# al-mcintyre/mCaller

Hardware: AMD Instinct MI355X
Metric: m6A calls/sec (GATC motif, E. coli-like synthetic eventalign) (higher is better)
Workload: dtype f64 (K1 window means, everything written); K2 hidden layer f32 + f64 output + f64 re-evaluation near print boundaries (MCALLER_MLP_FP64=1 = f64 throughout: ms_per_step_fp64_mlp); 1 GPU; synthetic 1e+08 eventalign rows per GPU and step, -m GATC, NN classifier (r95 two-base MLP), skip_thresh 0; two resident tables taken in turn, every step a FULL pass (the table declared new: positions + event indices streamed, every row validated); step=full pass, passes_in_flight=4, events_per_gpu=100000000, flush_records_per_gpu=204194, copy_out_bytes_per_pass=8767737

## Files before the change

include/mcaller_hip.h:

```cpp
#ifndef MCALLER_HIP_H
#define MCALLER_HIP_H

#define MC_E_NO_FREE_SLOT (-16)

#include <stdint.h>

#ifdef __cplusplus
extern "C" {
#endif

#define MC_MAX_K 8

#define MC_F_KMER_EQ    0x01
#define MC_F_MODEL_N    0x02
#define MC_F_SEG_START  0x04
#define MC_F_NAME_START 0x08

typedef struct mc_table_view {
    int64_t n_rows;
    const int32_t *pos;
    const int32_t *event_model_e4;
    const int32_t *event_idx;
    const uint8_t *flags;
    int32_t n_seg;
    const int64_t *seg_row_begin;
    const int32_t *seg_read;
    const int32_t *seg_contig;
    int32_t n_reads;
    const uint8_t *model_n_bits;
    const uint16_t *idx_rel_bits;
} mc_table_view;
void mc_pack_model_n(const uint8_t *flags, int64_t n_rows, uint8_t *out);
void mc_pack_idx_rel(const int32_t *event_idx, int64_t n_rows, uint16_t *out);

typedef struct mc_ref_view {
    int32_t n_contigs;
    const int64_t *contig_len;
    const int64_t *seq_off;
    const uint8_t *seq;
    const int64_t *word_off;
    const uint32_t *mbits_fwd;
    const uint32_t *mbits_rev;
    int64_t n_seq_bytes, n_words;
} mc_ref_view;

#define MC_I_EMPTY_MASK   0x000000FFu
#define MC_I_REV          0x00000100u
#define MC_I_TOO_MANY     0x00000200u
#define MC_I_MULTI        0x00000400u
#define MC_I_EDGE         0x00000800u
#define MC_I_NEXT_SHIFT   16

typedef struct mc_calls_view {
    int64_t capacity;
    double  *feats;
    int32_t *site_pos;
    int32_t *site_seg;
    int64_t *close_row;
    uint32_t *info;
    double  *prob;
    int32_t *call_row;
    int64_t n_call_rows;
    int32_t *close_row32;
    int32_t compacted;
    const int32_t *feats_lo32;
    const uint32_t *feats_hi32;
    const uint8_t *feats_wide;
    int64_t n_wide;
} mc_calls_view;

const char *mc_last_error(void);
const char *mc_version(void);
int mc_host_cores(void);
int mc_mark_motifs(const char *seq, int64_t n, const char *motif_fwd, const char *repl_fwd, int32_t m_fwd,
                   const char *motif_rev, const char *repl_rev, int32_t m_rev, char *upper_out, char *fwd_out, char *rev_out);

#define MC_IUPAC_MAX_MOTIFS 8
#define MC_IUPAC_MAX_LEN 32
typedef struct mc_iupac_motif {
    int32_t m;
    uint32_t called;
    uint8_t set[MC_IUPAC_MAX_LEN];
} mc_iupac_motif;
typedef struct mc_iupac_spec {
    int32_t n_motifs, pad;
    mc_iupac_motif fwd[MC_IUPAC_MAX_MOTIFS];
    mc_iupac_motif rev[MC_IUPAC_MAX_MOTIFS];
} mc_iupac_spec;
int mc_iupac_spec_add(mc_iupac_spec *spec, const char *motif, int32_t m, uint32_t called);
int mc_mark_iupac(const char *seq, int64_t n, const mc_iupac_spec *spec, char *upper_out, char *fwd_out, char *rev_out);

void *mc_host_alloc(int64_t bytes);
void mc_host_free(void *p);
int mc_host_is_pinned(const void *p);
int mc_host_pool_config(int32_t parser_uses_pool, int64_t keep_bytes);

typedef struct mc_parsed mc_parsed;
int mc_parse_eventalign(const char *path, int64_t startline, int64_t endline,
                        const char *const *contig_names, int32_t n_contigs, int32_t n_threads,
                        mc_parsed **out);
int mc_parse_eventalign_range(const char *path, int64_t byte_begin, int64_t byte_end,
                              const char *const *contig_names, int32_t n_contigs, int32_t n_threads, mc_parsed **out);
int mc_eventalign_read_cuts(const char *path, int32_t n_parts, int64_t *cuts);
int mc_eventalign_read_cuts_range(const char *path, int64_t lo, int64_t hi, int32_t n_parts, int64_t *cuts);
int mc_eventalign_read_cuts_at(const char *path, int64_t lo, int64_t hi, const int64_t *want, int32_t n_want, int64_t *cuts);
int mc_eventalign_consumed_range(const char *path, int64_t startline, int64_t endline, int64_t *lo, int64_t *hi);
int mc_parsed_view(const mc_parsed *p, mc_table_view *out);
const char *mc_parsed_read_name(const mc_parsed *p, int32_t read_id);
int64_t mc_parsed_n_unknown(const mc_parsed *p);
const char *mc_parsed_unknown_name(const mc_parsed *p, int64_t i);
int32_t mc_parsed_n_pieces(const mc_parsed *p);
void mc_parsed_free(mc_parsed *p);

typedef struct mc_fastq mc_fastq;
int mc_fastq_read_quality(const char *path, int32_t n_threads, mc_fastq **out);
int64_t mc_fastq_view(const mc_fastq *f, const char **key_pool, const int64_t **key_off, const double **mean);
void mc_fastq_free(mc_fastq *f);

typedef struct mc_ctx mc_ctx;
int mc_ctx_create(int device, mc_ctx **out);
int mc_bind_to_device_numa_node(int device);
// ... 142 lines not shown
} mc_nb_params;
int mc_nb_fit(mc_ctx *ctx, const mc_nb_params *prm, const double *X, const uint8_t *y, int64_t n_samples, int32_t n_in, int32_t n_jobs,
              const int64_t *train_off, const int32_t *train_idx, const int64_t *val_off, const int32_t *val_idx, double *theta,
              double *var, double *epsilon, int64_t *class_count, int64_t *val_correct);

typedef struct mc_devparse_result {
    int32_t status;
    int64_t n_lines, n_rows;
    int32_t n_seg, n_unknown;
    const int64_t *seg_row_begin;
    const int32_t *seg_contig;
    const int64_t *seg_name_off;
    const int32_t *seg_name_len;
    const uint8_t *seg_name_start;
    const int64_t *unknown_off;
    const int32_t *unknown_len;
    const uint8_t *flags;
} mc_devparse_result;
int mc_read_file_range(const char *path, int64_t byte_begin, int64_t byte_end, char *dst, int32_t n_threads);
int mc_map_file_range(const char *path, int64_t lo, int64_t hi, void **handle, const char **ptr);
void mc_unmap_file_range(void *handle);
int mc_ctx_parse_begin(mc_ctx *ctx, const char *text, int64_t n_bytes, const char *const *contig_names, int32_t n_contigs,
                       int64_t max_rows, int32_t *slot);
int mc_ctx_parse_end(mc_ctx *ctx, int32_t slot, mc_devparse_result *out);
int mc_ctx_parse_finish(mc_ctx *ctx, int32_t slot, const int32_t *seg_read, int32_t n_reads, const double *read_qual);
int mc_ctx_parse_abandon(mc_ctx *ctx, int32_t slot);
int mc_ctx_fetch_columns(mc_ctx *ctx, int32_t slot, int64_t n_rows, int32_t *pos, int32_t *event_model_e4, int32_t *event_idx,
                         uint8_t *flags);
int mc_ctx_fetch_model_n_bits(mc_ctx *ctx, int32_t slot, int64_t n_rows, uint8_t *out);
int mc_ctx_fetch_idx_rel_bits(mc_ctx *ctx, int32_t slot, int64_t n_rows, uint16_t *out);
int mc_ctx_fetch_pos_rel_bits(mc_ctx *ctx, int32_t slot, int64_t n_rows, uint16_t *out);
int mc_ctx_fetch_unit_summaries(mc_ctx *ctx, int32_t slot, int64_t n_rows, int32_t *out);

typedef struct mc_format_args {
    const mc_calls_view *rec;
    int64_t n_records;
    int32_t k;
    const mc_table_view *table;
    const mc_ref_view *ref;
    const char *const *contig_names;
    const char *const *read_names;
    const char *const *read_qual_txt;
    const char *tail_chrom;
    const char *label_meth;
    const char *label_unmeth;
    const uint8_t *submodel_of_char;
} mc_format_args;
int mc_format_diffs(const mc_format_args *args, int64_t first, int32_t n_threads, char **text, int64_t *n_bytes,
                    int64_t *n_rows, int64_t *stop_at);
int mc_count_records(const mc_calls_view *rec, int64_t n, const int32_t *seg_read, int64_t n_seg, int64_t *counts3, int32_t *ascending,
                     uint8_t *pos_marks, int64_t n_marks, int64_t *pos_min, int64_t *pos_top);
int mc_calls_expand(const mc_calls_view *rec, int64_t n_records, int32_t k, int32_t *call_row_out, int64_t *close_row_out,
                    double *feats_out);
void mc_free(void *p);
int mc_repr_double(double v, char *out32);
int mc_repr_fixed4(int32_t d, char *out32);
int mc_repr_double_rowtext(double v, char *out32);

typedef struct mc_text_source {
    const char *text;
    const char *path;
    int64_t n_bytes;
} mc_text_source;

typedef struct mc_bed_params {
    int64_t min_depth;
    double mod_threshold;
    int32_t control;
    int32_t with_probs;
    int32_t gff;
    int32_t site_stats;
} mc_bed_params;
typedef struct mc_bed_stats {
    int64_t n_bytes, n_lines, n_counted, n_entries, n_sites, n_out_bytes;
    int64_t decline_line;
    int32_t decline_reason;
    int32_t longest_probe;
    int64_t table_slots;
    int64_t kernel_bytes;
    double ms_read, ms_h2d, ms_kernels, ms_d2h, ms_total;
} mc_bed_stats;
#define MC_BED_DECLINE_HIGH_BYTE   1
#define MC_BED_DECLINE_CONTROL     2
#define MC_BED_DECLINE_FIELDS      3
#define MC_BED_DECLINE_POSITION    4
#define MC_BED_DECLINE_CONTEXT     5
#define MC_BED_DECLINE_LABEL       6
#define MC_BED_DECLINE_NO_PROB     7
#define MC_BED_DECLINE_LONG_LINE   8
#define MC_BED_DECLINE_TABLE       9
#define MC_BED_DECLINE_ROWS        10
#define MC_BED_DECLINE_MEMORY      11
#define MC_BED_DECLINE_OPTIONS     12
#define MC_BED_DECLINE_POS_HIGH_BYTE 13
#define MC_BED_DECLINE_POS_CONTROL   14
#define MC_BED_DECLINE_POS_LONG_LINE 15
#define MC_BED_DECLINE_VALUE         16
#define MC_BED_DECLINE_FEW_VALUES    17
#define MC_BED_DECLINE_MANY_VALUES   18
#define MC_BED_DECLINE_VALUE_COUNT   19
#define MC_BED_DECLINE_ZERO_VARIANCE 20
#define MC_BED_DECLINE_FAR_TAIL      21
#define MC_BED_DECLINE_PRINT_RANGE   22
#define MC_BED_DECLINE_ROUNDING_TIE  23
#define MC_BED_DECLINE_DEPTH         24
#define MC_BED_DECLINE_PROBABILITY   25
// ... 390 lines not shown
```

mcaller_amd/_lib.py:

```python
import ctypes as C
import os

import numpy as np

from . import _abi

_HERE = os.path.dirname(os.path.abspath(__file__))
LIB_PATH = os.environ.get('MCALLER_LIB') or os.path.join(_HERE, 'libmcaller_hip.so')

ABI = _abi.load()
_K, _S = ABI.constants, ABI.structs

MC_MAX_K = _K['MC_MAX_K']
F_KMER_EQ, F_MODEL_N, F_SEG_START, F_NAME_START = (_K['MC_F_' + n] for n in ('KMER_EQ', 'MODEL_N', 'SEG_START', 'NAME_START'))
I_EMPTY_MASK, I_REV, I_TOO_MANY, I_MULTI, I_EDGE, I_NEXT_SHIFT = (
    _K['MC_I_' + n] for n in ('EMPTY_MASK', 'REV', 'TOO_MANY', 'MULTI', 'EDGE', 'NEXT_SHIFT'))
E_NO_FREE_SLOT = _K['MC_E_NO_FREE_SLOT']


class McError(RuntimeError):
    code = None


TableView = _S['mc_table_view']
# ... 597 lines not shown
    if not (L.ndim == 1 and L.shape == bound.shape and len(L) >= 1):
        raise ValueError('curcombine: two arrays of one length, at least 1')
    out, b, st = np.zeros(2), C.c_double(), C.c_int32()
    rc = lib().mc_curcombine(L.ctypes.data, bound.ctypes.data, len(L), float(log10c), out.ctypes.data, C.byref(b), C.byref(st))
    if rc != 0:
        raise ValueError('mc_curcombine: %d' % rc)
    return float(out[0]), float(out[1]), float(b.value), int(st.value)


def hypergeom_round4(v):
    return lib().mc_hypergeom_round4(float(v))


def hypergeom_tie4(v, err):
    return bool(lib().mc_hypergeom_tie4(float(v), float(err)))


def parse_double(token):
    if isinstance(token, str):
        token = token.encode('latin-1', 'replace')
    out = C.c_double()
    return out.value if lib().mc_parse_double(token, len(token), C.byref(out)) else None


def repr_double_rowtext(x):
    buf = C.create_string_buffer(40)
    n = lib().mc_repr_double_rowtext(float(x), buf)
    return buf.value.decode() if n >= 0 else None


def repr_fixed4(d):
    buf = C.create_string_buffer(40)
    lib().mc_repr_fixed4(int(d), buf)
    return buf.value.decode()


class Records(object):

    def __init__(self, capacity, k):
        self.k = k
        self.capacity = int(capacity)
        c = max(1, self.capacity)
        self.feats = np.zeros(c * k, dtype=np.float64)
        self.site_pos = np.zeros(c, dtype=np.int32)
        self.site_seg = np.zeros(c, dtype=np.int32)
        self.close_row = np.zeros(c, dtype=np.int64)
        self.info = np.zeros(c, dtype=np.uint32)
        self.prob = np.full(c, np.nan, dtype=np.float64)
        self.n = 0

    def view(self):
        v = CallsView()
        v.capacity = self.capacity
        v.site_pos, v.site_seg = _ptr(self.site_pos), _ptr(self.site_seg)
        v.info, v.prob = _ptr(self.info), _ptr(self.prob)
        if self._feats is None and self._packed is not None:
            lo, hi, wide = self._packed
            v.feats_lo32, v.feats_hi32, v.feats_wide, v.n_wide = _ptr(lo), _ptr(hi), _ptr(wide), len(hi)
        else:
            v.feats = _ptr(self.feats)
        if self._close_row is not None or self._close_row32 is None:
            v.close_row = _ptr(self.close_row)
        else:
            v.close_row32 = _ptr(self._close_row32)
        if self._compacted:
            v.compacted, v.n_call_rows = 1, int(self._n_calls)
            if self._call_row is not None:
                v.call_row = _ptr(self._call_row)
        return v

    @classmethod
    def from_view(cls, v, n, k, owner):
        r = cls.__new__(cls)
        r.k, r.capacity, r.n, r._owner = k, n, n, owner
        if v.feats:
            r.feats = _from_ptr(v.feats, n * k, np.float64)
        r.site_pos = _from_ptr(v.site_pos, n, np.int32)
        r.site_seg = _from_ptr(v.site_seg, n, np.int32)
        if v.close_row:
            r._close_row = _from_ptr(v.close_row, n, np.int64)
        else:
            r._close_row32 = _from_ptr(v.close_row32, n, np.int32)
        r.info = _from_ptr(v.info, n, np.uint32)
        if v.compacted:
            m = int(v.n_call_rows)
            r._compacted = True
            if v.call_row:
                r._call_row = _from_ptr(v.call_row, n, np.int32)
            r._n_calls = m
            if v.feats:
                r.feats = _from_ptr(v.feats, m * k, np.float64)
            else:
                r._packed = (_from_ptr(v.feats_lo32, m * k, np.int32), _from_ptr(v.feats_hi32, int(v.n_wide), np.uint32),
                             _from_ptr(v.feats_wide, m, np.uint8))
            r.prob = _from_ptr(v.prob, m, np.float64)
        else:
            r.prob = _from_ptr(v.prob, n, np.float64)
        return r

    _close_row = _close_row32 = _call_row = _feats = _packed = None
    _compacted = False

    @property
    def feats(self):
        if self._feats is None and self._packed is not None:
            out = np.empty(max(1, self._n_calls * self.k), dtype=np.float64)
            v = self.view()
            check(lib().mc_calls_expand(C.byref(v), int(self.n), int(self.k), None, None, _ptr(out)))
            self._feats = out[:self._n_calls * self.k]
        return self._feats

    @feats.setter
    def feats(self, a):
        self._feats = a

    @property
    def close_row(self):
        if self._close_row is None and self._close_row32 is not None:
            self._close_row = self._close_row32.astype(np.int64)
        return self._close_row

    @close_row.setter
    def close_row(self, a):
        self._close_row = a

    @property
    def call_row(self):
        if self._call_row is None and self._compacted:
            keep = (self.info[:self.n] & I_TOO_MANY) == 0
            rows = np.cumsum(keep, dtype=np.int64) - 1
            rows[~keep] = -1
            self._call_row = rows.astype(np.int32)
        return self._call_row

    @call_row.setter
    def call_row(self, a):
        self._call_row = a
        self._compacted = a is not None

    def count(self, n, seg_read=None, pos_marks=None):
        v = self.view()
        counts = np.zeros(3, dtype=np.int64)
        asc, lo, top = C.c_int32(0), C.c_int64(0), C.c_int64(0)
        if seg_read is not None:
            seg_read = np.ascontiguousarray(seg_read, dtype=np.int32)
        check(lib().mc_count_records(C.byref(v), int(n), _ptr(seg_read) if seg_read is not None else None,
                                     len(seg_read) if seg_read is not None else 0, _ptr(counts) if seg_read is not None else None,
                                     C.byref(asc), _ptr(pos_marks) if pos_marks is not None else None,
                                     len(pos_marks) if pos_marks is not None else 0, C.byref(lo), C.byref(top)))
        return (tuple(int(c) for c in counts) if seg_read is not None else None), bool(asc.value), int(lo.value), int(top.value)

    @property
    def n_calls(self):
        return self._n_calls if self._compacted else self.n

    def by_record(self):
        if self.call_row is None:
            return self
        n, k = self.n, self.k
        r = Records(n, k)
        r.n = n
        for name in ('site_pos', 'site_seg', 'close_row', 'info'):
            getattr(r, name)[:n] = getattr(self, name)[:n]
        kept = self.call_row[:n] >= 0
        rows = self.call_row[:n][kept]
        r.feats.reshape(-1, k)[:n][kept] = self.feats.reshape(-1, k)[rows]
        r.prob[:n][kept] = self.prob[rows]
        return r


# ... 17 lines not shown
```

mcaller_amd/csrc/mc_classify.hip:

```cpp
#include "mc_dev.h"
#include "mc_rows.h"

namespace {

template <bool PIN>
struct VgprConstT {
    double v;
    __device__ __forceinline__ explicit VgprConstT(double x) : v(x) { if (PIN) asm volatile("" : "+v"(v)); }
    __device__ __forceinline__ operator double() const { return v; }
};
template <bool PIN>
struct ExpConstsT {
    using VgprConst = VgprConstT<PIN>;
    VgprConst two_log2e{2.8853900817779268}, magic{6755399441055744.0}, half_ln2_hi{-0.3465735901845619},
        half_ln2_lo{-9.541074646352939e-11};
    VgprConst t_max4{87.5};
    VgprConst g9{5.1405589494805136e-05}, g8{0.0002828297056809958}, g7{0.0014109321451518497}, g6{0.00634918945176432},
        g5{0.02539682542470863}, g4{0.08888888907016779}, g3{0.26666666666656197}, g2{0.6666666666659861},
        g1{1.3333333333333335}, g0{2.0000000000000004};
};
using ExpConsts = ExpConstsT<true>;

template <class EC>
__device__ __forceinline__ double exp2t_plus1(double t, const EC &C) {
// ... 85 lines not shown
__device__ __forceinline__ float tanh32s(float s) {
    return __builtin_fmaf(__builtin_amdgcn_rcpf(1.0f + __builtin_amdgcn_exp2f(s)), -2.0f, 1.0f);
}
__device__ __forceinline__ f2 tanh32s_2(f2 s) {
    const f2 d = (f2){__builtin_amdgcn_exp2f(s.x), __builtin_amdgcn_exp2f(s.y)} + 1.0f;
    const f2 r = {__builtin_amdgcn_rcpf(d.x), __builtin_amdgcn_rcpf(d.y)};
    return __builtin_elementwise_fma(r, (f2){-2.0f, -2.0f}, (f2){1.0f, 1.0f});
}

__device__ __forceinline__ double threshold_distance(double p) {
    const double t = p * 100.0;
    const double d = fabs((t - floor(t)) - 0.5) * 0.01;
    return fmin(d, fabs(p - 0.5));
}

struct K2Pieces {
    const int32_t *cnt;
    int room;
    int64_t n;
};
#ifndef MC_K2_THREADS
#define MC_K2_THREADS 1024
#endif
constexpr int K2_THREADS = MC_K2_THREADS;
constexpr int K2B = K2_THREADS;
constexpr int K2_WAVES = K2_THREADS / 64;
constexpr int K2_FIX = K2B + 256;
static_assert(K2_WAVES >= 4 && K2_WAVES % 4 == 0, "four unit quarters");
static_assert(K2_MAXM <= 16, "a wave's list claims are one atomic of K2_MAXM lanes; the loops over the sub-models are written out");

#ifdef MC_K2_TRACE
__device__ unsigned long long g_k2_trace[1024 * 16 * 16];
#define K2_STAMP(i) do { if (lane == 0 && blockIdx.x < 1024) g_k2_trace[((size_t)blockIdx.x * K2_WAVES + wave) * 16 + (i)] = wall_clock64(); g_k2_trace[((size_t)blockIdx.x * K2_WAVES + wave) * 16 + 8 + (i)] = clock64(); } while (0)
__device__ unsigned long long g_k2_timeline[256 * 24 * 8];
#define K2_TL(i) do { if (tid == 0 && blockIdx.x < 256 && stretch_no < 24) g_k2_timeline[((size_t)blockIdx.x * 24 + stretch_no) * 8 + (i)] = wall_clock64(); } while (0)
__device__ unsigned long long g_side_trace[1024 * 16 * 16];
#define K2_WALL(i) do { if ((threadIdx.x & 63) == 0 && blockIdx.x < 1024) g_side_trace[((size_t)blockIdx.x * K2_WAVES + (threadIdx.x >> 6)) * 16 + (i)] = wall_clock64(); } while (0)
#else
#define K2_STAMP(i) do { } while (0)
#define K2_TL(i) do { } while (0)
#define K2_WALL(i) do { } while (0)
#endif


#define MC_SCALAR_MEM __attribute__((address_space(4)))

struct SidePack {
    K1Args A;
    const Payload *sorted;
    unsigned char *out;
    size_t out_bytes;
    Counters *host_status;
    int close32, score;
};
struct NoPack {};
#ifndef MC_SIDE_WAVES
#define MC_SIDE_WAVES 4
#endif
template <int NI_T, bool FAST, bool PACK = false, bool ROOMY = false, int TH = K2_THREADS>
__global__ __launch_bounds__(TH) __attribute__((amdgpu_waves_per_eu((FAST && !ROOMY) ? 8 : (ROOMY && FAST ? MC_SIDE_WAVES : 4), (FAST && !ROOMY) ? 8 : (ROOMY && FAST ? MC_SIDE_WAVES : 4)))) void k2_mlp(DevMlp M, const double *__restrict__ feats, int k,
                                                     const int32_t *__restrict__ site_seg, const int32_t *__restrict__ seg_read,
                                                     const double *__restrict__ qual, const uint32_t *__restrict__ info,
                                                     const uint8_t *__restrict__ submodel_in, int64_t n,
                                                     double *__restrict__ prob, const unsigned long long *__restrict__ n_dev,
                                                     const unsigned int *__restrict__ overflow, K2Pieces P,
                                                     std::conditional_t<PACK, SidePack, NoPack> SP) {
    if constexpr (PACK) {
        if (*overflow) {
            constexpr unsigned head_words = offsetof(Counters, end_of_head) / 4;
            if (blockIdx.x == 0 && threadIdx.x < head_words)
                reinterpret_cast<volatile unsigned int *>(SP.host_status)[threadIdx.x] = reinterpret_cast<const unsigned int *>(SP.A.cnt)[threadIdx.x];
            return;
        }
    } else if (overflow && *overflow) return;
    if (n_dev) n = min(n, (int64_t)*n_dev);
    K2_WALL(0);
    constexpr int KB = TH, KW = TH / 64, KFIX = TH + 256;
    static_assert(KW >= 4 && KW % 4 == 0, "four unit quarters");
    constexpr int NX = NI_T ? NI_T : MC_MAX_K + 1;
    const int H = M.n_hidden, NI = NI_T ? NI_T : M.n_in, S = NI + 2, NM = min(M.n_models, K2_MAXM);
    using part_t = std::conditional_t<FAST, float, double>;
    __shared__ uint16_t s_list[K2_MAXM][KB];
    __shared__ int s_tot[2][K2_MAXM];
    __shared__ double s_q[KB];
    __shared__ part_t s_part[4][KB];
    __shared__ float s_marg[FAST ? KB : 1];
    __shared__ unsigned long long s_fixlist[FAST ? KFIX : 1];
    __shared__ int s_nfix;
    __shared__ int32_t s_slot[KB];
    __shared__ uint32_t s_fixrow[(FAST && PACK) ? KFIX : 1];
    __shared__ int2 s_pk[PACK ? 2 : 1][PACK ? KW : 1];
    __shared__ unsigned long long s_base[PACK ? 2 : 1][4];
    __shared__ unsigned long long s_red[PACK ? 6 : 1][PACK ? KW : 1];
    __shared__ unsigned long long s_lay[PACK ? 8 : 1];
    const int tid = threadIdx.x, lane = tid & 63;
    const int wave = __builtin_amdgcn_readfirstlane(tid >> 6);
    const unsigned long long below = (1ull << lane) - 1ull;
    const ExpConstsT<!FAST> C;
    K2_STAMP(0);
    __shared__ uint32_t s_simd_of_wave[KW / 4];
    const int simd = (int)__builtin_amdgcn_s_getreg((2 - 1) << 11 | 4 << 6 | 4) & 3;
    __shared__ uint8_t s_soc[256];
    if (tid < 256) s_soc[tid] = M.sub_of_char ? M.sub_of_char[tid] : (uint8_t)255;
    if (lane == 0) reinterpret_cast<uint8_t *>(s_simd_of_wave)[wave] = (uint8_t)simd;
    if (tid < 2 * K2_MAXM) (&s_tot[0][0])[tid] = 0;
    if (tid == 0) s_nfix = 0;
    __syncthreads();
    int quarter, g_first, g_step;
    {
        uint32_t per_simd = 0;
        int slot = 0;
        for (int w4 = 0; w4 < KW / 4; ++w4) {
            const uint32_t four = __builtin_amdgcn_readfirstlane(s_simd_of_wave[w4]);
#pragma unroll
            for (int b = 0; b < 4; ++b) {
                const int sd = (four >> (8 * b)) & 3;
                per_simd += 1u << (8 * sd);
                slot += (w4 * 4 + b < wave && sd == simd) ? 1 : 0;
            }
        }
        const bool by_simd = (per_simd & 0xFFu) && (per_simd & 0xFF00u) && (per_simd & 0xFF0000u) && (per_simd & 0xFF000000u);
        quarter = by_simd ? simd : wave & 3;
        g_first = by_simd ? slot : wave >> 2;
        g_step = by_simd ? (int)((per_simd >> (8 * simd)) & 0xFFu) : KW / 4;
    }
    const bool pieces = P.cnt != nullptr;
    const int64_t n_units = pieces ? P.n : n;
    const int64_t per = (n_units + gridDim.x - 1) / gridDim.x;
    int64_t lo = min(n_units, blockIdx.x * per), hi = min(n_units, lo + per);
    K2_WALL(1);
    if constexpr (PACK) {
        unsigned long long v[6] = {0, 0, 0, 0, 0, 0};
        if (pieces) {
            for (int64_t j0 = 32 * (int64_t)tid; j0 < P.n; j0 += 32 * TH) {
                int4 k4[8];
#pragma unroll
                for (int e = 0; e < 8; ++e) k4[e] = *reinterpret_cast<const int4 *>(SP.A.piece_kw + min(j0 + 4 * e, (P.n - 1) & ~(int64_t)3));
#pragma unroll
                for (int e = 0; e < 32; ++e) {
                    const int64_t j = j0 + e;
                    if (j >= P.n) continue;
                    const int4 kk = k4[e >> 2];
                    const uint32_t kw = (uint32_t)((e & 3) == 0 ? kk.x : (e & 3) == 1 ? kk.y : (e & 3) == 2 ? kk.z : kk.w);
                    const uint32_t c = kw & 511u, kept = (kw >> 9) & 511u, wide = kw >> 18;
                    v[0] += kept; v[1] += wide; v[2] += c;
                    if (j < lo) { v[3] += kept; v[4] += wide; v[5] += c; }
                }
            }
        } else {
            const int64_t per_c = (n + PACK_WGS - 1) / PACK_WGS;
            const int c0 = (int)((int64_t)blockIdx.x * PACK_WGS / gridDim.x), c1 = (int)((int64_t)(blockIdx.x + 1) * PACK_WGS / gridDim.x);
            lo = min(n, c0 * per_c); hi = min(n, c1 * per_c);
            for (int j = tid; j < PACK_WGS; j += TH) {
                const unsigned long long kk = SP.A.chunk_cnt[PACK_PAD * j], ww = SP.A.chunk_cnt[PACK_PAD * j + 1];
                v[0] += kk; v[1] += ww;
                if (j < c0) { v[3] += kk; v[4] += ww; }
            }
            if (tid == 0) { v[2] = (unsigned long long)n; v[5] = (unsigned long long)lo; }
        }
        K2_WALL(2);
        if (tid < 6) s_red[PACK ? tid : 0][0] = 0ull;
        __syncthreads();
#pragma unroll
        for (int i = 0; i < 6; ++i) {
            unsigned long long x = v[i];
#pragma unroll
            for (int o = 32; o > 0; o >>= 1) x += __shfl_xor(x, o);
            if (lane == 0 && x) atomicAdd(&s_red[PACK ? i : 0][0], x);
        }
        __syncthreads();
#pragma unroll
        for (int i = 0; i < 6; ++i) v[i] = s_red[PACK ? i : 0][0];
        __syncthreads();
        const size_t need_bytes = pack_tail(pack_layout((int64_t)v[2], SP.close32).feats, (size_t)v[0], k, (size_t)v[1]).end;
        const bool too_big = need_bytes > SP.out_bytes;
        if (too_big) lo = hi;
        if (tid == 0) {
            const PackLayout PL = pack_layout((int64_t)v[2], SP.close32);
            const PackTail PTl = pack_tail(PL.feats, (size_t)v[0], k, (size_t)v[1]);
            s_lay[0] = PL.pos; s_lay[1] = PL.seg; s_lay[2] = PL.info; s_lay[3] = PTl.lo32; s_lay[4] = PTl.wmask; s_lay[5] = PTl.hi32;
            s_lay[6] = PTl.prob;
            s_base[0][0] = v[3]; s_base[0][1] = v[4]; s_base[0][2] = v[5];
            s_red[0][1] = v[2]; s_red[1][1] = v[0]; s_red[2][1] = v[1];
            s_red[3][1] = need_bytes;
        }
        __syncthreads();
        K2_WALL(3);
        const int64_t n_rare = too_big ? 0 : (int64_t)SP.A.cnt->n_rare;
        if (n_rare > 0) {
            const int64_t rlo = pieces ? lo * P.room : lo, rhi = pieces ? hi * P.room : hi;
            for (int64_t i = tid; i < n_rare; i += TH) {
                const int64_t q = SP.A.rare_list[i];
#ifndef MC_SIDE_NO_RARE
                if (q >= rlo && q < rhi && finish_rare_record<false>(SP.A, SP.sorted, q, true)) {
                    const unsigned long long was = atomicExch(&SP.A.cnt->irregular_pass, SP.A.pass_no);
                    asm volatile("" :: "v"(was));
                }
#endif
            }
            __syncthreads();
        }
    }
    K2_WALL(4);
    K2_STAMP(1);
    auto again_in_fp64 = [&](int n_fix) {
        for (int f = wave; f < n_fix; f += KW) {
            const unsigned long long ent = s_fixlist[FAST ? f : 0];
            const int64_t r = (int64_t)(ent & ((1ull << 56) - 1ull));
            const int mdl = (int)(ent >> 56);
            double x[NX];
            const double q = qual[seg_read[site_seg[r]]];
#pragma unroll
            for (int i = 0; i < NX; ++i) x[i] = i < k ? feats[r * k + i] : (i == k ? q : 0.0);
            double part = 0.0;
            for (int u = lane; u < H; u += 64) {
                const double *wu = M.wu + ((size_t)mdl * H + u) * S;
                double a0 = x[0] * wu[0];
#pragma unroll
                for (int i = 1; i < NX; ++i)
                    if (i < NI) a0 = fma(x[i], wu[i], a0);
                part = fma(tanh_1exp(a0 + wu[NI], C), wu[NI + 1], part);
            }
#pragma unroll
            for (int o = 32; o > 0; o >>= 1) part += __shfl_xor(part, o);
            if (lane == 0) {
                const double pr = logistic(part + M.b2[mdl], C);
                prob[r] = pr;
                if constexpr (PACK) reinterpret_cast<double *>(SP.out + s_lay[PACK ? 6 : 0])[s_fixrow[(FAST && PACK) ? f : 0]] = pr;
            }
        }
    };
    int buf = 0, stretch_no = 0;
    (void)stretch_no;
    int64_t base = lo;
    while (base < hi) {
        K2_STAMP(7);
        K2_TL(0);
        int n_here, np_here = 1, my_slot = tid;
        int64_t slot0 = base;
        if (pieces) {
            const bool have = lane < 16 && base + lane < hi;
            const int c = have ? min(max(P.cnt[base + lane], 0), P.room) : 0;
            int incl = c;
#pragma unroll
            for (int o = 1; o < 16; o <<= 1) {
                const int v = __shfl_up(incl, o);
                if (lane >= o) incl += v;
            }
            np_here = max(1, __popcll(__ballot(have && incl <= KB)));
            n_here = min(__builtin_amdgcn_readlane(incl, np_here - 1), KB);
            int before = 0, j = 0;
#pragma unroll
            for (int t = 0; t < 15; ++t) {
                const int inc_t = __builtin_amdgcn_readlane(incl, t);
                if (t + 1 < np_here && inc_t <= tid) { j = t + 1; before = inc_t; }
            }
            my_slot = j * P.room + (tid - before);
            slot0 = base * (int64_t)P.room;
            s_slot[tid] = my_slot;
        } else n_here = (int)min((int64_t)KB, hi - base);
        const int64_t r = slot0 + my_slot;
        int mi = 255;
        double qv = 0.0;
        [[maybe_unused]] int p_nw = -1;
        if (tid < n_here) {
            if (submodel_in) mi = submodel_in[r];
            else {
                const uint32_t inf = info[r];
                const int32_t seg = site_seg[r];
                if constexpr (PACK) { if (!(inf & MC_I_TOO_MANY)) p_nw = __popc((uint32_t)SP.A.O.wmask[r] & ((1u << k) - 1u)); }
                bool scored = !(inf & (MC_I_TOO_MANY | MC_I_EDGE));
                if constexpr (PACK) scored = scored && SP.score != 0;
                if (scored) {
                    mi = s_soc[(inf >> MC_I_NEXT_SHIFT) & 0xFFu];
                    qv = qual[seg_read[seg]];
                }
            }
        }
        if constexpr (PACK) {
            const int nk = __popcll(__ballot(p_nw >= 0));
            int nw = max(p_nw, 0);
#pragma unroll
            for (int o = 32; o > 0; o >>= 1) nw += __shfl_xor(nw, o);
            if (lane == 0) s_pk[PACK ? buf : 0][PACK ? wave : 0] = make_int2(nk, nw);
        }
        int rank = 0, cnt_lane = 0;
#pragma unroll
        for (int m = 0; m < K2_MAXM; ++m) {
            const unsigned long long bal = __ballot(mi == m && m < NM);
            if (mi == m) rank = __popcll(bal & below);
            if (lane == m) cnt_lane = __popcll(bal);
        }
        int wbase = 0;
        if (lane < K2_MAXM && cnt_lane) wbase = atomicAdd(&s_tot[buf][lane], cnt_lane);
        int mybase = 0;
#pragma unroll
        for (int m = 0; m < K2_MAXM; ++m) {
            const int b = __builtin_amdgcn_readlane(wbase, m);
            mybase = mi == m ? b : mybase;
        }
        if (mi < NM) s_list[mi][mybase + rank] = (uint16_t)tid;
        s_q[tid] = qv;
        K2_STAMP(2);
        K2_WALL(5);
        K2_TL(1);
        __syncthreads();
        K2_WALL(6);
        K2_TL(2);
        int tot[K2_MAXM], gs[K2_MAXM], n_groups = 0;
#pragma unroll
        for (int m = 0; m < K2_MAXM; ++m) {
            tot[m] = __builtin_amdgcn_readfirstlane(s_tot[buf][m]);
            gs[m] = n_groups;
            n_groups += (tot[m] + 63) >> 6;
        }
        if (tid < K2_MAXM) s_tot[buf ^ 1][tid] = 0;
        K2_STAMP(3);
        K2_WALL(7);
        const int u0 = quarter * H / 4, u1 = (quarter + 1) * H / 4;
        for (int g = g_first; g < n_groups; g += g_step) {
            int mdl = 0, tot_m = tot[0], lg = g;
#pragma unroll
            for (int m = 1; m < K2_MAXM; ++m)
                if (g >= gs[m] && tot[m] > 0) { mdl = m; tot_m = tot[m]; lg = g - gs[m]; }
            const int idx = lg * 64 + lane;
            const bool valid = idx < tot_m;
            const int off = s_list[mdl][valid ? idx : lg * 64];
            const int64_t rr = slot0 + (pieces ? s_slot[off] : off);
            double x[NX];
            if (submodel_in) {
#pragma unroll
                for (int i = 0; i < NX; ++i) x[i] = i < NI ? feats[rr * NI + i] : 0.0;
            } else {
                const double q = s_q[off];
#pragma unroll
                for (int i = 0; i < NX; ++i) x[i] = i < k ? feats[rr * k + i] : (i == k ? q : 0.0);
            }
// ... 35 lines not shown
                        if (i < NI) m = __builtin_fmaf(fabsf(xx[i].x) * 1.0000002f, mg[1 + i], m);
                    s_marg[FAST ? off : 0] = m * 1.000001f;
                }
            } else {
                const MC_SCALAR_MEM double *wu = (const MC_SCALAR_MEM double *)M.wu + ((size_t)mdl * H + u0) * S;
                int u = u0;
                for (; u + 4 <= u1; u += 4, wu += 4 * S) {
                    double a0 = x[0] * wu[0], a1 = x[0] * wu[S], a2 = x[0] * wu[2 * S], a3 = x[0] * wu[3 * S];
    #pragma unroll
                    for (int i = 1; i < NX; ++i)
                        if (i < NI) {
                            a0 = fma(x[i], wu[i], a0);
                            a1 = fma(x[i], wu[S + i], a1);
                            a2 = fma(x[i], wu[2 * S + i], a2);
                            a3 = fma(x[i], wu[3 * S + i], a3);
                        }
                    a0 += wu[NI]; a1 += wu[S + NI]; a2 += wu[2 * S + NI]; a3 += wu[3 * S + NI];
                    tanh_4(a0, a1, a2, a3, C);
                    z = fma(a0, wu[NI + 1], z);
                    z = fma(a1, wu[S + NI + 1], z);
                    z = fma(a2, wu[2 * S + NI + 1], z);
                    z = fma(a3, wu[3 * S + NI + 1], z);
                }
                for (; u < u1; ++u, wu += S) {
                    double a0 = x[0] * wu[0];
    #pragma unroll
                    for (int i = 1; i < NX; ++i)
                        if (i < NI) a0 = fma(x[i], wu[i], a0);
                    z = fma(tanh_1exp(a0 + wu[NI], C), wu[NI + 1], z);
                }
            }
            if (valid) s_part[quarter][off] = (part_t)z;
        }
        K2_STAMP(4);
        K2_WALL(8);
        K2_TL(3);
        __syncthreads();
        K2_WALL(9);
        K2_STAMP(5);
        K2_TL(4);
        [[maybe_unused]] double p_pr = __longlong_as_double(0x7ff8000000000000LL);
        [[maybe_unused]] bool p_fix = false;
        if (mi < NM) {
            const double z = (((double)s_part[0][tid] + (double)s_part[1][tid]) + (double)s_part[2][tid]) + (double)s_part[3][tid];
            const double pr = logistic(z + M.b2[mi], C);
            prob[r] = pr;
            const bool fix = FAST && !(threshold_distance(pr) > (double)s_marg[FAST ? tid : 0]);
            if constexpr (PACK) { p_pr = pr; p_fix = fix; }
            else if (fix) s_fixlist[FAST ? atomicAdd(&s_nfix, 1) : 0] = (unsigned long long)r | (unsigned long long)mi << 56;
        }
        if constexpr (PACK) {
            K2_WALL(11);
            if (tid == 0) {
                unsigned kept_s = 0, wide_s = 0;
                for (int w = 0; w < KW; ++w) { const int2 c = s_pk[PACK ? buf : 0][PACK ? w : 0]; kept_s += (unsigned)c.x; wide_s += (unsigned)c.y; }
                s_base[PACK ? buf ^ 1 : 0][0] = s_base[PACK ? buf : 0][0] + kept_s;
                s_base[PACK ? buf ^ 1 : 0][1] = s_base[PACK ? buf : 0][1] + wide_s;
                s_base[PACK ? buf ^ 1 : 0][2] = s_base[PACK ? buf : 0][2] + (unsigned long long)n_here;
            }
            if (tid < n_here) {
                const uint32_t inf = info[r];
                const int32_t seg = site_seg[r], pos = SP.A.O.site_pos[r];
                const int64_t close = SP.A.O.close_row[r];
                const bool keep = !(inf & MC_I_TOO_MANY);
                const uint32_t wm = keep ? ((uint32_t)SP.A.O.wmask[r] & ((1u << k) - 1u)) : 0u;
                double fx[MC_MAX_K];
#pragma unroll
                for (int f = 0; f < MC_MAX_K; ++f) fx[f] = (keep && f < k) ? feats[r * k + f] : 0.0;
                const unsigned long long kb = __ballot(keep);
                const int nw = __popc(wm);
                int w_incl = nw;
#pragma unroll
                for (int o = 1; o < 64; o <<= 1) {
                    const int y = __shfl_up(w_incl, o);
                    if (lane >= o) w_incl += y;
                }
                unsigned long long row = s_base[PACK ? buf : 0][0] + (unsigned)__popcll(kb & below), wpos = s_base[PACK ? buf : 0][1] + (unsigned)(w_incl - nw);
#pragma unroll
                for (int w = 0; w < KW; ++w) {
                    const int2 c = s_pk[PACK ? buf : 0][PACK ? w : 0];
                    if (w < wave) { row += (unsigned)c.x; wpos += (unsigned)c.y; }
                }
                const unsigned long long real0 = s_base[PACK ? buf : 0][2];
                const int64_t io = pieces ? (int64_t)real0 + tid : r;
                unsigned char *const out = SP.out;
                if (SP.close32) reinterpret_cast<int32_t *>(out)[io] = (int32_t)close;
                else reinterpret_cast<int64_t *>(out)[io] = close;
                reinterpret_cast<int32_t *>(out + s_lay[0])[io] = pos;
                reinterpret_cast<int32_t *>(out + s_lay[PACK ? 1 : 0])[io] = seg;
                reinterpret_cast<uint32_t *>(out + s_lay[PACK ? 2 : 0])[io] = inf;
                if (keep) {
                    int32_t *o_lo = reinterpret_cast<int32_t *>(out + s_lay[PACK ? 3 : 0]) + row * k;
                    uint32_t *o_hi = reinterpret_cast<uint32_t *>(out + s_lay[PACK ? 5 : 0]);
                    (out + s_lay[PACK ? 4 : 0])[row] = (uint8_t)wm;
                    reinterpret_cast<double *>(out + s_lay[PACK ? 6 : 0])[row] = p_pr;
#pragma unroll
                    for (int f = 0; f < MC_MAX_K; ++f)
                        if (f < k) {
                            if (!((wm >> f) & 1u)) o_lo[f] = (int32_t)rint(fx[f] * 1e4);
                            else {
                                const unsigned long long bits = (unsigned long long)__double_as_longlong(fx[f]);
                                o_lo[f] = (int32_t)(uint32_t)bits;
                                o_hi[wpos++] = (uint32_t)(bits >> 32);
                            }
                        }
                    if (p_fix) {
                        const int at = atomicAdd(&s_nfix, 1);
                        s_fixlist[FAST ? at : 0] = (unsigned long long)r | (unsigned long long)mi << 56;
                        s_fixrow[(FAST && PACK) ? at : 0] = (uint32_t)row;
                    }
                }
            }
        }
        base += pieces ? np_here : KB;
        buf ^= 1;
        K2_STAMP(6);
        K2_WALL(10);
        K2_TL(5);
        ++stretch_no;
#ifdef MC_K2_TRACE
        if (lane == 0 && blockIdx.x < 1024)
            g_k2_trace[((size_t)blockIdx.x * K2_WAVES + wave) * 16 + 7] = (unsigned)simd | (unsigned)quarter << 4 | (unsigned)g_first << 8 | (unsigned)g_step << 16 | (unsigned long long)n_groups << 24;
#endif
    }
    if constexpr (FAST) {
        __syncthreads();
        again_in_fp64(s_nfix);
    }
    K2_WALL(13);
    if constexpr (PACK) {
        __shared__ int s_last;
        __syncthreads();
        if (tid == 0) s_last = atomicAdd(&SP.A.cnt->side_done, 1ull) == (unsigned long long)gridDim.x - 1ull;
        __syncthreads();
        if (s_last) {
            constexpr unsigned head_words = offsetof(Counters, end_of_head) / 4;
            constexpr int kept_word = (int)(offsetof(Counters, n_kept) / 4);
            constexpr int overflow_word = (int)(offsetof(Counters, overflow) / 4), need_word = (int)(offsetof(Counters, pack_need) / 4);
            static_assert(offsetof(Counters, n_wide) == offsetof(Counters, n_kept) + 8 && offsetof(Counters, n_records) == 0, "Counters layout");
            static_assert(sizeof(Counters::overflow) == 4 && sizeof(Counters::pack_need) == 8 && offsetof(Counters, pack_need) % 8 == 0, "Counters layout");
            const unsigned long long need_bytes = s_red[PACK ? 3 : 0][PACK ? 1 : 0];
            const bool too_big = need_bytes > SP.out_bytes;
            if (tid < (int)head_words && (tid < kept_word || tid >= kept_word + 4) && tid >= 2) {
                unsigned int w = __hip_atomic_load(reinterpret_cast<unsigned int *>(SP.A.cnt) + tid, __ATOMIC_RELAXED, __HIP_MEMORY_SCOPE_AGENT);
                if (too_big && tid == overflow_word) w |= 1u;
                if (too_big && (tid == need_word || tid == need_word + 1)) w = (unsigned int)(need_bytes >> (tid == need_word ? 0 : 32));
                reinterpret_cast<volatile unsigned int *>(SP.host_status)[tid] = w;
            }
            if (tid == 0) {
                *reinterpret_cast<volatile unsigned long long *>(&SP.host_status->n_records) = s_red[0][PACK ? 1 : 0];
                *reinterpret_cast<volatile unsigned long long *>(&SP.host_status->n_kept) = s_red[PACK ? 1 : 0][PACK ? 1 : 0];
                *reinterpret_cast<volatile unsigned long long *>(&SP.host_status->n_wide) = s_red[PACK ? 2 : 0][PACK ? 1 : 0];
            }
        }
    }
    K2_WALL(14);
}

constexpr int K3_THREADS = 256;
__global__ __launch_bounds__(K3_THREADS) void k3_forest(DevForest F, const double *__restrict__ feats, int k,
                                                        const int32_t *__restrict__ site_seg, const int32_t *__restrict__ seg_read,
                                                        const double *__restrict__ qual, const uint32_t *__restrict__ info,
                                                        const uint8_t *__restrict__ submodel_in, int64_t n,
                                                        double *__restrict__ prob, const unsigned long long *__restrict__ n_dev,
                                                        const unsigned int *__restrict__ overflow) {
    __shared__ double s_x[K3_THREADS][MC_MAX_K + 2];
    if (overflow && *overflow) return;
    if (n_dev) n = min(n, (int64_t)*n_dev);
    const int NI = F.n_in;
    const int tid = threadIdx.x, lane = tid & 63, wave = __builtin_amdgcn_readfirstlane(tid >> 6);
    const int64_t n_waves = (int64_t)gridDim.x * (K3_THREADS / 64);
    if (n <= n_waves * 16) {
        double *x = s_x[wave * 64];
        for (int64_t r = (int64_t)blockIdx.x * (K3_THREADS / 64) + wave; r < n; r += n_waves) {
            int mi;
            if (submodel_in) {
                mi = submodel_in[r];
                if (lane < NI) x[lane] = (double)(float)feats[r * NI + lane];
            } else {
                const uint32_t inf = info[r];
                if (inf & (MC_I_TOO_MANY | MC_I_EDGE)) continue;
                mi = F.sub_of_char[(inf >> MC_I_NEXT_SHIFT) & 0xFFu];
                if (lane < k) x[lane] = (double)(float)feats[r * k + lane];
                if (lane == k) x[k] = (double)(float)qual[seg_read[site_seg[r]]];
            }
            if (mi >= F.n_models) continue;
            __builtin_amdgcn_fence(__ATOMIC_ACQ_REL, "wavefront");
            const int t0 = F.model_tree_off[mi], t1 = F.model_tree_off[mi + 1];
            double sum = 0.0;
            for (int tb = t0; tb < t1; tb += 64) {
                const int t = tb + lane;
                double q = 0.0;
                if (t < t1) {
                    int node = F.tree_node_off[t];
                    int l;
                    while ((l = F.left[node]) >= 0) node = (x[F.feature[node]] <= F.threshold[node]) ? l : F.right[node];
                    const double v0 = F.value[2 * (size_t)node], v1 = F.value[2 * (size_t)node + 1];
                    double norm = (-0.0 + v0) + v1;
                    if (norm == 0.0) norm = 1.0;
                    q = v1 / norm;
                }
                const int here = min(64, t1 - tb);
                for (int j = 0; j < here; ++j)
                    sum += __hiloint2double(__builtin_amdgcn_readlane(__double2hiint(q), j), __builtin_amdgcn_readlane(__double2loint(q), j));
            }
// ... 333 lines not shown
            const bool literal = noted != 0xFFu || !look;
            for (int f = 0; f < k; ++f) {
                const double x = s_feats[tid * k + f];
                int32_t d = 0;
                const bool narrow = literal ? !((noted >> f) & 1u) : slot_is_narrow(x, &d);
                if (narrow) lo32[f] = literal ? (int32_t)rint(x * 1e4) : d;
                else {
                    const unsigned long long bits = (unsigned long long)__double_as_longlong(x);
                    lo32[f] = (int32_t)(uint32_t)bits;
                    hi32[n_w++] = (uint32_t)(bits >> 32);
                    wmask |= 1u << f;
                }
            }
        }
        const unsigned long long kmask = __ballot(keep);
        unsigned int w_incl = n_w;
        for (int o = 1; o < 64; o <<= 1) {
            const unsigned int y = __shfl_up(w_incl, o);
            if (lane >= o) w_incl += y;
        }
        const unsigned long long vmask = __ballot(valid);
        if (lane == 63) s_wave[1][wave] = w_incl;
        if (lane == 0) { s_wave[0][wave] = (unsigned int)__popcll(kmask); s_wave[2][wave] = (unsigned int)__popcll(vmask); }
        __syncthreads();
        unsigned int in_strip = (unsigned int)__popcll(kmask & ((1ull << lane) - 1ull)), strip = 0, w_off = w_incl - n_w, w_strip = 0;
        unsigned int r_in_strip = (unsigned int)__popcll(vmask & ((1ull << lane) - 1ull)), r_strip = 0;
        for (int j = 0; j < PACK_THREADS / 64; ++j) {
            if (j < wave) { in_strip += s_wave[0][j]; w_off += s_wave[1][j]; r_in_strip += s_wave[2][j]; }
            strip += s_wave[0][j];
            w_strip += s_wave[1][j];
            r_strip += s_wave[2][j];
        }
        if (valid) {
            const int64_t io = holes ? (int64_t)(rbase + r_in_strip) : i;
            if (close32) o_close32[io] = (int32_t)O.close_row[i];
            else o_close[io] = O.close_row[i];
            o_pos[io] = O.site_pos[i];
            o_seg[io] = O.site_seg[i];
            o_info[io] = info;
            if (keep) {
                const unsigned long long row = base + in_strip;
                o_prob[row] = O.prob[i];
                o_mask[row] = (uint8_t)wmask;
                for (int f = 0; f < k; ++f) o_lo[row * k + f] = lo32[f];
                for (unsigned int j = 0; j < n_w; ++j) o_hi[wbase + w_off + j] = hi32[j];
            }
        }
        __syncthreads();
        base += strip;
        wbase += w_strip;
        rbase += r_strip;
    }
}


}

#ifndef MC_K2_WG_PER_CU
#define MC_K2_WG_PER_CU 1
#endif
#ifndef MC_SIDE_WGS_SPARSE
#define MC_SIDE_WGS_SPARSE 128
#endif
#ifndef MC_K2_WG_MANY
#define MC_K2_WG_MANY 2
#endif

void mc_launch_classifier(const DevMlp &M, const DevForest &F, const DevSimple &S, const DevSvm &V, int n_cu, hipStream_t st, const double *feats, int k,
                          const int32_t *site_seg, const int32_t *seg_read, const double *qual, const uint32_t *info,
                          const uint8_t *submodel_in, int64_t n, double *prob, const unsigned long long *n_dev, const unsigned int *overflow,
                          const int32_t *piece_cnt, int piece_room, int64_t n_pieces) {
    if (n <= 0) return;
    const K2Pieces P{(piece_room > 0 && piece_room < K2B) ? piece_cnt : nullptr, piece_room, n_pieces};
    if (V.sv) {
        const unsigned grid = (unsigned)std::max<int64_t>(1, std::min<int64_t>((n + K3S_THREADS - 1) / K3S_THREADS, (int64_t)n_cu * 8));
        if (V.n_in == 7)
            hipLaunchKernelGGL(k3_svm<7>, dim3(grid), dim3(K3S_THREADS), 0, st, V, feats, k, site_seg, seg_read, qual, info, submodel_in, n,
                               prob, n_dev, overflow);
        else
            hipLaunchKernelGGL(k3_svm<0>, dim3(grid), dim3(K3S_THREADS), 0, st, V, feats, k, site_seg, seg_read, qual, info, submodel_in, n,
                               prob, n_dev, overflow);
    } else if (F.left)
        hipLaunchKernelGGL(k3_forest, dim3((unsigned)std::max<int64_t>(1, std::min<int64_t>((n + 3) / 4, (int64_t)n_cu * 8))), dim3(K3_THREADS), 0, st,
                           F, feats, k, site_seg, seg_read, qual, info, submodel_in, n, prob, n_dev, overflow);
    else if (S.params)
        hipLaunchKernelGGL(k3_simple, dim3((unsigned)((n + 63) / 64)), dim3(64), 0, st, S, feats, k, site_seg, seg_read, qual, info,
                           submodel_in, n, prob, n_dev, overflow);
    else {
        const bool fast = M.fast && M.wp32 && !submodel_in;
        const bool many = P.cnt != nullptr || n >= ((int64_t)4 << 20);
        const unsigned grid = (unsigned)std::max<int64_t>(1, std::min<int64_t>((n + 255) / 256, (int64_t)n_cu * ((fast && many) ? MC_K2_WG_MANY : MC_K2_WG_PER_CU)));
        if (M.n_in == 7 && fast)
            hipLaunchKernelGGL((k2_mlp<7, true>), dim3(grid), dim3(K2_THREADS), 0, st, M, feats, k, site_seg, seg_read, qual, info, submodel_in, n,
                               prob, n_dev, overflow, P, NoPack{});
        else if (M.n_in == 7)
            hipLaunchKernelGGL((k2_mlp<7, false>), dim3(grid), dim3(K2_THREADS), 0, st, M, feats, k, site_seg, seg_read, qual, info, submodel_in, n,
                               prob, n_dev, overflow, P, NoPack{});
        else if (fast)
            hipLaunchKernelGGL((k2_mlp<0, true>), dim3(grid), dim3(K2_THREADS), 0, st, M, feats, k, site_seg, seg_read, qual, info, submodel_in, n,
                               prob, n_dev, overflow, P, NoPack{});
        else
            hipLaunchKernelGGL((k2_mlp<0, false>), dim3(grid), dim3(K2_THREADS), 0, st, M, feats, k, site_seg, seg_read, qual, info, submodel_in, n,
                               prob, n_dev, overflow, P, NoPack{});
    }
}

void mc_launch_pack_count(const DevRecords &O, const Counters *cnt, int k, unsigned long long *chunk_cnt, int holes, hipStream_t st) {
    hipLaunchKernelGGL(k_pack_count, dim3(PACK_WGS), dim3(PACK_THREADS), 0, st, O, cnt, k, chunk_cnt, holes);
}

void mc_launch_pack(const DevRecords &O, const Counters *cnt, const unsigned long long *chunk_cnt, unsigned char *out, size_t out_bytes, int k,
                    int close32, Counters *host_status, int holes, int look, hipStream_t st, hipEvent_t stop) {
    if (stop) hipExtLaunchKernelGGL(k_pack, dim3(PACK_WGS), dim3(PACK_THREADS), 0, st, nullptr, stop, 0, O, cnt, chunk_cnt, out, out_bytes, k, close32, host_status, holes, look);
    else hipLaunchKernelGGL(k_pack, dim3(PACK_WGS), dim3(PACK_THREADS), 0, st, O, cnt, chunk_cnt, out, out_bytes, k, close32, host_status, holes, look);
}

bool mc_launch_side(const DevMlp &M, bool other_classifier, int n_cu, hipStream_t st, const K1Args &A, const Payload *sorted, const int32_t *seg_read,
                    const double *qual, int64_t cap, int score, unsigned char *out, size_t out_bytes, int close32, Counters *host_status,
                    int piece_room, int64_t n_pieces, hipEvent_t stop) {
    static const bool off = getenv("MCALLER_SIDE_FUSED") && atoi(getenv("MCALLER_SIDE_FUSED")) == 0;
    if (off || cap <= 0) return false;
    if (score && (other_classifier || !M.W1)) return false;
    const bool by_piece = piece_room > 0;
    constexpr int TH_SIDE = MC_SIDE_MAX_ROOM;
    if (by_piece ? (piece_room >= TH_SIDE || !A.piece_kw || !A.piece_cnt) : !A.chunk_cnt) return false;
    SidePack SP;
    SP.A = A; SP.sorted = sorted; SP.out = out; SP.out_bytes = out_bytes; SP.host_status = host_status; SP.close32 = close32; SP.score = score;
    const K2Pieces P{by_piece ? A.piece_cnt : nullptr, piece_room, n_pieces};
    const bool fast = score && M.fast && M.wp32;
    unsigned grid;
    const int grid_env = getenv("MCALLER_SIDE_GRID") ? atoi(getenv("MCALLER_SIDE_GRID")) : 0;
    if (by_piece) grid = (unsigned)std::max<int64_t>(1, std::min<int64_t>(n_pieces, grid_env > 0 ? (int64_t)grid_env : (int64_t)n_cu * (MC_SIDE_WAVES / 2)));
    else {
        const int want = grid_env > 0 ? grid_env : MC_SIDE_WGS_SPARSE;
        grid = 1;
        while (grid * 2 <= (unsigned)std::min<int64_t>(std::min(want, PACK_WGS), (int64_t)n_cu * 2)) grid *= 2;
    }
    const unsigned long long *n_dev = (const unsigned long long *)&A.cnt->n_records;
    const unsigned int *overflow = (const unsigned int *)&A.cnt->overflow;
#define MC_SIDE_LAUNCH(NI, FA) hipExtLaunchKernelGGL((k2_mlp<NI, FA, true, true, TH_SIDE>), dim3(grid), dim3(TH_SIDE), 0, st, nullptr, stop, 0, M, (const double *)A.O.feats, A.k, \
        (const int32_t *)A.O.site_seg, seg_read, qual, (const uint32_t *)A.O.info, (const uint8_t *)nullptr, cap, A.O.prob, n_dev, overflow, P, SP)
    if (score && M.n_in == 7 && fast) MC_SIDE_LAUNCH(7, true);
    else if (score && M.n_in == 7) MC_SIDE_LAUNCH(7, false);
    else if (fast) MC_SIDE_LAUNCH(0, true);
    else MC_SIDE_LAUNCH(0, false);
#undef MC_SIDE_LAUNCH
    return true;
}

namespace {
__global__ void k_tanh32_err(unsigned long long *out) {
    unsigned long long worst = 0ull;
    for (unsigned long long i = blockIdx.x * (unsigned long long)blockDim.x + threadIdx.x; i < (1ull << 32); i += (unsigned long long)gridDim.x * blockDim.x) {
        const float x = __uint_as_float((unsigned)i);
        if (!(fabsf(x) <= 3.4e38f)) continue;
        const double err = fabs((double)tanh32s(x) - tanh((double)x * 0.34657359027997264));
        const unsigned long long b = (unsigned long long)__double_as_longlong(err);
        worst = b > worst ? b : worst;
    }
    for (int o = 32; o > 0; o >>= 1) { const unsigned long long v = __shfl_xor(worst, o); worst = v > worst ? v : worst; }
    if ((threadIdx.x & 63) == 0) atomicMax(out, worst);
}
}
extern "C" int mc_debug_tanh32_max_err(double *out) {
    unsigned long long *d = nullptr;
    HIP_TRY(hipMalloc((void **)&d, 8));
    HIP_TRY(hipMemset(d, 0, 8));
    hipLaunchKernelGGL(k_tanh32_err, dim3(4096), dim3(256), 0, 0, d);
    unsigned long long h = 0;
    HIP_TRY(hipMemcpy(&h, d, 8, hipMemcpyDeviceToHost));
    (void)hipFree(d);
    memcpy(out, &h, 8);
    return 0;
}

#ifdef MC_K2_TRACE
extern "C" int mc_debug_k2_timeline(unsigned long long *out, int64_t n_words) {
    if (n_words > 256 * 24 * 8) n_words = 256 * 24 * 8;
    return hipMemcpyFromSymbol(out, HIP_SYMBOL(g_k2_timeline), (size_t)n_words * 8) == hipSuccess ? 0 : -10;
}
// ... 10 lines not shown
```

mcaller_amd/csrc/mc_ctx.h:

```cpp
#pragma once
#include "mc_dev.h"
#include "mc_own.h"

#include <atomic>
#include <string>

#ifndef MC_PASSES_IN_FLIGHT_N
#define MC_PASSES_IN_FLIGHT_N 6
#endif
constexpr int MC_PASSES_IN_FLIGHT = MC_PASSES_IN_FLIGHT_N;
constexpr int MC_ROW_TEXT_BLOCKS = 6;
static_assert(MC_ROW_TEXT_BLOCKS <= 8, "a block's handle is ticket * 8 + index");

constexpr size_t COPY_BY_KERNEL_MAX = (size_t)4 << 20;
constexpr size_t COPY_BY_KERNEL_MAX_STREAMING = (size_t)64 << 20;

struct K0Set {
    NbDesc *desc = nullptr;
    int64_t *nb_f0 = nullptr;
};

struct PassBufs {
    K0Set K;
    Counters *cnt = nullptr;
// ... 74 lines not shown
    int kp_state = 0;
    bool from_parser = false;
    int64_t kp_flags_sent = 0;
    std::vector<int64_t> kp_seg_row, kp_seg_off, kp_unk_off;
    std::vector<int32_t> kp_seg_contig, kp_seg_len, kp_unk_len;
    std::vector<uint8_t> kp_seg_ns;
    Pool kp_allocs{"device parser slot"};
    long long tmpl_ref = -1;
    Pool allocs{"table slot"};
};

struct Classifier {
    enum Kind { NONE = -1, MLP = 0, FOREST = 1, SIMPLE = 2, SVM = 3 };
    DevMlp M;
    DevForest F;
    DevSimple Sc;
    DevSvm Vs;
    Pool pool{"classifier"};
    Kind kind = NONE;
    int n_in = 0;
    const uint8_t *sub_of_char = nullptr;
    void clear() {
        pool.clear();
        M = DevMlp(); F = DevForest(); Sc = DevSimple(); Vs = DevSvm();
        kind = NONE; n_in = 0; sub_of_char = nullptr;
    }
    void set(Kind k, int n, const uint8_t *soc) { kind = k; n_in = n; sub_of_char = soc; }
};

enum {
    EV_K0_START, EV_K0_END, EV_SCAN_START, EV_SCAN_END, EV_EMIT_END, EV_K2_START, EV_K2_END,
    EV_LIST_END,
    EV_EMIT_START,
    EV_DONE, EV_COPIED, EV_TEXT, EV_N
};

struct AsyncBuf {
    PassBufs B;
    DevRecords H;
    Pinned st;
    unsigned char *pack = nullptr;
    Pinned pack_host;
    unsigned long long *chunk_cnt = nullptr;
    int32_t *piece_cnt = nullptr;
    int32_t *piece_kw = nullptr;
    int64_t piece_cap = 0;
    size_t pack_bytes = 0;
    int32_t *h_lo32 = nullptr;
    uint32_t *h_hi32 = nullptr;
    unsigned char *h_wmask = nullptr;
    int64_t h_n_wide = 0;
    int32_t *h_close32 = nullptr;
    bool close32 = false;
    int64_t h_n_calls = 0;
    Event ev[EV_N];
    mc_params prm;
    int64_t cap = 0, n_nb = 0;
    int k = 0;
    bool used = false, copying = false, timed = true;
    bool one_kernel = false;
    int want_text = 0;
    int text_block = -1;
    bool emit_aside = false;
    int fused_room = 0;
    int64_t slots = 0;
    int slot = -1;
    const double *qual = nullptr;
    int32_t n_qual = 0;
    Pool dev_allocs{"pass buffers"}, k0_allocs{"strand resolve output"};
};

struct RowTextCtx {
    int on = 0;
    char lab_meth[8] = {}, lab_unmeth[8] = {};
    int lab_meth_len = 0, lab_unmeth_len = 0;
    RowTextScratch S = {};
    int64_t cap_rec = 0, cap_rows = 0, cap_wide = 0, cap_num = 0;
    Pool allocs{"row text scratch"}, out_allocs{"row text"};
    char *out = nullptr;
    size_t out_cap = 0;
    double bytes_per_row = 0.0;
    bool room_forced = false;
    struct Block {
        Pinned text, st;
        size_t cap = 0;
        std::atomic<int> busy{0};
    } blocks[MC_ROW_TEXT_BLOCKS];
    int next_ticket = 0;
    long long n_text = 0, n_no_block = 0, n_host_needed = 0, n_too_small = 0, n_other = 0;
    int last_block = -1;
    int64_t last_bytes = 0, last_rows = 0;
};

struct TextStages {
    Pinned stage[2];
    size_t cap = 0;
    Event ev[2];
    void release() {
        for (Pinned &p : stage) p.reset();
        cap = 0;
    }
};

struct mc_ctx {
    int device = 0;
    Stream stream;
// ... 115 lines not shown
```

mcaller_amd/csrc/mc_dev.h:

```cpp
#ifndef MC_DEV_H
#define MC_DEV_H
#include <hip/hip_runtime.h>
#include <hip/hip_ext.h>
#include <sched.h>

#include <algorithm>
#include <cctype>
#include <chrono>
#include <cmath>
#include <cstdio>
#include <cstdlib>
#include <cstring>
#include <type_traits>
#include <vector>

#include "../../include/mcaller_hip.h"

void mc_set_error(const char *fmt, ...);

#define HIP_TRY(expr)                                                                       \
    do {                                                                                    \
        hipError_t _e = (expr);                                                             \
        if (_e != hipSuccess) {                                                             \
            mc_set_error("%s failed: %s (%s:%d)", #expr, hipGetErrorString(_e), __FILE__, __LINE__); \
// ... 76 lines not shown
    double *feats = nullptr;
    int32_t *site_pos = nullptr, *site_seg = nullptr;
    int64_t *close_row = nullptr;
    uint32_t *info = nullptr;
    double *prob = nullptr;
    uint8_t *wmask = nullptr;
};

struct DevMlp {
    int32_t n_models = 0, n_in = 0, n_hidden = 0;
    double *W1 = nullptr, *b1 = nullptr, *W2 = nullptr, *b2 = nullptr;
    double *wu = nullptr;
    float *wp32 = nullptr;
    float *margin = nullptr;
    int fast = 0;
    uint8_t *sub_of_char = nullptr;
};
constexpr double K2_TANH32_MAX_ERR = 2.5e-7;

struct DevForest {
    int32_t n_models = 0, n_in = 0;
    int32_t *model_tree_off = nullptr, *tree_node_off = nullptr, *left = nullptr, *right = nullptr, *feature = nullptr;
    double *threshold = nullptr, *value = nullptr;
    uint8_t *sub_of_char = nullptr;
};

struct DevSimple {
    int32_t kind = 0, n_models = 0, n_in = 0, stride = 0;
    double *params = nullptr;
    uint8_t *sub_of_char = nullptr;
};

constexpr int K3S_MAXM = 8;
struct DevSvm {
    int32_t n_models = 0, n_in = 0;
    int32_t *model_sv_off = nullptr;
    double *sv = nullptr, *params = nullptr;
    uint8_t *sub_of_char = nullptr;
};

constexpr int NSHARD = 64, SHARD_PAD = 16;

struct Counters {
    unsigned long long n_records;
    unsigned int overflow;
    unsigned int violation;
    unsigned int n_big;
    unsigned int n_rare;
    unsigned long long n_kept;
    unsigned long long n_wide;
    unsigned long long side_done;
    unsigned long long pack_need;
    unsigned long long irregular_pass;
    unsigned long long end_of_head;
    unsigned long long pad_to_line[SHARD_PAD];
    unsigned long long shard[NSHARD * SHARD_PAD];
};
constexpr unsigned long long ST_UNPUBLISHED = ~0ull;

#define MC_FRONT_OF_THE_QUEUE __builtin_amdgcn_s_setprio(3)
#ifndef MC_SCAN_SUMMARY
#define MC_SCAN_SUMMARY 1
#endif
#ifndef MC_EVENTS_ON_KERNELS
#define MC_EVENTS_ON_KERNELS 1
#endif

__device__ __forceinline__ double div1e4(int x) {
    const double xd = (double)x, r = 1.0 / 10000.0;
    const double q0 = xd * r;
    return fma(fma(-q0, 10000.0, xd), r, q0);
}

__device__ __forceinline__ bool slot_is_narrow(double v, int32_t *d_out) {
    const double t = rint(v * 1e4);
    if (!(fabs(t) < 2147483648.0)) return false;
    const int32_t d = (int32_t)t;
    if (__double_as_longlong(div1e4(d)) != __double_as_longlong(v)) return false;
    *d_out = d;
    return true;
}

__device__ __forceinline__ int first_m(const uint32_t *__restrict__ bits, int64_t L, int64_t pos, int k) {
    if (pos >= L) return -1;
    const int64_t w0 = pos >> 5;
    const uint64_t lo = bits[w0], hi = bits[w0 + 1];
    uint64_t w = ((hi << 32) | lo) >> (pos & 31);
    w &= (1ull << k) - 1ull;
    return w ? __builtin_ctzll(w) : -1;
}

__device__ __forceinline__ int bit_at(const uint32_t *__restrict__ bits, int64_t p) {
    return (int)((bits[p >> 5] >> (p & 31)) & 1u);
}

__device__ __forceinline__ unsigned char comp_char(unsigned char c) {
    switch (c) {
        case 'A': return 'T';
        case 'C': return 'G';
        case 'G': return 'C';
        case 'T': return 'A';
        case 'N': return 'N';
        case 'M': return 'M';
        default: return 0xFF;
    }
}

constexpr uint32_t MC_I_BIG = 0x1000u;
// ... 2 lines not shown

struct RowSrc {
    const int32_t *g_pos;
    const int2 *g_evmu;
    const uint8_t *g_flags;
    bool stray_pending;
    double stray_val;
};

__device__ __forceinline__ double next_val(RowSrc &S, int64_t &cur) {
    if (S.stray_pending) {
        S.stray_pending = false;
        return S.stray_val;
    }
    for (;;) {
        const int64_t r = cur++;
        if (!(S.g_flags[r] & MC_F_MODEL_N)) {
            const int2 e = S.g_evmu[r];
            return (double)(e.x - e.y) / 10000.0;
        }
    }
}

__device__ __forceinline__ double leaf_sum(RowSrc &S, int64_t &cur, int n) {
    const int n8 = n < 8 ? 0 : n - (n % 8);
    double r0 = 0.0, r1 = 0.0, r2 = 0.0, r3 = 0.0, r4 = 0.0, r5 = 0.0, r6 = 0.0, r7 = 0.0;
    for (int i = 0; i < n8; ++i) {
        const double v = next_val(S, cur);
        switch (i & 7) {
            case 0: r0 += v; break;
            case 1: r1 += v; break;
            case 2: r2 += v; break;
            case 3: r3 += v; break;
            case 4: r4 += v; break;
            case 5: r5 += v; break;
            case 6: r6 += v; break;
            default: r7 += v; break;
        }
    }
    double res = n8 ? ((r0 + r1) + (r2 + r3)) + ((r4 + r5) + (r6 + r7)) : -0.0;
    for (int i = n8; i < n; ++i) res += next_val(S, cur);
    return res;
}

#ifndef MC_PACK_WGS
#define MC_PACK_WGS 512
#endif
#ifndef MC_PACK_THREADS
#define MC_PACK_THREADS 512
#endif
constexpr int PACK_WGS = MC_PACK_WGS, PACK_THREADS = MC_PACK_THREADS;

constexpr int PACK_PAD = 16;

__device__ __forceinline__ void count_for_packing(unsigned long long *chunk_cnt, int64_t q, int64_t n_rec, bool kept, int n_wide) {
    if (!chunk_cnt || !kept) return;
    const uint32_t per = (uint32_t)((n_rec + PACK_WGS - 1) / PACK_WGS);
    const uint32_t b = (uint32_t)q / per;
    atomicAdd(&chunk_cnt[PACK_PAD * b], 1ull);
    if (n_wide) atomicAdd(&chunk_cnt[PACK_PAD * b + 1], (unsigned long long)n_wide);
}

__device__ __forceinline__ void count_wave_for_packing(unsigned long long *chunk_cnt, int64_t n_rec, bool kept, int64_t q, uint32_t wmask, int k) {
    if (!chunk_cnt) return;
    const unsigned long long km = __ballot(kept);
    if (!km) return;
    uint32_t per = (uint32_t)((n_rec + PACK_WGS - 1) / PACK_WGS);
    asm volatile("" : "+s"(per));
    const uint32_t bq = kept ? (uint32_t)q / per : 0u;
    const int first = __ffsll((unsigned long long)km) - 1;
    const uint32_t b0 = (uint32_t)__shfl((int)bq, first);
    if (!__ballot(kept && bq != b0)) {
        int nw = 0;
        for (int f = 0; f < k; ++f) nw += __popcll(__ballot(kept && ((wmask >> f) & 1u)));
        if ((int)(threadIdx.x & 63) == first) {
            atomicAdd(&chunk_cnt[PACK_PAD * b0], (unsigned long long)__popcll(km));
            if (nw) atomicAdd(&chunk_cnt[PACK_PAD * b0 + 1], (unsigned long long)nw);
        }
    } else if (kept) {
        atomicAdd(&chunk_cnt[PACK_PAD * bq], 1ull);
        if (wmask) atomicAdd(&chunk_cnt[PACK_PAD * bq + 1], (unsigned long long)__popc(wmask));
    }
}

constexpr uint32_t PF_EXTRA = 1, PF_CLOSE_NS = 2, PF_MULTI = 8, PF_REV = 16, PF_STRAY = 32;
constexpr int WROWS = 64;
constexpr int FRONT = 64;

struct __attribute__((aligned(16))) Payload {
    int64_t r;
    int64_t close_row;
    int32_t m;
    int32_t close_pos;
    uint32_t flags;
    int32_t nb;
};
static_assert(sizeof(Payload) == 32, "Payload layout");

constexpr int MC_SIDE_MAX_ROOM = 512;

struct K1Args {
    DevTable T;
    DevRef R;
    const NbDesc *desc;
    Payload *payload;
    long long payload_cap;
    long long *tile_chunk;
    int chunk_shift;
    int shard_shift;
    int shard_mask;
    int32_t *tile_cnt;
    int32_t *tile_half;
    const int32_t *tile_local;
    const int64_t *group_sum;
    int64_t *tile_first;
    DevRecords O;
    Counters *cnt;
    int k, skip_thresh, tail_contig;
// ... 15 lines not shown
            if (!(T.flags[rr] & MC_F_MODEL_N)) { close_pos = T.pos[rr]; return rr; }
            ++rr;
            continue;
        }
        close_ns = true;
        while (bb + 1 < T.n_nb && T.nb_row_begin[bb + 1] <= rr) ++bb;
        if (desc[bb].filtered) { rr = T.nb_row_begin[bb + 1]; continue; }
        if (!(T.flags[rr] & MC_F_MODEL_N)) { close_pos = T.pos[rr]; return rr; }
        ++rr;
    }
    close_ns = true;
    return tail_contig >= 0 ? T.n_rows : -1;
}

constexpr int PT = 16;
constexpr int NCHUNK = TILE / 64 + 1;
#ifndef MC_CHUNK
#define MC_CHUNK 1024
#endif
constexpr int CHUNK = MC_CHUNK;
constexpr int NCH = TILE / CHUNK;
constexpr int NQ = CHUNK / 512;
static_assert(CHUNK % 512 == 0 && TILE % CHUNK == 0, "whole stripes, whole chunks");

constexpr int NQT = TILE / 512;

__host__ __device__ inline bool scan_tile_is_whole(const NbDesc &d, int64_t t0, int nrows) {
    if (nrows != TILE || d.row_begin >= t0 || d.row_end < t0 + TILE) return false;
    return d.mode != MODE_REGULAR || (d.first() >= 0 && d.first() <= t0);
}

constexpr int GROUP = 1024;

__device__ __forceinline__ int64_t tile_slot(const int32_t *__restrict__ tile_local, const int64_t *__restrict__ group_sum,
                                             int64_t tile, int lane) {
    const int g = (int)(tile / GROUP);
    long long part = 0;
    for (int i = lane; i < g; i += 64) part += group_sum[i];
    for (int o = 32; o > 0; o >>= 1) part += __shfl_xor(part, o);
    return part + tile_local[tile];
}

constexpr int EG = 8;
constexpr int K2_MAXM = 8;

struct PackLayout { size_t pos, seg, info, feats; };
__host__ __device__ inline PackLayout pack_layout(int64_t n, int close32) {
    PackLayout L;
    L.pos = (size_t)n * (close32 ? 4 : 8);
    L.seg = L.pos + (size_t)n * 4;
    L.info = L.seg + (size_t)n * 4;
    L.feats = (L.info + (size_t)n * 4 + 7) & ~(size_t)7;
    return L;
}

struct PackTail { size_t lo32, prob, wmask, hi32, end; };
__host__ __device__ inline PackTail pack_tail(size_t feats_off, size_t m, int k, size_t n_wide) {
    PackTail T;
    T.lo32 = feats_off;
    T.prob = (T.lo32 + m * (size_t)k * 4 + 7) & ~(size_t)7;
    T.wmask = T.prob + m * 8;
    T.hi32 = (T.wmask + m + 3) & ~(size_t)3;
    T.end = T.hi32 + n_wide * 4;
    return T;
}

struct LitArgs {
    DevTable T;
    DevRef R;
    const NbDesc *desc;
    const int64_t *nb_f0;
    const double *qual;
    double qual_thresh;
    int k, skip_thresh, tail_contig, entry_read, entry_first_idx;
    int32_t *run_cnt;
    int32_t *run_rows;
    const int32_t *cnt_local;
    const int64_t *cnt_group;
    const int32_t *rows_local;
    const int64_t *rows_group;
    double *scratch;
    DevRecords L;
    int write;
};


constexpr int SCAN_VALIDATE = 0;
constexpr int SCAN_STREAM = 1;
constexpr int SCAN_SUMMARY = 2;
constexpr int SCAN_VALIDATE_SUMMARY = 3;


void mc_launch_first_site(const DevTable &T, const DevRef &R, const double *qual, double qual_thresh, int k, NbDesc *desc, int64_t *nb_f0,
                          Counters *cnt, int classify, int skip_thresh, unsigned long long pass_no, int hyp, int make_tmpl, hipStream_t st);
void mc_launch_classify(const DevTable &T, const DevRef &R, NbDesc *desc, const int64_t *nb_f0, int entry_read, int k, int skip_thresh,
                        Counters *cnt, unsigned long long pass_no, hipStream_t st);
void mc_launch_extend(const DevTable &T, NbDesc *desc, const int64_t *nb_f0, int entry_read, Counters *cnt, unsigned long long pass_no,
                      hipStream_t st);
void mc_launch_unit_columns(const DevTable &T, hipStream_t st);
void mc_launch_scan(const K1Args &A, bool dense, int scan_mode, hipStream_t st);
void mc_launch_group_scan(const int32_t *cnt, int64_t n, int32_t *local, int64_t *group_sum, hipStream_t st);
void mc_launch_list(const K1Args &A, Payload *sorted, int gather, hipStream_t st, hipEvent_t stop = nullptr);
int mc_emit_occupancy(void);
void mc_launch_emit(const K1Args &A, const Payload *sorted, unsigned grid, hipStream_t st, hipEvent_t stop, hipEvent_t start = nullptr);
void mc_launch_emit_runs(const K1Args &A, Payload *sorted, hipStream_t st, hipEvent_t stop);
int mc_fused_room(double density);
int mc_fused_room_max(void);
int64_t mc_fused_pieces(const DevTable &T);
void mc_launch_fused(const K1Args &A, Payload *sorted, int cap, bool validate, hipStream_t st, hipEvent_t stop);
void mc_launch_rare(const K1Args &A, const Payload *sorted, const int64_t *rare_list, int64_t n_rare, hipStream_t st);
void mc_launch_rare_dev(const K1Args &A, const Payload *sorted, const int64_t *rare_list, hipStream_t st);
void mc_launch_bigfix(const K1Args &A, int64_t n, hipStream_t st);
void mc_launch_literal(const LitArgs &LA, unsigned grid, hipStream_t st);
void mc_launch_merge(const DevRecords &O, int64_t n_o, const DevRecords &L, int64_t n_l, const DevRecords &M, int k, hipStream_t st);
void mc_launch_classifier(const DevMlp &M, const DevForest &F, const DevSimple &S, const DevSvm &V, int n_cu, hipStream_t st, const double *feats, int k,
                          const int32_t *site_seg, const int32_t *seg_read, const double *qual, const uint32_t *info,
                          const uint8_t *submodel_in, int64_t n, double *prob, const unsigned long long *n_dev, const unsigned int *overflow,
                          const int32_t *piece_cnt = nullptr, int piece_room = 0, int64_t n_pieces = 0);
void mc_launch_pack_count(const DevRecords &O, const Counters *cnt, int k, unsigned long long *chunk_cnt, int holes, hipStream_t st);
void mc_launch_pack(const DevRecords &O, const Counters *cnt, const unsigned long long *chunk_cnt, unsigned char *out, size_t out_bytes, int k,
                    int close32, Counters *host_status, int holes, int look, hipStream_t st, hipEvent_t stop);
bool mc_launch_side(const DevMlp &M, bool other_classifier, int n_cu, hipStream_t st, const K1Args &A, const Payload *sorted, const int32_t *seg_read,
                    const double *qual, int64_t cap, int score, unsigned char *out, size_t out_bytes, int close32, Counters *host_status,
                    int piece_room, int64_t n_pieces, hipEvent_t stop);

struct KpSeg { long long row; long long name_off; int name_len; int contig; int name_start; int pad; };

struct RowTextStatus {
    unsigned long long n_bytes;
    unsigned long long n_rows;
    unsigned int host_needed;
    unsigned int too_small;
};

struct RowTextIn {
    const unsigned char *pack;
    int64_t n, m, n_wide;
    int k, close32;
    const int64_t *seg_begin;
    const int32_t *seg_read, *seg_contig;
    int32_t n_seg;
    const KpSeg *segs;
    const char *text;
    const double *qual;
    int32_t n_qual;
    DevRef R;
    const uint32_t *cn_off, *cn_len;
    const char *cn_chars;
    const uint8_t *sub_of_char;
    int32_t tail_contig;
    char lab_meth[8], lab_unmeth[8];
    int lab_meth_len, lab_unmeth_len;
};

struct RowTextScratch {
    uint32_t *kept_blk, *wide_blk;
    uint32_t *wide_pref;
    uint32_t *rec_len, *rec_row;
    unsigned long long *len_blk;
    double *wval;
    unsigned long long *num_lo;
    uint32_t *num_meta;
    RowTextStatus *st;
};

void mc_row_text_scratch_sizes(int64_t n, int64_t m, int64_t *rec_blocks, int64_t *row_blocks);
void mc_launch_row_text(const RowTextIn &I, const RowTextScratch &S, char *out, size_t out_cap, char *out_host, RowTextStatus *st_host,
                        hipStream_t st);
void mc_launch_row_text_probe(const RowTextIn &I, const RowTextScratch &S, const int32_t *fixed, int64_t n_fixed, const double *prob,
                              int64_t n_prob, int shift, char *out, int32_t *len, uint8_t *ok, hipStream_t st);

#endif
```

mcaller_amd/csrc/mc_emit.hip:

```cpp
#include "mc_dev.h"
#include "mc_rows.h"

namespace {

__device__ __forceinline__ void emit_extra(const K1Args &A, const NbDesc &d, int nb_abs, int64_t slot) {
    int close_pos;
    bool close_ns;
    const int64_t close_row = find_close(A.T, A.desc, A.tail_contig, nb_abs, d.row_end, d.extra_row(), close_pos, close_ns);
    for (int s = 0; s < A.k; ++s) A.O.feats[slot * A.k + s] = 0.0;
    A.O.site_pos[slot] = d.extra_mpos;
    A.O.site_seg[slot] = A.T.nb_seg_begin[nb_abs];
    A.O.close_row[slot] = close_row;
    A.O.info[slot] = MC_I_TOO_MANY | ((!close_ns && d.extra_multi()) ? MC_I_MULTI : 0u);
    A.O.wmask[slot] = 0xFF;
    A.O.prob[slot] = __longlong_as_double(0x7ff8000000000000LL);
}


__device__ __forceinline__ Payload tile_payload(const K1Args &A, int64_t tile, int j) {
    long long slot = tile * PT + j;
    if (j >= PT) slot = A.tile_chunk[tile * NCHUNK + ((j - PT) >> A.chunk_shift)] + ((j - PT) & ((1 << A.chunk_shift) - 1));
    return A.payload[slot];
}

// ... 6 lines not shown
    const int64_t q = rare_list[i];
    const Payload P = sorted[q];
    const NbDesc d = A.desc[P.nb];
    RowSrc S{A.T.pos, A.T.evmu, A.T.flags, false, 0.0};
    emit_record(A, S, d, P.nb, P.r, P.m, q);
    bigfix_record(A, q);
}

#ifdef MC_EM_TRACE
__device__ unsigned long long g_em_trace[1024 * 2 * 8];
#define EM_STAMP(i) do { if (threadIdx.x == 0 && blockIdx.x < 1024 && em_round < 2) g_em_trace[(blockIdx.x * 2 + em_round) * 8 + (i)] = wall_clock64(); } while (0)
#else
#define EM_STAMP(i) do { } while (0)
#endif
#ifndef MC_EMIT_WAVES
#define MC_EMIT_WAVES 6
#endif
__global__ __launch_bounds__(256) __attribute__((amdgpu_waves_per_eu(MC_EMIT_WAVES, MC_EMIT_WAVES))) void k1_emit(K1Args A, const Payload *__restrict__ sorted) {
    const DevTable &T = A.T;
    const int lane = threadIdx.x & 63;
    [[maybe_unused]] int em_round = 0;
    EM_STAMP(7);
    if (A.cnt->overflow) return;
    const int64_t n_rec = min((int64_t)A.cnt->n_records, A.O.capacity);
    const int k = A.k;
    const int64_t stride = (int64_t)gridDim.x * blockDim.x;
    Payload Pn;
    Pn.flags = PF_EXTRA; Pn.nb = 0; Pn.r = 0; Pn.m = 0; Pn.close_row = 0; Pn.close_pos = 0;
    {
        const int64_t q0 = (blockIdx.x * (int64_t)blockDim.x + threadIdx.x) / EG;
        if (q0 < n_rec) Pn = sorted[q0];
    }
    const int wave_in_wg = __builtin_amdgcn_readfirstlane((int)threadIdx.x >> 6);
    for (int64_t tw = blockIdx.x * (int64_t)blockDim.x + wave_in_wg * 64; tw / EG < n_rec; tw += stride) {
    int lane_now = lane;
    uint32_t nan_hi = 0x7ff80000u;
    asm volatile("" : "+v"(lane_now), "+v"(nan_hi));
    const int64_t t = tw + lane_now;
    EM_STAMP(0);
    const int s = lane_now & (EG - 1);
    const int gsh = lane_now & ~(EG - 1);
    const double no_prob = __longlong_as_double((long long)((unsigned long long)nan_hi << 32));
    const int64_t q = t / EG;
    const bool live = q < n_rec;
    const Payload P = Pn;
    {
        const int64_t qn = (t + stride) / EG;
        Pn.flags = PF_EXTRA;
        if (qn < n_rec) Pn = sorted[qn];
    }
    const int64_t r = P.r;
    const int m = P.m;
    const bool window = live && !(P.flags & PF_EXTRA);
    const NbDesc *dp = A.desc + P.nb;
    static_assert(offsetof(NbDesc, row_begin) == 0 && offsetof(NbDesc, mask_off) == 16 && offsetof(NbDesc, first_delta) == 24 && offsetof(NbDesc, contig_len) == 28,
                  "the descriptor's second 16 bytes: mask_off, first_delta, contig_len");
    int2 d_rb = *reinterpret_cast<const int2 *>(&dp->row_begin);
    int4 d_1 = reinterpret_cast<const int4 *>(dp)[1];
    int32_t d_sdel = dp->seq_delta;
    int32_t seg_of = T.nb_seg_begin[P.nb];
    int pj[4];
    uint32_t fj[4];
    {
        const int32_t *pp = T.pos + (r - s);
        const uint8_t *fp = T.flags + (r - s);
#pragma unroll
        for (int e = 0; e < 4; ++e) {
            pj[e] = pp[-8 * e];
            fj[e] = fp[-8 * e];
        }
    }
    asm volatile("" : "+v"(d_rb.x), "+v"(d_rb.y), "+v"(d_1.x), "+v"(d_1.y), "+v"(d_1.z), "+v"(d_1.w), "+v"(d_sdel),
                      "+v"(seg_of), "+v"(pj[0]), "+v"(pj[1]), "+v"(pj[2]), "+v"(pj[3]), "+v"(fj[0]), "+v"(fj[1]), "+v"(fj[2]), "+v"(fj[3]));
    EM_STAMP(1);
    const int64_t d_row_begin = ((int64_t)(uint32_t)d_rb.x) | ((int64_t)d_rb.y << 32), d_mask_off = ((int64_t)(uint32_t)d_1.x) | ((int64_t)d_1.y << 32);
    const int64_t d_first = d_1.z < 0 ? -1 : d_row_begin + d_1.z;
    const int64_t Lc = d_1.w;
    if (live && !window && s == 0) {
        for (int s2 = 0; s2 < k; ++s2) A.O.feats[q * k + s2] = 0.0;
        A.O.wmask[q] = 0;
        A.O.site_pos[q] = m;
        A.O.site_seg[q] = seg_of;
        A.O.close_row[q] = P.close_row;
        A.O.info[q] = MC_I_TOO_MANY | ((!(P.flags & PF_CLOSE_NS) && (dp->xflags & 1)) ? MC_I_MULTI : 0u);
        A.O.prob[q] = no_prob;
    }
    uint32_t W = 0xFFFFFFFFu;
    bool stop_any = false;
    int back = 0;
    auto sort_rows = [&](const int E0) {
#pragma unroll
        for (int e = 0; e < 4; ++e) {
            const bool inb = 8 * (E0 + e) <= back;
            const bool nj = fj[e] & MC_F_MODEL_N;
            const int code = m - pj[e];
            const bool inw = inb && !nj && code >= 0 && code < k;
            stop_any = stop_any || !inb || (!nj && code >= k);
            W = (W & ~(15u << (4 * (E0 + e)))) | ((inw ? (uint32_t)code : 15u) << (4 * (E0 + e)));
        }
    };
    if (window) {
        back = (int)min(r - max(d_row_begin, d_first), (int64_t)1 << 20) - s;
        sort_rows(0);
    }
    bool covered = ((__ballot(stop_any) >> gsh) & 0xFFull) != 0ull;
    if (__ballot(window && !covered)) {
        if (window && !covered) {
            const int32_t *pp = T.pos + (r - s);
            const uint8_t *fp = T.flags + (r - s);
#pragma unroll
            for (int e = 0; e < 4; ++e) {
                pj[e] = pp[-8 * (4 + e)];
                fj[e] = fp[-8 * (4 + e)];
            }
            sort_rows(4);
        }
        covered = ((__ballot(stop_any) >> gsh) & 0xFFull) != 0ull;
    }
    const bool fast = window && covered;
    if (window && !covered && s == 0) A.rare_list[atomicAdd(&A.cnt->n_rare, 1u)] = q;
    EM_STAMP(2);
    const bool rev0 = P.flags & PF_REV;
    const bool edge = m - k + 1 < 0 || (int64_t)m + k > Lc || m < 1 || m + 1 >= Lc;
    const int at = edge ? 0 : (rev0 ? m - 1 : m + 1);
    uint32_t ctx_word = ((rev0 ? A.R.mr : A.R.mf) + d_mask_off)[at >> 5];
    const bool seq_near = d_sdel != NO_SEQ_DELTA;
    uint32_t ctx_base = A.R.seq[(seq_near ? 32 * d_mask_off + d_sdel : (int64_t)0) + at];
// ... 60 lines not shown
                    v[p] = is_stray[p] ? stray_val : div1e4(e[p].x - e[p].y);
                if (base + 8 <= n8) {
                    r0 += v[0]; r1 += v[1]; r2 += v[2]; r3 += v[3]; r4 += v[4]; r5 += v[5]; r6 += v[6]; r7 += v[7];
                    if (base + 8 == n8) acc = ((r0 + r1) + (r2 + r3)) + ((r4 + r5) + (r6 + r7));
                } else {
#pragma unroll
                    for (int p = 0; p < 8; ++p)
                        if (base + p < n) acc += v[p];
                }
            }
            f = (0.0 + acc) / (double)n;
        }
        const int dst = (too_many || rev) ? s : k - 1 - s;
        A.O.feats[q * k + dst] = f;
        int32_t as_int;
        if (!too_many && !slot_is_narrow(f, &as_int)) wide_bit = 1u << dst;
    }
    wide_bit |= (unsigned)__shfl_xor((int)wide_bit, 1);
    wide_bit |= (unsigned)__shfl_xor((int)wide_bit, 2);
    wide_bit |= (unsigned)__shfl_xor((int)wide_bit, 4);
    if (s == 0) {
        A.O.wmask[q] = (uint8_t)wide_bit;
        uint32_t info = rev ? MC_I_REV : 0u;
        if (too_many) info |= MC_I_TOO_MANY;
        else {
            uint32_t em = empties;
            if (!rev) em = (__brev(empties) >> 24) >> (8 - k);
            info |= em & MC_I_EMPTY_MASK;
            info_ctx = true;
        }
        if (P.flags & PF_MULTI) info |= MC_I_MULTI;
        A.O.site_pos[q] = m;
        A.O.site_seg[q] = seg_of;
        A.O.close_row[q] = P.close_row;
        A.O.prob[q] = no_prob;
        info_out = info;
        kept_rec = !too_many;
    }
    }
    EM_STAMP(3);
    asm volatile("" : "+v"(ctx_word), "+v"(ctx_base));
    EM_STAMP(4);
    if (fast && s == 0) {
        if (info_ctx) {
            if (edge) info_out |= MC_I_EDGE;
            else {
                if (!seq_near) ctx_base = A.R.seq[A.R.seq_off[dp->contig] + at];
                const unsigned char ch = ((ctx_word >> (at & 31)) & 1u) ? 'M' : (rev0 ? comp_char((unsigned char)ctx_base) : (unsigned char)ctx_base);
                info_out |= ((uint32_t)ch) << MC_I_NEXT_SHIFT;
            }
        }
        A.O.info[q] = info_out;
    }
    count_wave_for_packing(A.chunk_cnt, n_rec, kept_rec, q, wide_bit, k);
    EM_STAMP(5);
    ++em_round;
    }
}

#ifndef MC_ET
#define MC_ET 1024
#endif
#ifndef MC_ER_WAVES
#define MC_ER_WAVES 7
#endif
constexpr int ET = MC_ET;
#ifndef MC_EH
#define MC_EH 128
#endif
constexpr int EH = MC_EH;
constexpr int ER = ET + EH;
constexpr int E_THREADS = 256;
constexpr int E_MAXB = 16;
constexpr uint8_t RUN_WIDE = 1, RUN_UNUSABLE = 2;
static_assert(TILE % ET == 0, "whole pieces per tile");

#ifdef MC_ER_TRACE
__device__ unsigned long long g_er_trace[1024 * 8];
#define ER_STAMP(i) do { if (tid == 0 && blockIdx.x >= 40000 && blockIdx.x < 41024) g_er_trace[(blockIdx.x - 40000) * 8 + (i)] = wall_clock64(); } while (0)
#else
#define ER_STAMP(i) do { } while (0)
#endif

struct RunBlock {
    int16_t end, lb;
    int id, contig, contig_len, stray_q;
    uint32_t xflags;
    int64_t mask_off;
};
static_assert(sizeof(RunBlock) == 32, "RunBlock layout");

__device__ __forceinline__ void lds_barrier() { asm volatile("s_waitcnt lgkmcnt(0)\n\ts_barrier" ::: "memory"); }

constexpr int E_CHUNKS = ER / 64;
constexpr int E_CPW = 5;
static_assert(ER % 64 == 0 && E_THREADS == 256 && (E_CHUNKS + 3) / 4 <= E_CPW, "the chunks are split over 4 waves, at most E_CPW each");
static_assert(ER < (1 << 12), "s_rrow keeps RUN_* above the row");
constexpr int E_RF_SHIFT = 12;

__global__ __launch_bounds__(E_THREADS) __attribute__((amdgpu_waves_per_eu(MC_ER_WAVES, MC_ER_WAVES))) void k1_emit_runs(K1Args A, Payload *__restrict__ sorted) {
    __shared__ uint8_t s_rid[ET];
    __shared__ int16_t s_cb[E_CHUNKS];
    __shared__ int32_t s_dc[ER + 8];
    __shared__ double s_mean[ER];
    __shared__ uint16_t s_rpos[ER];
    __shared__ uint16_t s_rrow[ER];
    __shared__ uint16_t s_rc0[ER + 2];
// ... 361 lines not shown
```

mcaller_amd/csrc/mc_format.cpp:

```cpp
#include "mc_decimal.h"
#include "mc_sortkey.h"
#include "mc_rowtext.h"
#include "mc_tstat.h"
#include "mc_hypergeom.h"
#include "mc_fisher.h"
#include "mc_bh.h"
#include "mc_twosample.h"
#include "mc_curcombine.h"
#include "mc_npsum.h"
#include "../../include/mcaller_hip.h"

#include <algorithm>
#include <charconv>
#include <chrono>
#include <cstdio>
#include <cmath>
#include <cstdlib>
#include <cstring>
#include <functional>
#include <mutex>
#include <string>
#include <vector>

void mc_set_error(const char *fmt, ...);
// ... 105 lines not shown
    }
}

struct PartBuf {
    char *p = nullptr;
    size_t cap = 0, used = 0;
    void need(size_t more) {
        if (used + more <= cap) return;
        const size_t ncap = std::max(cap * 2, used + more + (1u << 20));
        char *q = (char *)realloc(p, ncap);
        if (!q) throw std::bad_alloc();
        p = q; cap = ncap;
    }
};
std::mutex g_fmt_mu;
std::vector<PartBuf> g_parts;
struct OutBlock { char *p; size_t cap; bool busy; };
std::mutex g_out_mu;
std::vector<OutBlock> g_out;

char *out_alloc(size_t n) {
    std::lock_guard<std::mutex> lk(g_out_mu);
    int best = -1;
    for (size_t i = 0; i < g_out.size(); ++i)
        if (!g_out[i].busy && g_out[i].cap >= n && (best < 0 || g_out[i].cap < g_out[(size_t)best].cap)) best = (int)i;
    if (best >= 0) { g_out[(size_t)best].busy = true; return g_out[(size_t)best].p; }
    const size_t cap = std::max<size_t>(n + n / 4, 1u << 20);
    char *p = (char *)malloc(cap);
    if (!p) return nullptr;
    for (size_t i = 0; i < g_out.size(); ++i)
        if (!g_out[i].busy) { free(g_out[i].p); g_out[i] = OutBlock{p, cap, true}; return p; }
    if (g_out.size() < 4) { g_out.push_back(OutBlock{p, cap, true}); return p; }
    return p;
}

bool out_release(void *p) {
    std::lock_guard<std::mutex> lk(g_out_mu);
    for (auto &b : g_out)
        if (b.p == p) { b.busy = false; return true; }
    return false;
}

struct Job {
    const mc_format_args *a;
    std::vector<size_t> name_len, qual_len, contig_len_txt;
    size_t tail_len = 0, lab_pos_len = 0, lab_neg_len = 0;
};

inline int32_t seg_of_row(const mc_table_view *t, int64_t r) {
    const int64_t *b = t->seg_row_begin, *e = b + t->n_seg + 1;
    return (int32_t)(std::upper_bound(b, e, r) - b) - 1;
}

inline bool build_context(const mc_format_args *a, int64_t j, char *ctx) {
    const mc_calls_view *rec = a->rec;
    const mc_ref_view *ref = a->ref;
    const int k = a->k;
    const uint32_t info = rec->info[j];
    if (info & MC_I_EDGE) return false;
    const int32_t seg = rec->site_seg[j];
    if (seg < 0 || seg >= a->table->n_seg) return false;
    const int32_t cid = a->table->seg_contig[seg];
    if (cid < 0 || cid >= ref->n_contigs) return false;
    const int64_t L = ref->contig_len[cid], m = rec->site_pos[j];
    const int64_t lo = m - k + 1, hi = m + k;
    if (lo < 0 || hi > L) return false;
    const bool rev = info & MC_I_REV;
    const uint8_t *seq = ref->seq + ref->seq_off[cid];
    const uint32_t *bits = (rev ? ref->mbits_rev : ref->mbits_fwd) + ref->word_off[cid];
    const int n = 2 * k - 1;
    for (int i = 0; i < n; ++i) {
        const int64_t p = lo + i;
        const int c = ((bits[p >> 5] >> (p & 31)) & 1u) ? 'M' : seq[p];
        if (!rev) ctx[i] = (char)c;
        else {
            const int cc = comp_of(c);
            if (cc < 0) return false;
            ctx[n - 1 - i] = (char)cc;
        }
    }
    if (ctx[k - 1] != 'M') return false;
    const unsigned char nxt = (unsigned char)ctx[k];
    if (a->submodel_of_char[nxt] == 255) return false;
    if (((info >> MC_I_NEXT_SHIFT) & 0xFFu) != nxt) return false;
    return true;
}

inline int64_t close_row_of(const mc_calls_view *rec, int64_t j) {
    return rec->close_row ? rec->close_row[j] : (int64_t)rec->close_row32[j];
}

int64_t kept_in(const mc_calls_view *rec, int64_t lo, int64_t hi) {
    int64_t kept = 0;
    for (int64_t j = lo; j < hi; ++j) kept += (rec->info[j] & MC_I_TOO_MANY) ? 0 : 1;
    return kept;
}

int64_t wide_before(const mc_calls_view *rec, int64_t row) {
    int64_t w = 0;
    for (int64_t r = 0; r < row; ++r) w += __builtin_popcount(rec->feats_wide[r]);
    return w;
}

struct RowCursor {
    const mc_calls_view *rec;
    int64_t kept;
    int64_t wide;
    bool wide_known;
    RowCursor(const mc_calls_view *r, int64_t first)
        : rec(r), kept(r->compacted && !r->call_row ? kept_in(r, 0, first) : 0), wide(0), wide_known(false) {}
    RowCursor(const mc_calls_view *r, int64_t kept_before, int64_t wide_before_)
        : rec(r), kept(kept_before), wide(wide_before_), wide_known(true) {}
    int64_t row(int64_t j, uint32_t info) {
        if (!rec->compacted) return j;
        if (rec->call_row) return rec->call_row[j];
        return (info & MC_I_TOO_MANY) ? -1 : kept++;
    }
    unsigned feats_for_print(int64_t row, int k, double *f, int32_t *d) {
        if (rec->feats) { memcpy(f, rec->feats + row * k, (size_t)k * sizeof(double)); return 0u; }
        if (!wide_known) { wide = wide_before(rec, row); wide_known = true; }
        const unsigned mask = rec->feats_wide[row];
        const int32_t *lo = rec->feats_lo32 + row * k;
        for (int s = 0; s < k; ++s) {
            if ((mask >> s) & 1u) {
                const uint64_t bits = ((uint64_t)rec->feats_hi32[wide++] << 32) | (uint32_t)lo[s];
                memcpy(&f[s], &bits, 8);
            } else {
                d[s] = lo[s];
            }
        }
        return ~mask & ((1u << k) - 1u);
    }
    void feats(int64_t row, int k, double *f) {
        if (rec->feats) { memcpy(f, rec->feats + row * k, (size_t)k * sizeof(double)); return; }
        if (!wide_known) { wide = wide_before(rec, row); wide_known = true; }
        const unsigned mask = rec->feats_wide[row];
        const int32_t *lo = rec->feats_lo32 + row * k;
        for (int s = 0; s < k; ++s) {
            if ((mask >> s) & 1u) {
                const uint64_t bits = ((uint64_t)rec->feats_hi32[wide++] << 32) | (uint32_t)lo[s];
                memcpy(&f[s], &bits, 8);
            } else {
                f[s] = (double)lo[s] / 1e4;
            }
        }
    }
};

int64_t format_range(const Job &J, int64_t j0, int64_t j1, PartBuf &out_shared, int64_t &n_rows_shared, const RowCursor &start) {
    PartBuf out = out_shared;
    int64_t n_rows = 0;
    struct WriteBack {
        PartBuf &shared, &mine;
        int64_t &rows_shared, &rows_mine;
        ~WriteBack() { shared = mine; rows_shared = rows_mine; }
    } write_back{out_shared, out, n_rows_shared, n_rows};
    const mc_format_args *a = J.a;
    const mc_calls_view *rec = a->rec;
    const mc_table_view *t = a->table;
    const int k = a->k;
    out.used = 0;
    RowCursor cur = start;
    int32_t cseg = -1;
    int64_t j = j0;
    for (; j < j1; ++j) {
        const uint32_t info = rec->info[j];
        const int64_t row = cur.row(j, info);
        if (info & MC_I_TOO_MANY) continue;
        if (std::isnan(rec->prob[row])) break;
        const int32_t seg = rec->site_seg[j];
        const int32_t rid = t->seg_read[seg];
        const int64_t crow = close_row_of(rec, j);
        if (cseg < 0 || crow < t->seg_row_begin[cseg] || (cseg < t->n_seg && crow >= t->seg_row_begin[cseg + 1])) {
            if (cseg >= 0 && cseg + 1 < t->n_seg && crow >= t->seg_row_begin[cseg + 1] && crow < t->seg_row_begin[cseg + 2]) ++cseg;
            else cseg = seg_of_row(t, crow);
        }
        const char *chrom;
        size_t chrom_len;
        if (cseg >= t->n_seg) { chrom = a->tail_chrom; chrom_len = J.tail_len; }
        else { const int32_t cc = t->seg_contig[cseg]; chrom = a->contig_names[cc]; chrom_len = J.contig_len_txt[(size_t)cc]; }
        const size_t need = chrom_len + J.name_len[(size_t)rid] + J.qual_len[(size_t)rid] + (size_t)k * 32 + 160;
        out.need(need);
        char *o = out.p + out.used;
        o = put_str(o, chrom, chrom_len); *o++ = '\t';
        o = put_str(o, a->read_names[rid], J.name_len[(size_t)rid]); *o++ = '\t';
        o = put_int(o, rec->site_pos[j]); *o++ = '\t';
        if (!build_context(a, j, o)) break;
        o += 2 * k - 1;
        *o++ = '\t';
        const uint32_t empty = info & MC_I_EMPTY_MASK;
        double f[MC_MAX_K];
        int32_t d[MC_MAX_K];
        const unsigned as_int = cur.feats_for_print(row, k, f, d);
        for (int i = 0; i < k; ++i) {
            if ((empty >> i) & 1u) *o++ = '0';
            else if ((as_int >> i) & 1u) o = put_fixed4(o, d[i]);
            else o = put_repr(o, f[i]);
            *o++ = ',';
        }
        o = put_str(o, a->read_qual_txt[rid], J.qual_len[(size_t)rid]); *o++ = '\t';
        *o++ = (info & MC_I_REV) ? '-' : '+'; *o++ = '\t';
        const double p1 = rec->prob[row];
        if (p1 >= 0.5) o = put_str(o, a->label_meth, J.lab_pos_len);
        else o = put_str(o, a->label_unmeth, J.lab_neg_len);
        *o++ = '\t';
        const double h = std::nearbyint(p1 * 100.0);
        if (h >= 0.0 && h <= 100.0) {
            const int hi = (int)h;
            if (hi == 100) { memcpy(o, "1.0", 3); o += 3; }
            else { *o++ = '0'; *o++ = '.'; *o++ = (char)('0' + hi / 10); if (hi % 10) *o++ = (char)('0' + hi % 10); }
        } else o = put_repr(o, h / 100.0);
        *o++ = '\n';
        out.used = (size_t)(o - out.p);
        ++n_rows;
    }
    return j;
}

}

extern "C" int mc_format_diffs(const mc_format_args *a, int64_t first, int32_t n_threads, char **text, int64_t *n_bytes,
                               int64_t *n_rows, int64_t *stop_at) {
    *text = nullptr;
    *n_bytes = 0;
    *n_rows = 0;
    *stop_at = first;
    if (!a || !a->rec || !a->table || !a->ref || a->k < 1 || a->k > MC_MAX_K || first < 0 || first > a->n_records) {
        mc_set_error("mc_format_diffs: bad arguments");
        return -12;
    }
    const int64_t n = a->n_records;
    const int threads = n_threads > 0 ? n_threads : mc_host_cores();
    const int nt = (int)std::min<int64_t>(threads > 1 ? 4 * (int64_t)threads : 1, std::max<int64_t>(1, (n - first) / 2048));

    Job J;
    J.a = a;
    const mc_table_view *t = a->table;
    J.name_len.resize((size_t)std::max(t->n_reads, 0));
    J.qual_len.resize((size_t)std::max(t->n_reads, 0));
    for (int32_t i = 0; i < t->n_reads; ++i) {
        J.name_len[(size_t)i] = a->read_names[i] ? strlen(a->read_names[i]) : 0;
        J.qual_len[(size_t)i] = a->read_qual_txt[i] ? strlen(a->read_qual_txt[i]) : 0;
    }
    J.contig_len_txt.resize((size_t)std::max(a->ref->n_contigs, 0));
    for (int32_t i = 0; i < a->ref->n_contigs; ++i) J.contig_len_txt[(size_t)i] = strlen(a->contig_names[i]);
    J.tail_len = a->tail_chrom ? strlen(a->tail_chrom) : 0;
    J.lab_pos_len = strlen(a->label_meth);
    J.lab_neg_len = strlen(a->label_unmeth);
    std::lock_guard<std::mutex> own_the_pieces(g_fmt_mu);
    if (g_parts.size() < (size_t)nt) g_parts.resize((size_t)nt);
    std::vector<PartBuf> &parts = g_parts;
    std::vector<int64_t> rows((size_t)nt, 0), stops((size_t)nt, n);
    std::vector<int> failed((size_t)nt, 0);
    static const bool fmt_timing = getenv("MCALLER_FMT_TIMING") != nullptr;
    std::vector<double> t_piece((size_t)nt, 0.0);
    auto piece_lo = [&](int w) { return first + (n - first) * w / nt; };
    const mc_calls_view *rec0 = a->rec;
    const bool counted = rec0->compacted && !rec0->call_row;
    std::vector<int64_t> kept0((size_t)nt + 1, 0), wide0((size_t)nt + 1, 0);
    if (counted) {
        kept0[0] = kept_in(rec0, 0, first);
        mc_parallel_for(nt, [&](int w) { kept0[(size_t)w + 1] = kept_in(rec0, piece_lo(w), piece_lo(w + 1)); });
        for (int w = 0; w < nt; ++w) kept0[(size_t)w + 1] += kept0[(size_t)w];
        if (!rec0->feats && rec0->feats_wide) {
            wide0[0] = wide_before(rec0, kept0[0]);
            mc_parallel_for(nt, [&](int w) {
                int64_t c = 0;
                for (int64_t r = kept0[(size_t)w], e = kept0[(size_t)w + 1]; r < e; ++r) c += __builtin_popcount(rec0->feats_wide[r]);
                wide0[(size_t)w + 1] = c;
            });
            for (int w = 0; w < nt; ++w) wide0[(size_t)w + 1] += wide0[(size_t)w];
        }
    }
    auto work = [&](int w) {
        const int64_t lo = piece_lo(w), hi = piece_lo(w + 1);
        const RowCursor start = counted ? RowCursor(rec0, kept0[(size_t)w], wide0[(size_t)w]) : RowCursor(rec0, lo);
        const auto t_a = std::chrono::steady_clock::now();
        try {
            stops[(size_t)w] = format_range(J, lo, hi, parts[(size_t)w], rows[(size_t)w], start);
        } catch (const std::bad_alloc &) { failed[(size_t)w] = 1; }
        if (fmt_timing) t_piece[(size_t)w] = std::chrono::duration<double>(std::chrono::steady_clock::now() - t_a).count();
    };
    const auto t_0 = std::chrono::steady_clock::now();
    mc_parallel_for(nt, work);
    if (fmt_timing) {
        fprintf(stderr, "[mc_format_diffs] %d pieces in %.2f ms:", nt, std::chrono::duration<double>(std::chrono::steady_clock::now() - t_0).count() * 1e3);
        for (int w = 0; w < nt; ++w) fprintf(stderr, " %.2f", t_piece[(size_t)w] * 1e3);
        fprintf(stderr, "\n");
    }
    for (int w = 0; w < nt; ++w)
        if (failed[(size_t)w]) { mc_set_error("mc_format_diffs: out of memory"); return -10; }
    int64_t stop = n;
    int last = nt;
    for (int w = 0; w < nt; ++w)
        if (stops[(size_t)w] < piece_lo(w + 1)) { stop = stops[(size_t)w]; last = w + 1; break; }
    *stop_at = stop;
    size_t total = 0;
    std::vector<size_t> at((size_t)last + 1, 0);
    for (int w = 0; w < last; ++w) { at[(size_t)w] = total; total += parts[(size_t)w].used; }
    char *outp = out_alloc(std::max<size_t>(total, 1));
    if (!outp) {
        mc_set_error("mc_format_diffs: out of memory (%zu bytes)", total);
        return -10;
    }
    mc_parallel_for(last, [&](int w) { memcpy(outp + at[(size_t)w], parts[(size_t)w].p, parts[(size_t)w].used); });
    for (int w = 0; w < last; ++w) *n_rows += rows[(size_t)w];
    *text = outp;
    *n_bytes = (int64_t)total;
    return 0;
}

extern "C" int mc_count_records(const mc_calls_view *rec, int64_t n, const int32_t *seg_read, int64_t n_seg, int64_t *counts3,
                                int32_t *ascending, uint8_t *pos_marks, int64_t n_marks, int64_t *pos_min, int64_t *pos_top) {
    if (!rec || n < 0 || (n > 0 && (!rec->info || !rec->site_pos || !rec->site_seg)) || (counts3 && !seg_read)) {
        mc_set_error("mc_count_records: bad arguments");
        return -12;
    }
    int64_t too = 0, wskips = 0, multi = 0, lo_pos = INT64_MAX, top = 0;
    bool asc = true;
    int64_t prev_key = INT64_MIN;
    for (int64_t j = 0; j < n; ++j) {
        const uint32_t info = rec->info[j];
        const int32_t pos = rec->site_pos[j];
        const bool is_too = (info & MC_I_TOO_MANY) != 0;
        if (counts3) {
            const int32_t seg = rec->site_seg[j];
            if (seg < 0 || seg >= n_seg) { mc_set_error("mc_count_records: record %lld names segment %d of %lld", (long long)j, seg, (long long)n_seg); return -12; }
            const int64_t key = ((int64_t)seg_read[seg] << 32) | (int64_t)(uint32_t)pos;
            asc = asc && key > prev_key;
            prev_key = key;
            too += is_too;
            wskips += !is_too && (info & MC_I_EMPTY_MASK) != 0;
            multi += (info & MC_I_MULTI) != 0;
        }
        if (!is_too) {
            lo_pos = std::min<int64_t>(lo_pos, pos);
            top = std::max<int64_t>(top, (int64_t)pos + 1);
            if (pos_marks && pos >= 0 && pos < n_marks) pos_marks[pos] = 1;
        }
    }
    if (counts3) { counts3[0] = too; counts3[1] = wskips; counts3[2] = multi; }
    if (ascending) *ascending = asc ? 1 : 0;
    if (pos_min) *pos_min = lo_pos == INT64_MAX ? 0 : lo_pos;
    if (pos_top) *pos_top = top;
    return 0;
}

extern "C" int mc_calls_expand(const mc_calls_view *rec, int64_t n, int32_t k, int32_t *call_row_out, int64_t *close_row_out,
                               double *feats_out) {
    if (!rec || n < 0 || (n > 0 && !rec->info) || (close_row_out && n > 0 && !rec->close_row && !rec->close_row32) ||
        (feats_out && (k < 1 || k > MC_MAX_K || (!rec->feats && !(rec->feats_lo32 && rec->feats_wide))))) {
        mc_set_error("mc_calls_expand: bad arguments");
        return -12;
    }
    const int nt = (int)std::max<int64_t>(1, std::min<int64_t>(mc_host_cores(), n / 16384));
    auto piece = [&](int w, int64_t &lo, int64_t &hi) { lo = n * w / nt; hi = n * (w + 1) / nt; };
    const bool count_rows = rec->compacted && !rec->call_row && (call_row_out || feats_out);
    std::vector<int64_t> kept((size_t)nt + 1, 0), wide((size_t)nt + 1, 0);
    if (count_rows)
        mc_parallel_for(nt, [&](int w) { int64_t lo, hi; piece(w, lo, hi); kept[(size_t)w + 1] = kept_in(rec, lo, hi); });
    for (int w = 0; w < nt; ++w) kept[(size_t)w + 1] += kept[(size_t)w];
    const bool packed = feats_out && !rec->feats;
    auto first_row = [&](int w) -> int64_t {
        if (!rec->compacted) { int64_t lo, hi; piece(std::min(w, nt - 1), lo, hi); return w >= nt ? n : lo; }
        if (rec->call_row) {
            if (w >= nt) return rec->n_call_rows;
            int64_t lo, hi; piece(w, lo, hi);
            for (int64_t j = lo; j < n; ++j) if (rec->call_row[j] >= 0) return rec->call_row[j];
            return rec->n_call_rows;
        }
        return kept[(size_t)w];
    };
    if (packed) {
        mc_parallel_for(nt, [&](int w) {
            int64_t c = 0;
            for (int64_t r = first_row(w), e = first_row(w + 1); r < e; ++r) c += __builtin_popcount(rec->feats_wide[r]);
            wide[(size_t)w + 1] = c;
        });
        for (int w = 0; w < nt; ++w) wide[(size_t)w + 1] += wide[(size_t)w];
    }
    mc_parallel_for(nt, [&](int w) {
        int64_t lo, hi;
        piece(w, lo, hi);
        if (close_row_out)
            for (int64_t j = lo; j < hi; ++j) close_row_out[j] = close_row_of(rec, j);
        if (call_row_out) {
            int64_t row = kept[(size_t)w];
            for (int64_t j = lo; j < hi; ++j) {
                if (!rec->compacted) call_row_out[j] = (int32_t)j;
                else if (rec->call_row) call_row_out[j] = rec->call_row[j];
                else call_row_out[j] = (rec->info[j] & MC_I_TOO_MANY) ? -1 : (int32_t)row++;
            }
        }
        if (feats_out) {
            const int64_t r0 = first_row(w), r1 = first_row(w + 1);
            if (rec->feats) {
                if (r1 > r0) memcpy(feats_out + r0 * k, rec->feats + r0 * k, (size_t)(r1 - r0) * (size_t)k * sizeof(double));
            } else {
                RowCursor cur(rec, lo);
                cur.wide = wide[(size_t)w];
                cur.wide_known = true;
                for (int64_t r = r0; r < r1; ++r) cur.feats(r, k, feats_out + r * k);
            }
        }
    });
    return 0;
}

extern "C" void mc_free(void *p) {
    if (p && !out_release(p)) free(p);
}

extern "C" int mc_repr_fixed4(int32_t d, char *out32) {
    char *e = put_fixed4(out32, d);
    *e = 0;
    return (int)(e - out32);
}

extern "C" int mc_repr_double_rowtext(double v, char *out32) {
    RtStore w{out32};
    uint64_t lo;
    uint32_t meta;
    rt_num_pack(rt_num_of(v), &lo, &meta);
    const RtNum n = rt_num_unpack(lo, meta);
    if (!n.ok) { out32[0] = 0; return -1; }
    rt_put_num(w, n);
    *w.p = 0;
    if ((int)(w.p - out32) != rt_num_length(n)) { out32[0] = 0; return -2; }
    return (int)(w.p - out32);
}

extern "C" int mc_repr_double(double v, char *out32) {
    char *e = put_repr(out32, v);
    *e = 0;
    return (int)(e - out32);
}

extern "C" int mc_parse_double(const char *s, int32_t n, double *out) {
    if (!s || !out || n < 0) return 0;
    return dc_parse(s, n, out);
}

extern "C" int mc_tstat(double n, double mean, double var, double *t, double *log10_p) {
    if (!t || !log10_p) return -12;
    return ts_stat(n, mean, var, t, log10_p);
}
extern "C" double mc_tstat_round3(double v) { return ts_round3(v); }
extern "C" int mc_tstat_tie(double v, double err) { return ts_tie(v, err) ? 1 : 0; }
extern "C" int mc_tstat_site(const double *X, int64_t n_rows, int32_t n_cols, double *out2) {
    if (!X || !out2 || n_rows < 1 || n_cols < 2) return -12;
    TsSite site;
    if (n_rows < 2) site.flags = TS_BAD_N;
    for (int32_t j = 0; j + 1 < n_cols && n_rows >= 2; ++j) {
        TsSum sum, sq;
        double sum_abs = 0.0;
        for (int64_t i = 0; i < n_rows; ++i) { sum.add(X[i * n_cols + j]); sum_abs += fabs(X[i * n_cols + j]); }
// ... 146 lines not shown
```

mcaller_amd/csrc/mc_scan.hip:

```cpp
#include "mc_dev.h"

namespace {

__global__ __launch_bounds__(256) void k_unit_columns(DevTable T) {
    const int64_t g4 = blockIdx.x * (int64_t)256 + threadIdx.x;
    const bool have = g4 * 4 < T.n_rows;
    int4 p = make_int4(0, 0, 0, 0);
    if (have) {
        p = *reinterpret_cast<const int4 *>(T.pos + g4 * 4);
        reinterpret_cast<int32_t *>(T.unit_pp)[g4] = (g4 & 1) ? p.w : p.x;
    }
    int before = __shfl_up(p.w, 1);
    if ((threadIdx.x & 63) == 0 && have && g4 > 0) before = T.pos[g4 * 4 - 1];
    const int ps[5] = {before, p.x, p.y, p.z, p.w};
    uint32_t dec = 0, zero = 0;
#pragma unroll
    for (int e = 0; e < 4; ++e) {
        const int64_t r = g4 * 4 + e;
        const bool in = r < T.n_rows;
        dec |= (in && r > 0 && ps[e + 1] < ps[e] ? 1u : 0u) << e;
        zero |= (in && ps[e + 1] == 0 ? 1u : 0u) << e;
    }
    const uint32_t mine = dec | (zero << 8);
    const uint32_t other = __shfl_down(mine, 1);
// ... 876 lines not shown
                        if (far) {
                            const RowRes fr = far_row(G, gbits, d.contig_len, nb_abs, d.row_end, c0 + i);
                            closed = fr.closed; m = fr.m; cp = fr.cp; cr = fr.cr; pf = fr.pf;
                        }
                    }
                    Payload P;
                    P.r = c0 + i; P.close_row = cr; P.m = m; P.close_pos = cp;
                    P.flags = pf | (d.stray_q != NO_STRAY ? PF_STRAY : 0u) | (d.rev ? PF_REV : 0u);
                    P.nb = nb_abs;
                    S.put(closed, P);
                }
            }
        }
        }
        if (CG <= 64 && has_c) {
            int nslow = 1;
            while (nb0 + 2 + nslow < T.n_nb && T.nb_row_begin[nb0 + 2 + nslow] < c1) ++nslow;
            scan_blocks_slowly(A, nb0 + 2, nslow, c0, c1, S, lane);
        }
        if (CG <= 64 && more) __syncthreads();
        if (CG > 64 && ch == 0) half = S.total;
    }
    if (lane == 0) A.tile_cnt[tile] = S.total;
    if (CG > 64 && lane == 0) A.tile_half[tile] = half;
}

__global__ __launch_bounds__(GROUP) void k1_group_scan(const int32_t *__restrict__ tile_cnt, int64_t n_tiles,
                                                       int32_t *__restrict__ tile_local, int64_t *__restrict__ group_sum) {
    MC_FRONT_OF_THE_QUEUE;
    __shared__ int s_w[GROUP / 64];
    const int tid = threadIdx.x, lane = tid & 63, wave = tid >> 6;
    const int64_t t = blockIdx.x * (int64_t)GROUP + tid;
    const int c = t < n_tiles ? tile_cnt[t] : 0;
    int incl = c;
    for (int o = 1; o < 64; o <<= 1) {
        const int v = __shfl_up(incl, o);
        if (lane >= o) incl += v;
    }
    if (lane == 63) s_w[wave] = incl;
    __syncthreads();
    int off = 0, total = 0;
    for (int w = 0; w < GROUP / 64; ++w) {
        if (w < wave) off += s_w[w];
        total += s_w[w];
    }
    if (t < n_tiles) tile_local[t] = off + incl - c;
    if (tid == 0) group_sum[blockIdx.x] = total;
}

__global__ __launch_bounds__(256) void k1_list(K1Args A, Payload *__restrict__ sorted, int gather) {
    MC_FRONT_OF_THE_QUEUE;
    const DevTable &T = A.T;
    if (A.chunk_cnt && blockIdx.x == 0)
        for (int i = threadIdx.x; i < PACK_WGS; i += blockDim.x) { A.chunk_cnt[PACK_PAD * i] = 0ull; A.chunk_cnt[PACK_PAD * i + 1] = 0ull; }
    constexpr int LG = 8;
    const int64_t tile = (blockIdx.x * (int64_t)blockDim.x + threadIdx.x) / LG;
    const int l = threadIdx.x & (LG - 1);
    const bool have = tile < T.n_tiles;
    const int64_t tl = have ? tile : T.n_tiles - 1;
    const int g = (int)(tl / GROUP);
    long long part = 0;
    for (int i = l; i < g; i += LG) part += A.group_sum[i];
#pragma unroll
    for (int o = LG / 2; o > 0; o >>= 1) part += __shfl_xor(part, o);
    if (!have) return;
    const int c = A.tile_cnt[tile];
    const int64_t first = part + A.tile_local[tile];
    if (tile == T.n_tiles - 1 && l == 0) A.cnt->n_records = (unsigned long long)(first + c);
    if (!gather && l == 0) A.tile_first[tile] = first;
    if (c == 0) return;
    if (first + c > A.O.capacity) { if (l == 0) atomicOr(&A.cnt->overflow, 1u); return; }
    if (!gather) {
        for (int ci = l; PT + (ci << A.chunk_shift) < c; ci += LG)
            if (A.tile_chunk[tile * NCHUNK + ci] < 0) atomicOr(&A.cnt->overflow, 1u);
        return;
    }
    for (int j = l; j < c; j += LG) {
        long long slot = tile * PT + j;
        if (j >= PT) {
            const long long cb = A.tile_chunk[tile * NCHUNK + ((j - PT) >> A.chunk_shift)];
            if (cb < 0) { atomicOr(&A.cnt->overflow, 1u); continue; }
            slot = cb + ((j - PT) & ((1 << A.chunk_shift) - 1));
        }
        sorted[first + j] = A.payload[slot];
    }
}


}

void mc_launch_unit_columns(const DevTable &T, hipStream_t st) {
    hipLaunchKernelGGL(k_unit_columns, dim3((unsigned)((T.n_rows / 4 + 256) / 256)), dim3(256), 0, st, T);
}

void mc_launch_scan(const K1Args &A, bool dense, int scan_mode, hipStream_t st) {
    const dim3 grid((unsigned)A.T.n_tiles);
    constexpr int CG_DENSE = CHUNK / 8 + 2;
    if (dense) {
        if (scan_mode == SCAN_VALIDATE) hipLaunchKernelGGL((k1_scan<CG_DENSE, SCAN_VALIDATE>), grid, dim3(64), 0, st, A);
        else hipLaunchKernelGGL((k1_scan<CG_DENSE, SCAN_STREAM>), grid, dim3(64), 0, st, A);
    } else {
        if (scan_mode == SCAN_VALIDATE) hipLaunchKernelGGL((k1_scan<64, SCAN_VALIDATE>), grid, dim3(64), 0, st, A);
        else if (scan_mode == SCAN_VALIDATE_SUMMARY) hipLaunchKernelGGL((k1_scan<64, SCAN_VALIDATE_SUMMARY>), grid, dim3(64), 0, st, A);
        else if (scan_mode == SCAN_STREAM) hipLaunchKernelGGL((k1_scan<64, SCAN_STREAM>), grid, dim3(64), 0, st, A);
        else hipLaunchKernelGGL((k1_scan<64, SCAN_SUMMARY>), grid, dim3(64), 0, st, A);
    }
}
// ... 11 lines not shown
```

mcaller_amd/csrc/mc_stream.hip:

```cpp
#include "mc_ctx.h"

static int ensure_pinned(mc_ctx *c, int64_t n, int k) {
    if (c->H.capacity >= n && c->h_k == k) return 0;
    c->H = DevRecords();
    const int64_t cap = std::max<int64_t>(n + n / 4, 1 << 16);
    const size_t bytes[6] = {(size_t)cap * k * 8, (size_t)cap * 4, (size_t)cap * 4, (size_t)cap * 8, (size_t)cap * 4, (size_t)cap * 8};
    for (int i = 0; i < 6; ++i)
        if (int rc = c->H_pin[i].alloc(bytes[i])) return rc;
    c->H.feats = c->H_pin[0].get<double>(); c->H.site_pos = c->H_pin[1].get<int32_t>(); c->H.site_seg = c->H_pin[2].get<int32_t>();
    c->H.close_row = c->H_pin[3].get<int64_t>(); c->H.info = c->H_pin[4].get<uint32_t>(); c->H.prob = c->H_pin[5].get<double>();
    c->H.capacity = cap;
    c->h_k = k;
    return 0;
}

static int copy_out_features(mc_ctx *c, int64_t n, int k, hipStream_t st) {
    HIP_TRY(hipMemcpyAsync(c->H.feats, c->O.feats, (size_t)n * k * 8, hipMemcpyDeviceToHost, st));
    HIP_TRY(hipMemcpyAsync(c->H.site_pos, c->O.site_pos, (size_t)n * 4, hipMemcpyDeviceToHost, st));
    HIP_TRY(hipMemcpyAsync(c->H.site_seg, c->O.site_seg, (size_t)n * 4, hipMemcpyDeviceToHost, st));
    HIP_TRY(hipMemcpyAsync(c->H.close_row, c->O.close_row, (size_t)n * 8, hipMemcpyDeviceToHost, st));
    HIP_TRY(hipMemcpyAsync(c->H.info, c->O.info, (size_t)n * 4, hipMemcpyDeviceToHost, st));
    return 0;
}

// ... 265 lines not shown
        if (prm->score && n > 0)
            launch_classifier(c, c->stream, c->O.feats, k, c->O.site_seg, T.seg_read, c->qual, c->O.info, (const uint8_t *)nullptr, n,
                              c->O.prob, (const unsigned long long *)nullptr, (const unsigned int *)nullptr);
        HIP_TRY(hipEventRecord(c->ev[4], c->stream));
        if (n > 0) {
            if (!early) { if (int rc = copy_out_features(c, n, k, c->stream)) return rc; }
            HIP_TRY(hipMemcpyAsync(c->H.prob, c->O.prob, (size_t)n * 8, hipMemcpyDeviceToHost, c->stream));
        }
        HIP_TRY(hipStreamSynchronize(c->stream));
        HIP_TRY(hipStreamSynchronize(c->copy_stream));
        HIP_TRY(hipGetLastError());
        for (int i = 0; i < 4; ++i) HIP_TRY(hipEventElapsedTime(&c->times[i], c->ev[i], c->ev[i + 1]));
        HIP_TRY(hipEventElapsedTime(&c->times[4], c->ev[0], c->ev[4]));
        c->last_n = n;
        c->last_slots = n;
        *n_records = n;
        return 0;
    }
    mc_set_error("record buffer overflow after 4 attempts");
    return -13;
}

extern "C" int mc_fetch_records(mc_ctx *c, const mc_calls_view *out) {
    HIP_TRY(hipSetDevice(c->device));
    const int64_t n = c->last_n;
    const int k = c->last_k;
    if (out->capacity < n) {
        mc_set_error("mc_fetch_records: capacity %lld < %lld records", (long long)out->capacity, (long long)n);
        return -12;
    }
    if (n == 0) return 0;
    memcpy(out->feats, c->H.feats, (size_t)n * k * 8);
    memcpy(out->site_pos, c->H.site_pos, (size_t)n * 4);
    memcpy(out->site_seg, c->H.site_seg, (size_t)n * 4);
    memcpy(out->close_row, c->H.close_row, (size_t)n * 8);
    memcpy(out->info, c->H.info, (size_t)n * 4);
    memcpy(out->prob, c->H.prob, (size_t)n * 8);
    return 0;
}

extern "C" int mc_fetch_records_view(mc_ctx *c, mc_calls_view *out) {
    out->capacity = c->last_n;
    out->feats = c->H.feats;
    out->site_pos = c->H.site_pos;
    out->site_seg = c->H.site_seg;
    out->close_row = c->H.close_row;
    out->info = c->H.info;
    out->prob = c->H.prob;
    out->call_row = nullptr;
    out->n_call_rows = 0;
    out->close_row32 = nullptr;
    out->compacted = 0;
    out->feats_lo32 = nullptr; out->feats_hi32 = nullptr; out->feats_wide = nullptr; out->n_wide = 0;
    return 0;
}

static int ensure_async_buf(mc_ctx *c, AsyncBuf &b, int64_t cap, int k, int64_t pack_rec = 0) {
    const DevTable &T = c->T;
    if (!b.ev[EV_DONE]) {
        for (int i = 0; i < EV_N; ++i)
            if (int rc = b.ev[i].create(i < EV_DONE ? hipEventDisableSystemFence : hipEventDefault)) return rc;
    }
    if (b.n_nb < T.n_nb) {
        if (b.used) HIP_TRY(hipEventSynchronize(b.ev[EV_DONE]));
        b.k0_allocs.clear();
        const int64_t nb = std::max<int64_t>(T.n_nb + T.n_nb / 4 + 64, c->scratch_nb);
        if (b.k0_allocs.get(&b.B.K.desc, (size_t)nb + 1) || b.k0_allocs.get(&b.B.K.nb_f0, (size_t)nb + 1)) return -10;
        b.n_nb = nb;
    }
    if (pack_rec <= 0 || pack_rec > cap) pack_rec = cap;
    const size_t pack_bytes = std::max((size_t)pack_rec * (20 + ((size_t)k + 1) * 8 + 1) + 128, c->pack_min_bytes);
    if (b.cap >= cap && b.k == k && b.pack_bytes >= pack_bytes) return 0;
    if (b.used) HIP_TRY(hipEventSynchronize(b.ev[EV_DONE]));
    b.dev_allocs.clear();
    b.H = DevRecords();
    if (alloc_records(b.dev_allocs, b.B.O, cap, k)) return -10;
    if (b.dev_allocs.get(&b.B.cnt, 1)) return -10;
    HIP_TRY(hipMemsetAsync(b.B.cnt, 0, sizeof(Counters), c->stream));
    if (cap >= (int64_t)1 << 31) {
        mc_set_error("mc_extract_features_async: %lld flush records per pass (call rows are 32 bits wide); use mc_extract_features",
                     (long long)cap);
        return -12;
    }
    if (b.dev_allocs.get(&b.pack, pack_bytes) || b.dev_allocs.get(&b.chunk_cnt, (size_t)PACK_PAD * PACK_WGS)) return -10;
    if (b.dev_allocs.get(&b.B.sorted, (size_t)cap) || b.dev_allocs.get(&b.B.rare, (size_t)cap)) return -10;
    b.piece_cap = cap / 16 + 64;
    if (b.dev_allocs.get(&b.piece_cnt, (size_t)b.piece_cap) || b.dev_allocs.get(&b.piece_kw, (size_t)b.piece_cap)) return -10;
    if (b.pack_host.alloc(pack_bytes)) return -10;
    b.pack_bytes = pack_bytes;
    b.H.capacity = cap;
    if (!b.st.p) { if (b.st.alloc(sizeof(Counters))) return -10; }
    b.cap = cap;
    b.k = k;
    b.used = false;
    return 0;
}

static int enqueue_k2(mc_ctx *c, AsyncBuf &b, const K1Args &A) {
    const DevTable &T = c->T;
    hipStream_t st = c->side_stream;
    HIP_TRY(hipStreamWaitEvent(st, b.ev[EV_EMIT_END], 0));
    mc_launch_rare_dev(A, b.B.sorted, b.B.rare, st);
    if (b.timed || !MC_EVENTS_ON_KERNELS) HIP_TRY(hipEventRecord(b.ev[EV_K2_START], st));
    if (b.prm.score)
        launch_classifier(c, st, b.B.O.feats, b.k, b.B.O.site_seg, T.seg_read, c->qual, b.B.O.info, (const uint8_t *)nullptr, b.cap, b.B.O.prob,
                          (const unsigned long long *)&b.B.cnt->n_records, (const unsigned int *)&b.B.cnt->overflow,
                          b.fused_room > 0 ? b.piece_cnt : nullptr, b.fused_room, b.fused_room > 0 ? b.slots / b.fused_room : 0);
    if (b.timed || !MC_EVENTS_ON_KERNELS) HIP_TRY(hipEventRecord(b.ev[EV_K2_END], st));
    return 0;
}

static int enqueue_side(mc_ctx *c, AsyncBuf &b, const K1Args &A, bool *done) {
    const DevTable &T = c->T;
    hipStream_t st = c->side_stream;
    *done = false;
    const bool other = c->clf.kind != Classifier::MLP && c->clf.kind != Classifier::NONE;
    if (b.prm.score && c->clf.kind != Classifier::MLP) return 0;
    HIP_TRY(hipStreamWaitEvent(st, b.ev[EV_EMIT_END], 0));
    if (b.timed || !MC_EVENTS_ON_KERNELS) HIP_TRY(hipEventRecord(b.ev[EV_K2_START], st));
    if (!mc_launch_side(c->clf.M, other, c->n_cu, st, A, b.B.sorted, T.seg_read, c->qual, b.cap, b.prm.score ? 1 : 0, b.pack, b.pack_bytes, b.close32 ? 1 : 0, (Counters *)b.st.dev,
                        b.fused_room, b.fused_room > 0 ? b.slots / b.fused_room : 0, MC_EVENTS_ON_KERNELS ? b.ev[EV_DONE] : nullptr))
        return 0;
    if (!MC_EVENTS_ON_KERNELS) HIP_TRY(hipEventRecord(b.ev[EV_DONE], st));
    HIP_TRY(hipGetLastError());
    *done = true;
    return 0;
}

static int enqueue_pack(mc_ctx *c, AsyncBuf &b, bool count) {
    hipStream_t s2 = c->side_stream;
    const int holes = b.fused_room > 0 ? 1 : 0;
    if (count) mc_launch_pack_count(b.B.O, b.B.cnt, b.k, b.chunk_cnt, holes, s2);
    mc_launch_pack(b.B.O, b.B.cnt, b.chunk_cnt, b.pack, b.pack_bytes, b.k, b.close32 ? 1 : 0, (Counters *)b.st.dev, holes, count ? 1 : 0, s2, MC_EVENTS_ON_KERNELS ? b.ev[EV_DONE] : nullptr);
    if (!MC_EVENTS_ON_KERNELS) HIP_TRY(hipEventRecord(b.ev[EV_DONE], s2));
    HIP_TRY(hipGetLastError());
    return 0;
}

extern "C" int mc_extract_features_async(mc_ctx *c, const mc_params *prm) {
    HIP_TRY(hipSetDevice(c->device));
    if (int rc = check_pass(c, prm)) return rc;
    if (c->ab_count >= MC_PASSES_IN_FLIGHT) {
        mc_set_error("mc_extract_features_async: %d passes are in flight; call mc_wait_records first", MC_PASSES_IN_FLIGHT);
        return -12;
    }
    const DevTable &T = c->T;
    const int k = prm->k;
    AsyncBuf &b = c->ab[c->ab_head];
    b.prm = *prm;
    if (T.n_rows == 0 || T.n_nb == 0) {
        if (int rc = ensure_async_buf(c, b, 1 << 16, k)) return rc;
        memset(b.st.p, 0, sizeof(Counters));
        b.B.pass_no = ++c->pass_counter;
        b.used = false;
        b.want_text = 0; b.text_block = -1;
        b.fused_room = 0; b.slots = 0;
        b.slot = -1;
        c->ab_head = (c->ab_head + 1) % MC_PASSES_IN_FLIGHT;
        c->ab_count += 1;
        return 0;
    }
    int64_t cap = std::max<int64_t>(guess_capacity(c), c->sync.O.capacity);
    const bool fused_wanted = !(getenv("MCALLER_DENSE_FUSED") && atoi(getenv("MCALLER_DENSE_FUSED")) == 0);
    int fused_room = 0;
    if (fused_wanted && dense_reference(c)) {
        const double density = (double)c->R.n_sites / (2.0 * (double)c->ref_total_len);
        if (const char *e = getenv("MCALLER_FUSED_ROOM")) fused_room = std::max(1, atoi(e));
        else fused_room = (int)std::min<int64_t>(mc_fused_room_max(), (int64_t)mc_fused_room(density) * c->fused_scale);
        cap = std::max<int64_t>(cap, mc_fused_pieces(T) * fused_room);
    }
    b.fused_room = fused_room;
    b.slots = fused_room > 0 ? mc_fused_pieces(T) * fused_room : 0;
    if (int rc = mc_ensure_scratch(c, T.n_nb, T.n_tiles)) return rc;
    if (int rc = ensure_records(c, cap, k)) return rc;
    int64_t pack_rec = fused_room > 0 ? std::min<int64_t>(cap, std::max<int64_t>(guess_capacity(c), c->sync.O.capacity)) : cap;
    if (const char *e = getenv("MCALLER_PACK_RECORDS")) { if (atoll(e) > 0) pack_rec = std::min<int64_t>(cap, atoll(e)); }
    if (int rc = ensure_async_buf(c, b, cap, k, pack_rec)) return rc;
    if (fused_room > 0 && mc_fused_pieces(T) > b.piece_cap) { b.fused_room = 0; b.slots = 0; }
    for (auto &other : c->ab)
        if (!other.used && (other.cap < cap || other.n_nb < T.n_nb || other.pack_bytes < b.pack_bytes)) { if (int rc = ensure_async_buf(c, other, cap, k, pack_rec)) return rc; }
    hipStream_t st = c->stream;
    if (!c->side_stream) { if (int rc = c->side_stream.create()) return rc; }
    b.timed = c->timing_every > 0 && (c->pass_seq++ % c->timing_every) == 0;
    const PassPlan plan = plan_pass(c);
    if (b.timed) HIP_TRY(hipEventRecord(b.ev[EV_K0_START], st));
    b.st.get<Counters>()->side_done = ST_UNPUBLISHED;
    b.B.pass_no = ++c->pass_counter;
    if (int rc = enqueue_k0(c, prm, b.B, plan, &b)) return rc;
    if (b.timed) HIP_TRY(hipEventRecord(b.ev[EV_SCAN_START], st));
    K1Args A;
    if (int rc = enqueue_k1(c, prm, b.B, plan, &b, &A)) return rc;
    b.emit_aside = !dense_reference(c);
    b.close32 = T.n_rows < INT32_MAX;
    b.want_text = c->rt.on;
    b.text_block = -1;
    b.one_kernel = false;
    if (int rc = enqueue_side(c, b, A, &b.one_kernel)) return rc;
    if (!b.one_kernel) {
        if (int rc = enqueue_k2(c, b, A)) return rc;
        if (int rc = enqueue_pack(c, b, A.chunk_cnt == nullptr)) return rc;
    }
    HIP_TRY(hipGetLastError());
    b.used = true;
    b.slot = c->cur;
    b.qual = c->qual;
    b.n_qual = c->n_qual;
    if (b.slot >= 0) c->slots[b.slot].refs += 1;
    c->ab_head = (c->ab_head + 1) % MC_PASSES_IN_FLIGHT;
    c->ab_count += 1;
    return 0;
}

int mc_sync_pass_streams(mc_ctx *c) {
    if (c->up_stream) HIP_TRY(hipStreamSynchronize(c->up_stream));
    if (c->parse_stream) HIP_TRY(hipStreamSynchronize(c->parse_stream));
    if (c->side_stream) HIP_TRY(hipStreamSynchronize(c->side_stream));
    HIP_TRY(hipStreamSynchronize(c->stream));
    HIP_TRY(hipStreamSynchronize(c->copy_stream));
    HIP_TRY(hipStreamSynchronize(c->copy_stream2));
    return 0;
}

extern "C" int mc_wait_records_begin(mc_ctx *c) {
    HIP_TRY(hipSetDevice(c->device));
    if (c->ab_count == 0) {
        mc_set_error("mc_wait_records_begin: no pass in flight");
        return -12;
    }
    int at = c->ab_tail, left = c->ab_count;
    while (left > 0 && c->ab[at].copying) { at = (at + 1) % MC_PASSES_IN_FLIGHT; --left; }
    if (left == 0) return 0;
    AsyncBuf &b = c->ab[at];
    hipStream_t cs = (at & 1) ? c->copy_stream2 : c->copy_stream;
    if (b.used) {
        HIP_TRY(hipEventSynchronize(b.ev[EV_DONE]));
        HIP_TRY(hipStreamWaitEvent(cs, b.ev[EV_DONE], 0));
    }
    const Counters &st = *b.st.get<Counters>();
    unsigned char *pack_host = b.pack_host.get<unsigned char>();
    if (b.used && st.side_done == ST_UNPUBLISHED) {
        mc_set_error("mc_wait_records_begin: pass %llu did not publish its counters", (unsigned long long)b.B.pass_no);
        return -12;
    }
    const bool special = st.overflow || st.irregular_pass == b.B.pass_no;
    if (b.used && !special && st.n_records > 0) {
        const size_t n = (size_t)std::min<int64_t>((int64_t)st.n_records, b.cap);
        const int k = b.k;
        const size_t m = (size_t)std::min<unsigned long long>(st.n_kept, n);
        const PackLayout L = pack_layout((int64_t)n, b.close32 ? 1 : 0);
        const size_t n_wide = (size_t)std::min<unsigned long long>(st.n_wide, (unsigned long long)m * (size_t)k);
        const PackTail PT_ = pack_tail(L.feats, m, k, n_wide);
        const size_t out_bytes = PT_.end;
        if (out_bytes > b.pack_bytes) {
            mc_set_error("mc_wait_records_begin: pass %llu counts %zu bytes of records, its packed block holds %zu",
                         (unsigned long long)b.B.pass_no, out_bytes, b.pack_bytes);
            return -12;
        }
        static const size_t by_kernel_env = getenv("MCALLER_RECORDS_BY_KERNEL_MAX") ? (size_t)atoll(getenv("MCALLER_RECORDS_BY_KERNEL_MAX")) : 0;
        bool text_on_the_link = false;
        for (const TableSlot &S : c->slots) text_on_the_link = text_on_the_link || S.kp_state == 1;
        const size_t by_kernel_max = by_kernel_env ? by_kernel_env : (text_on_the_link ? COPY_BY_KERNEL_MAX_STREAMING : COPY_BY_KERNEL_MAX);
        if (out_bytes <= by_kernel_max && c->side_stream) {
            cs = c->side_stream;
            if (int rc = mc_copy_by_kernel(pack_host, b.pack, out_bytes, cs)) return rc;
        } else HIP_TRY(hipMemcpyAsync(pack_host, b.pack, out_bytes, hipMemcpyDeviceToHost, cs));
        b.H.close_row = b.close32 ? nullptr : reinterpret_cast<int64_t *>(pack_host);
        b.h_close32 = b.close32 ? reinterpret_cast<int32_t *>(pack_host) : nullptr;
        b.H.site_pos = reinterpret_cast<int32_t *>(pack_host + L.pos);
        b.H.site_seg = reinterpret_cast<int32_t *>(pack_host + L.seg);
        b.H.info = reinterpret_cast<uint32_t *>(pack_host + L.info);
        b.H.feats = nullptr;
        b.h_lo32 = reinterpret_cast<int32_t *>(pack_host + PT_.lo32);
        b.H.prob = reinterpret_cast<double *>(pack_host + PT_.prob);
        b.h_wmask = pack_host + PT_.wmask;
        b.h_hi32 = reinterpret_cast<uint32_t *>(pack_host + PT_.hi32);
        b.h_n_wide = (int64_t)n_wide;
        b.h_n_calls = (int64_t)m;
        HIP_TRY(hipEventRecord(b.ev[EV_COPIED], cs));
        b.text_block = -1;
        if (b.want_text) { if (int rc = mc_enqueue_row_text(c, b, (int64_t)n, (int64_t)m, (int64_t)n_wide)) return rc; }
    }
    b.copying = true;
    return 0;
}

extern "C" int mc_wait_records(mc_ctx *c, int64_t *n_records, mc_calls_view *out) {
    HIP_TRY(hipSetDevice(c->device));
    if (c->ab_count == 0) {
        mc_set_error("mc_wait_records: no pass in flight");
        return -12;
    }
    if (!c->ab[c->ab_tail].copying) { if (int rc = mc_wait_records_begin(c)) return rc; }
    AsyncBuf &b = c->ab[c->ab_tail];
    c->ab_tail = (c->ab_tail + 1) % MC_PASSES_IN_FLIGHT;
    c->ab_count -= 1;
    b.copying = false;
    if (b.slot >= 0) {
        c->slots[b.slot].refs -= 1;
        c->held = b.slot;
        c->last_T = c->slots[b.slot].T;
    }
    const Counters st = *b.st.get<Counters>();
    const bool special = st.overflow || st.irregular_pass == b.B.pass_no;
    if (b.used && !special && st.n_records > 0) HIP_TRY(hipEventSynchronize(b.ev[EV_COPIED]));
    c->rt.last_block = -1; c->rt.last_bytes = c->rt.last_rows = 0;
    if (b.text_block >= 0) {
        auto &blk = c->rt.blocks[b.text_block];
        HIP_TRY(hipEventSynchronize(b.ev[EV_TEXT]));
        const RowTextStatus ts = *blk.st.get<RowTextStatus>();
        if (ts.too_small && st.n_kept > 0)
            c->rt.bytes_per_row = std::max(c->rt.bytes_per_row, 1.25 * (double)ts.n_bytes / (double)st.n_kept + 8.0);
        c->rt.n_host_needed += ts.host_needed ? 1 : 0;
        if (ts.host_needed && getenv("MCALLER_VERBOSE")) fprintf(stderr, "mcaller_hip: a pass's rows left to the host formatter (reasons 0x%x)\n", ts.host_needed);
        c->rt.n_too_small += ts.too_small ? 1 : 0;
        if (special || ts.host_needed || ts.too_small || ts.n_bytes > blk.cap) blk.busy.store(0);
        else { c->rt.n_text += 1; c->rt.last_block = b.text_block; c->rt.last_bytes = (int64_t)ts.n_bytes; c->rt.last_rows = (int64_t)ts.n_rows; }
        b.text_block = -1;
    }
    if (special && getenv("MCALLER_VERBOSE"))
        fprintf(stderr, "mcaller_hip: pass re-run synchronously (overflow %u, irregular %u, big %u, rare %u, records %llu)\n",
                st.overflow, (unsigned)(st.irregular_pass == b.B.pass_no), st.n_big, st.n_rare, st.n_records);
    c->last_fused_room = b.used ? b.fused_room : 0;
    c->last_rerun = special ? 1 : 0;
    if (special && st.overflow && st.pack_need > 0)
        c->pack_min_bytes = std::max(c->pack_min_bytes, (size_t)st.pack_need + (size_t)st.pack_need / 4);
    else if (special && st.overflow && b.fused_room > 0 && b.fused_room < mc_fused_room_max())
        c->fused_scale = std::min(c->fused_scale * 2, 64);
    if (special) {
        int64_t n = 0;
        const DevTable T_now = c->T;
        const double *q_now = c->qual;
        const int cur_now = c->cur, nq_now = c->n_qual;
        if (b.slot >= 0) { c->T = c->slots[b.slot].T; c->qual = const_cast<double *>(b.qual); c->n_qual = b.n_qual; c->cur = b.slot; }
        c->in_rerun = true;
        const int rc = mc_extract_features(c, &b.prm, &n);
        c->in_rerun = false;
        c->T = T_now; c->qual = const_cast<double *>(q_now); c->n_qual = nq_now; c->cur = cur_now;
        if (rc) return rc;
        c->last_timed = 1;
        *n_records = n;
        return mc_fetch_records_view(c, out);
    }
    const int64_t n = (int64_t)st.n_records;
    c->last_timed = (b.used && b.timed) ? 1 : 0;
    if (b.used && b.timed) {
        float t_k0 = 0, t_scan = 0, t_emit = 0, t_k2 = 0;
        HIP_TRY(hipEventElapsedTime(&t_k0, b.ev[EV_K0_START], b.ev[EV_SCAN_START]));
        if (b.emit_aside && MC_EVENTS_ON_KERNELS) {
            HIP_TRY(hipEventElapsedTime(&t_scan, b.ev[EV_SCAN_START], b.ev[EV_LIST_END]));
            HIP_TRY(hipEventElapsedTime(&t_emit, b.ev[EV_EMIT_START], b.ev[EV_EMIT_END]));
        } else {
            HIP_TRY(hipEventElapsedTime(&t_scan, b.ev[EV_SCAN_START], b.ev[EV_EMIT_END]));
            t_emit = 0.0f;
        }
        HIP_TRY(hipEventElapsedTime(&t_k2, b.ev[EV_K2_START], b.one_kernel ? b.ev[EV_DONE] : b.ev[EV_K2_END]));
        c->times[0] = t_k0; c->times[1] = t_scan; c->times[2] = t_emit; c->times[3] = t_k2;
        c->times[4] = t_k0 + t_scan + t_emit + t_k2;
    }
    c->O = b.B.O;
    c->last_n = n;
    c->last_slots = b.fused_room > 0 ? std::min<int64_t>(b.slots, b.cap) : n;
    c->last_k = b.k ? b.k : c->last_k;
    *n_records = n;
    out->capacity = n;
    out->feats = b.H.feats; out->site_pos = b.H.site_pos; out->site_seg = b.H.site_seg;
    out->close_row = b.H.close_row; out->info = b.H.info; out->prob = b.H.prob;
    out->close_row32 = b.h_close32;
    out->call_row = nullptr;
    out->compacted = 1;
    const bool packed = n > 0 && b.used;
    out->feats_lo32 = packed ? b.h_lo32 : nullptr;
    out->feats_hi32 = packed ? b.h_hi32 : nullptr;
    out->feats_wide = packed ? b.h_wmask : nullptr;
    out->n_wide = packed ? b.h_n_wide : 0;
    out->n_call_rows = n > 0 && b.used ? b.h_n_calls : 0;
    return 0;
}

extern "C" int mc_last_pass_info(mc_ctx *c, int32_t *fused_room, int32_t *rerun) {
    if (fused_room) *fused_room = c->last_fused_room;
    if (rerun) *rerun = c->last_rerun;
    return 0;
}

extern "C" int mc_ctx_last_scan_mode(mc_ctx *c) { return c->last_scan_mode; }

extern "C" int64_t mc_ctx_whole_tiles(mc_ctx *c, uint8_t *per_tile) {
    HIP_TRY(hipSetDevice(c->device));
    const DevTable &T = c->T;
    if (c->cur < 0 || !c->sync.K.desc || T.n_nb <= 0 || T.n_nb > c->scratch_nb || T.n_tiles <= 0) {
        mc_set_error("mc_ctx_whole_tiles: no table, or no synchronous pass over it yet");
        return -12;
    }
    HIP_TRY(hipStreamSynchronize(c->stream));
    std::vector<NbDesc> desc((size_t)T.n_nb);
    std::vector<int32_t> tile_nb((size_t)T.n_tiles);
    HIP_TRY(hipMemcpy(desc.data(), c->sync.K.desc, desc.size() * sizeof(NbDesc), hipMemcpyDeviceToHost));
    HIP_TRY(hipMemcpy(tile_nb.data(), T.tile_nb, tile_nb.size() * sizeof(int32_t), hipMemcpyDeviceToHost));
    int64_t n = 0;
    for (int64_t tile = 0; tile < T.n_tiles; ++tile) {
        const int64_t t0 = tile * TILE;
        int nb = tile_nb[(size_t)tile];
        if (nb < 0 || nb >= T.n_nb) { mc_set_error("mc_ctx_whole_tiles: tile %lld begins in block %d", (long long)tile, nb); return -12; }
        while (nb + 1 < T.n_nb && desc[(size_t)nb].row_end <= t0) ++nb;
        const bool whole = scan_tile_is_whole(desc[(size_t)nb], t0, (int)(std::min<int64_t>(t0 + TILE, T.n_rows) - t0));
        if (per_tile) per_tile[tile] = whole ? 1 : 0;
        n += whole;
    }
    return n;
}

extern "C" int mc_ctx_set_pass_timing(mc_ctx *c, int every_n) {
    if (every_n < 0) { mc_set_error("mc_ctx_set_pass_timing: every_n < 0"); return -12; }
    c->timing_every = every_n;
    return 0;
}

extern "C" int mc_last_pass_timed(mc_ctx *c) { return c->last_timed; }

extern "C" int mc_last_times_ms(mc_ctx *c, float *out5) {
    for (int i = 0; i < 5; ++i) out5[i] = c->times[i];
    return 0;
}

static int classifier_forward(mc_ctx *c, int which, const double *X, const uint8_t *submodel, int64_t n, double *p) {
    HIP_TRY(hipSetDevice(c->device));
    if (which != c->clf.kind) {
        mc_set_error("classifier forward: no %s set", which == 1 ? "forest" : (which == 2 ? "logistic / naive Bayes model" : (which == 3 ? "SVM" : "MLP")));
// ... 194 lines not shown
```

mcaller_amd/rows.py:

```python
import numpy as np

from . import _lib
from .device import get_device
from .refmark import MarkedReference, revcomp, strand

_I = _lib


def base_models(base, twobase=False):
    if base == 'A' and twobase:
        return {'MG': 'MG', 'MC': 'MH', 'MA': 'MH', 'MT': 'MH', 'MM': 'MH', 'MH': 'MH', 'AT': 'MH', 'AC': 'MH',
                'AG': 'MG', 'AA': 'MH', 'AM': 'MH'}
    base_model = {'M' + nextb: 'general' for nextb in ['A', 'C', 'G', 'T', 'M']}
    base_model.update({'A' + nextb: 'general' for nextb in ['A', 'C', 'G', 'T', 'M']})
    base_model.update({'T' + nextb: 'general' for nextb in ['A', 'C', 'G', 'T', 'M']})
    return base_model


def writefi(data, fi):
    with open(fi, 'a') as outfi:
        for entry in data:
            outfi.write('\t'.join(entry) + '\n')


# ... 90 lines not shown
        if not train:
            self.table, _, self.model_index, self.soc = submodel_setup(modelset, base)
            self.model_keys = modelset.keys()
        else:
            self.table = base_models(base, False)
            self.model_keys = None
        self.signals = {bm: {} for bm in self.table.values()} if train else None
        self.contexts = {bm: {} for bm in self.table.values()} if train else None
        self.stdout = None
        self.host_scored = {}
        self.blobs = []
        self.num_observations = 0
        self.pos_set, self.multi, self.w_skips, self.skipped = set(), set(), set(), set()
        self._n_pos = self._n_multi = self._n_wskips = self._n_skipped = self._kept_pos = None

    def write_to(self, sink):
        n = 0
        for b in self.blobs:
            if len(b):
                n += len(b)
                sink(b.view if isinstance(b, (_lib.LibBuffer, _lib.RowText)) else b)
            if isinstance(b, _lib.RowText):
                b.release()
        return n

    def text(self, max_rows=None):
        blob = b''.join(b.view if isinstance(b, (_lib.LibBuffer, _lib.RowText)) else b for b in self.blobs)
        if max_rows is None:
            return blob
        return b''.join(blob.splitlines(True)[:max_rows])

    @property
    def rows(self):
        return [line.split('\t') for line in self.text().decode('utf-8', 'surrogateescape').splitlines()]

    def counters(self):
        if self._n_pos is None and self._kept_pos is None and getattr(self, '_counted_natively', False):
            n = self._rec.n
            self._kept_pos = self._site_pos[:n][(self._info[:n] & _I.I_TOO_MANY) == 0]
        if self._n_pos is None and self._kept_pos is not None:
            self._n_pos = len(distinct_positions(self._kept_pos))
        n_pos = len(self.pos_set) if self._n_pos is None else self._n_pos
        n_multi = len(self.multi) if self._n_multi is None else self._n_multi
        n_wskips = len(self.w_skips) if self._n_wskips is None else self._n_wskips
        n_skipped = len(self.skipped) if self._n_skipped is None else self._n_skipped
        return ['thread finished processing...:', '%d observations' % self.num_observations,
                '%d positions' % n_pos, '%d regions with multiple methylated bases' % n_multi,
                '%d observations with skips included' % n_wskips,
                '%d observations with too many skips' % n_skipped]

    def _bind(self, rec):
        n = rec.n
        self._rec = rec
        self._info = rec.info[:n]
        self._site_pos = rec.site_pos[:n]
        self._seg_of = rec.site_seg[:n]
        self._lazy = None

    def _per_record(self):
        if self._lazy is None:
            rec, k, t, n = self._rec, self.k, self.P.table, self._rec.n
            m = rec.n_calls
            feats = rec.feats[:m * k].reshape(m, k)
            row = rec.call_row[:n] if rec.call_row is not None else None
            close_seg = np.searchsorted(t.seg_row_begin, rec.close_row[:n], side='right') - 1
            self._lazy = (feats, row, close_seg)
        return self._lazy

    def run(self, rec):
        self._bind(rec)
        n = rec.n
        if self.train or n == 0:
            for j in range(n):
                stop = self._one(j)
                if stop is not None:
                    return stop
            return None
        P, t = self.P, self.P.table
        text = getattr(rec, 'row_text', None)
        if text is not None:
            self.blobs.append(text)
            self.num_observations += text.n_rows
            self._count(n)
            return None
        label_meth = 'm6A' if self.base == 'A' else 'm' + self.base
        fmt = _lib.DiffsFormatter(rec, t, P.ref.device_arrays(), P.ref.names, [str(q) for q in P.qual_obj], self.k,
                                  label_meth, self.base, self.soc, tail_chrom=self.tail_chrom)
        first, done_to, stop_exc = 0, n, None
        while first < n:
            blob, n_rows, stop = fmt.rows(first, n_threads=FORMAT_THREADS[0])
            self.blobs.append(blob)
            self.num_observations += n_rows
            if stop >= n:
                break
            stop_exc = self._one(stop)
            if stop_exc is not None:
                done_to = stop
                break
            first = stop + 1
        self._count(done_to)
        return stop_exc

    def host_prob(self, rec):
        r = rec.by_record()
        p = np.array(r.prob[:r.n], dtype=np.float64)
        for j, v in self.host_scored.items():
            p[j] = v
        return p

    def _count(self, n):
# ... 56 lines not shown
                        p1 = rec.prob[row]
                        want = (inf >> _I.I_NEXT_SHIFT) & 0xFF
                        if (inf & _I.I_EDGE) or np.isnan(p1):
                            dev = self.device if self.device is not None else get_device()
                            p1 = dev.mlp_forward(np.array([diffs + [float(qual)]], dtype=np.float64),
                                                 np.array([mi], dtype=np.uint8))[0]
                            self.host_scored[j] = float(p1)
                        elif len(context) > half + 1 and ord(context[half + 1]) != want:
                            raise AssertionError('device and host disagree on the sub-model of %s' % line)
                        if p1 >= 0.5:
                            label = 'm6A' if self.base == 'A' else 'm' + self.base
                        else:
                            label = self.base
                        label = label + '\t' + fmt_float(round2(p1))
                    else:
                        label = self.pos_label[(chrom, mpos, strand(rev))]
                        self.signals[twobase_model].setdefault(label, []).append(diffs + [qual])
                        self.contexts[twobase_model].setdefault(label, []).append(context)
                    row = [chrom, read, str(mpos), context, diffs_txt, strand(rev), label]
                    self.blobs.append(('\t'.join(row) + '\n').encode('utf-8', 'surrogateescape'))
                except (IndexError, KeyError) as e:
                    print(line, '- Index or Key Error', file=self.stdout)
                    print(list(self.model_keys or []), list(self.table.keys()), context[centre:centre + 2], file=self.stdout)
                    print(e, file=self.stdout)
                    return SystemExit(0)
            else:
                print(line, file=self.stdout)
                return SystemExit(0)
            self.num_observations += 1
            self.pos_set.add(mpos)
        if inf & _I.I_MULTI:
            self.multi.add((read, mpos))
        return None


def distinct_positions(pos):
    pos = np.asarray(pos)
    if len(pos) == 0:
        return np.zeros(0, dtype=np.int32)
    lo, hi = int(pos.min()), int(pos.max())
    if lo < 0 or hi - lo > (1 << 28):
        return np.unique(pos)
    seen = np.zeros(hi - lo + 1, dtype=bool)
    seen[pos - lo] = True
    return (np.flatnonzero(seen) + lo).astype(pos.dtype, copy=False)


def cut_names(table, rec):
    names, seg_read = table.read_names, table.seg_read
    n = int(rec.n)
    if n == 0:
        every = set(names[int(r)] for r in seg_read)
        return every, every, False
    first_seg, last_seg = int(rec.site_seg[0]), int(rec.site_seg[n - 1])
    return (set(names[int(r)] for r in seg_read[:first_seg + 1]), set(names[int(r)] for r in seg_read[last_seg:]), True)


FORMAT_THREADS = [int(__import__('os').environ.get('MCALLER_FORMAT_THREADS', '0'))]


def head_contig(P, qual_thresh):
    t = P.table
    for seg in range(t.n_seg):
        if P.qual[t.seg_read[seg]] < qual_thresh:
            continue
        r0, r1 = int(t.seg_row_begin[seg]), int(t.seg_row_begin[seg + 1])
        if ((t.flags[r0:r1] & _lib.F_MODEL_N) == 0).any():
            return int(t.seg_contig[seg])
    return None
```

Baseline: 869.0 million calls/s.

## Pack per-record columns as 16-bit lows plus run table to shrink copy-out

Adds a narrow record layout in which close_row, site_pos and info are written as 16-bit low halves plus a byte. A run table keeps the segment and high bits whenever they change, so the device-to-host copy per pass shrinks from about 16 bytes per record to about 7. The host widens columns lazily through a new native expand function only when Python code touches them. In exchange it adds a ballot/popcount run-rank computation in K2, extra shared-memory reductions, and a fallback flag for records that do not fit. Widening on the host may still cost time if consumers read the columns every pass.

Result: faster. 941.6 million calls/s, median of 6 (+8.4%).

```diff
diff --git a/include/mcaller_hip.h b/include/mcaller_hip.h
--- a/include/mcaller_hip.h
+++ b/include/mcaller_hip.h
@@ -67,6 +67,13 @@
     const uint32_t *feats_hi32;
     const uint8_t *feats_wide;
     int64_t n_wide;
+    const uint16_t *close_lo16;
+    const uint16_t *pos_lo16;
+    const uint16_t *info_lo16;
+    const uint8_t *info_next;
+    const int32_t *runs;
+    int64_t n_runs;
+    int64_t copy_out_bytes;
 } mc_calls_view;
 
 const char *mc_last_error(void);
@@ -315,6 +322,8 @@
                      uint8_t *pos_marks, int64_t n_marks, int64_t *pos_min, int64_t *pos_top);
 int mc_calls_expand(const mc_calls_view *rec, int64_t n_records, int32_t k, int32_t *call_row_out, int64_t *close_row_out,
                     double *feats_out);
+int mc_records_expand(const mc_calls_view *rec, int64_t n_records, int32_t *site_pos_out, int32_t *site_seg_out, uint32_t *info_out,
+                      int64_t *close_row_out);
 void mc_free(void *p);
 int mc_repr_double(double v, char *out32);
 int mc_repr_fixed4(int32_t d, char *out32);
diff --git a/mcaller_amd/_lib.py b/mcaller_amd/_lib.py
--- a/mcaller_amd/_lib.py
+++ b/mcaller_amd/_lib.py
@@ -673,14 +673,23 @@
     def view(self):
         v = CallsView()
         v.capacity = self.capacity
-        v.site_pos, v.site_seg = _ptr(self.site_pos), _ptr(self.site_seg)
-        v.info, v.prob = _ptr(self.info), _ptr(self.prob)
+        v.prob = _ptr(self.prob)
+        v.copy_out_bytes = int(self.copy_out_bytes)
+        narrow = self._narrow is not None and self._site_pos is None
+        if narrow:
+            close_lo, pos_lo, info_lo, info_next, runs = self._narrow
+            v.close_lo16, v.pos_lo16, v.info_lo16, v.info_next = _ptr(close_lo), _ptr(pos_lo), _ptr(info_lo), _ptr(info_next)
+            v.runs, v.n_runs = _ptr(runs), len(runs) // 4
+        else:
+            v.site_pos, v.site_seg, v.info = _ptr(self.site_pos), _ptr(self.site_seg), _ptr(self.info)
         if self._feats is None and self._packed is not None:
             lo, hi, wide = self._packed
             v.feats_lo32, v.feats_hi32, v.feats_wide, v.n_wide = _ptr(lo), _ptr(hi), _ptr(wide), len(hi)
         else:
             v.feats = _ptr(self.feats)
-        if self._close_row is not None or self._close_row32 is None:
+        if narrow:
+            pass
+        elif self._close_row is not None or self._close_row32 is None:
             v.close_row = _ptr(self.close_row)
         else:
             v.close_row32 = _ptr(self._close_row32)
@@ -696,13 +705,18 @@
         r.k, r.capacity, r.n, r._owner = k, n, n, owner
         if v.feats:
             r.feats = _from_ptr(v.feats, n * k, np.float64)
-        r.site_pos = _from_ptr(v.site_pos, n, np.int32)
-        r.site_seg = _from_ptr(v.site_seg, n, np.int32)
-        if v.close_row:
-            r._close_row = _from_ptr(v.close_row, n, np.int64)
+        r.copy_out_bytes = int(v.copy_out_bytes)
+        if v.close_lo16:
+            r._narrow = (_from_ptr(v.close_lo16, n, np.uint16), _from_ptr(v.pos_lo16, n, np.uint16), _from_ptr(v.info_lo16, n, np.uint16),
+                         _from_ptr(v.info_next, n, np.uint8), _from_ptr(v.runs, 4 * int(v.n_runs), np.int32))
         else:
-            r._close_row32 = _from_ptr(v.close_row32, n, np.int32)
-        r.info = _from_ptr(v.info, n, np.uint32)
+            r.site_pos = _from_ptr(v.site_pos, n, np.int32)
+            r.site_seg = _from_ptr(v.site_seg, n, np.int32)
+            if v.close_row:
+                r._close_row = _from_ptr(v.close_row, n, np.int64)
+            else:
+                r._close_row32 = _from_ptr(v.close_row32, n, np.int32)
+            r.info = _from_ptr(v.info, n, np.uint32)
         if v.compacted:
             m = int(v.n_call_rows)
             r._compacted = True
@@ -720,7 +734,54 @@
         return r
 
     _close_row = _close_row32 = _call_row = _feats = _packed = None
+    _site_pos = _site_seg = _info = _narrow = None
     _compacted = False
+    copy_out_bytes = 0
+
+    @property
+    def n_runs(self):
+        return len(self._narrow[4]) // 4 if self._narrow is not None else 0
+
+    def _widen(self):
+        if self._narrow is not None and self._site_pos is None:
+            n = max(1, int(self.n))
+            pos, seg, info, close = (np.empty(n, dtype=t) for t in (np.int32, np.int32, np.uint32, np.int64))
+            v = self.view()
+            check(lib().mc_records_expand(C.byref(v), int(self.n), _ptr(pos), _ptr(seg), _ptr(info), _ptr(close)))
+            self._site_seg, self._info, self._close_row, self._site_pos = seg, info, close, pos
+
+    def end_segments(self):
+        if self._narrow is not None and self._site_pos is None:
+            runs = self._narrow[4]
+            return int(runs[1]), int(runs[-3])
+        return int(self.site_seg[0]), int(self.site_seg[self.n - 1])
+
+    @property
+    def site_pos(self):
+        self._widen()
+        return self._site_pos
+
+    @site_pos.setter
+    def site_pos(self, a):
+        self._site_pos = a
+
+    @property
+    def site_seg(self):
+        self._widen()
+        return self._site_seg
+
+    @site_seg.setter
+    def site_seg(self, a):
+        self._site_seg = a
+
+    @property
+    def info(self):
+        self._widen()
+        return self._info
+
+    @info.setter
+    def info(self, a):
+        self._info = a
 
     @property
     def feats(self):
@@ -737,6 +798,7 @@
 
     @property
     def close_row(self):
+        self._widen()
         if self._close_row is None and self._close_row32 is not None:
             self._close_row = self._close_row32.astype(np.int64)
         return self._close_row
diff --git a/mcaller_amd/csrc/mc_classify.hip b/mcaller_amd/csrc/mc_classify.hip
--- a/mcaller_amd/csrc/mc_classify.hip
+++ b/mcaller_amd/csrc/mc_classify.hip
@@ -161,6 +161,7 @@
     size_t out_bytes;
     Counters *host_status;
     int close32, score;
+    int narrow;
 };
 struct NoPack {};
 #ifndef MC_SIDE_WAVES
@@ -200,7 +201,8 @@
     __shared__ uint32_t s_fixrow[(FAST && PACK) ? KFIX : 1];
     __shared__ int2 s_pk[PACK ? 2 : 1][PACK ? KW : 1];
     __shared__ unsigned long long s_base[PACK ? 2 : 1][4];
-    __shared__ unsigned long long s_red[PACK ? 6 : 1][PACK ? KW : 1];
+    __shared__ unsigned long long s_red[PACK ? 8 : 1][PACK ? KW : 1];
+    __shared__ unsigned long long s_runm[PACK ? 2 : 1][PACK ? KW : 1];
     __shared__ unsigned long long s_lay[PACK ? 8 : 1];
     const int tid = threadIdx.x, lane = tid & 63;
     const int wave = __builtin_amdgcn_readfirstlane(tid >> 6);
@@ -238,8 +240,11 @@
     const int64_t per = (n_units + gridDim.x - 1) / gridDim.x;
     int64_t lo = min(n_units, blockIdx.x * per), hi = min(n_units, lo + per);
     K2_WALL(1);
+    [[maybe_unused]] bool narrow_k = false;
     if constexpr (PACK) {
         unsigned long long v[6] = {0, 0, 0, 0, 0, 0};
+        unsigned long long vr = 0, vr_before = 0;
+        const bool narrow = SP.narrow && !pieces && SP.A.cnt->n_rare == 0;
         if (pieces) {
             for (int64_t j0 = 32 * (int64_t)tid; j0 < P.n; j0 += 32 * TH) {
                 int4 k4[8];
@@ -264,11 +269,16 @@
                 const unsigned long long kk = SP.A.chunk_cnt[PACK_PAD * j], ww = SP.A.chunk_cnt[PACK_PAD * j + 1];
                 v[0] += kk; v[1] += ww;
                 if (j < c0) { v[3] += kk; v[4] += ww; }
+                if (narrow) {
+                    const unsigned long long rr = SP.A.chunk_cnt[PACK_PAD * j + PACK_RUNS_LANE];
+                    vr += rr;
+                    if (j < c0) vr_before += rr;
+                }
             }
             if (tid == 0) { v[2] = (unsigned long long)n; v[5] = (unsigned long long)lo; }
         }
         K2_WALL(2);
-        if (tid < 6) s_red[PACK ? tid : 0][0] = 0ull;
+        if (tid < 8) s_red[PACK ? tid : 0][0] = 0ull;
         __syncthreads();
 #pragma unroll
         for (int i = 0; i < 6; ++i) {
@@ -277,21 +287,34 @@
             for (int o = 32; o > 0; o >>= 1) x += __shfl_xor(x, o);
             if (lane == 0 && x) atomicAdd(&s_red[PACK ? i : 0][0], x);
         }
+        if (narrow) {
+#pragma unroll
+            for (int o = 32; o > 0; o >>= 1) { vr += __shfl_xor(vr, o); vr_before += __shfl_xor(vr_before, o); }
+            if (lane == 0 && vr) atomicAdd(&s_red[PACK ? 6 : 0][0], vr);
+            if (lane == 0 && vr_before) atomicAdd(&s_red[PACK ? 7 : 0][0], vr_before);
+        }
         __syncthreads();
 #pragma unroll
         for (int i = 0; i < 6; ++i) v[i] = s_red[PACK ? i : 0][0];
-        __syncthreads();
-        const size_t need_bytes = pack_tail(pack_layout((int64_t)v[2], SP.close32).feats, (size_t)v[0], k, (size_t)v[1]).end;
+        vr = s_red[PACK ? 6 : 0][0]; vr_before = s_red[PACK ? 7 : 0][0];
+        __syncthreads();
+        const size_t feats_at = narrow ? narrow_layout((int64_t)v[2], (int64_t)vr).feats : pack_layout((int64_t)v[2], SP.close32).feats;
+        const size_t need_bytes = pack_tail(feats_at, (size_t)v[0], k, (size_t)v[1]).end;
         const bool too_big = need_bytes > SP.out_bytes;
         if (too_big) lo = hi;
+        narrow_k = narrow;
         if (tid == 0) {
             const PackLayout PL = pack_layout((int64_t)v[2], SP.close32);
-            const PackTail PTl = pack_tail(PL.feats, (size_t)v[0], k, (size_t)v[1]);
-            s_lay[0] = PL.pos; s_lay[1] = PL.seg; s_lay[2] = PL.info; s_lay[3] = PTl.lo32; s_lay[4] = PTl.wmask; s_lay[5] = PTl.hi32;
+            const NarrowLayout NL = narrow_layout((int64_t)v[2], (int64_t)vr);
+            const PackTail PTl = pack_tail(feats_at, (size_t)v[0], k, (size_t)v[1]);
+            s_lay[0] = narrow ? NL.pos_lo : PL.pos; s_lay[1] = narrow ? NL.info_lo : PL.seg; s_lay[2] = narrow ? NL.info_next : PL.info;
+            s_lay[3] = PTl.lo32; s_lay[4] = PTl.wmask; s_lay[5] = PTl.hi32;
             s_lay[6] = PTl.prob;
-            s_base[0][0] = v[3]; s_base[0][1] = v[4]; s_base[0][2] = v[5];
+            s_lay[7] = NL.runs;
+            s_base[0][0] = v[3]; s_base[0][1] = v[4]; s_base[0][2] = v[5]; s_base[0][3] = vr_before;
             s_red[0][1] = v[2]; s_red[1][1] = v[0]; s_red[2][1] = v[1];
             s_red[3][1] = need_bytes;
+            s_red[4][1] = narrow ? vr : 0ull;
         }
         __syncthreads();
         K2_WALL(3);
@@ -372,12 +395,24 @@
         int mi = 255;
         double qv = 0.0;
         [[maybe_unused]] int p_nw = -1;
+        [[maybe_unused]] bool p_run = false;
         if (tid < n_here) {
             if (submodel_in) mi = submodel_in[r];
             else {
                 const uint32_t inf = info[r];
                 const int32_t seg = site_seg[r];
+                [[maybe_unused]] int64_t key_c = 0, key_cp = 0;
+                [[maybe_unused]] int32_t key_p = 0, key_pp = 0, key_sp = 0;
+                if constexpr (PACK) {
+                    if (narrow_k) {
+                        const int64_t rp = r > 0 ? r - 1 : 0;
+                        key_c = SP.A.O.close_row[r]; key_cp = SP.A.O.close_row[rp];
+                        key_p = SP.A.O.site_pos[r]; key_pp = SP.A.O.site_pos[rp];
+                        key_sp = site_seg[rp];
+                    }
+                }
                 if constexpr (PACK) { if (!(inf & MC_I_TOO_MANY)) p_nw = __popc((uint32_t)SP.A.O.wmask[r] & ((1u << k) - 1u)); }
+                if constexpr (PACK) p_run = narrow_k && (r == 0 || record_starts_run(seg, key_c, key_p, key_sp, key_cp, key_pp));
                 bool scored = !(inf & (MC_I_TOO_MANY | MC_I_EDGE));
                 if constexpr (PACK) scored = scored && SP.score != 0;
                 if (scored) {
@@ -392,6 +427,8 @@
 #pragma unroll
             for (int o = 32; o > 0; o >>= 1) nw += __shfl_xor(nw, o);
             if (lane == 0) s_pk[PACK ? buf : 0][PACK ? wave : 0] = make_int2(nk, nw);
+            const unsigned long long rm = __ballot(p_run);
+            if (lane == 0) s_runm[PACK ? buf : 0][PACK ? wave : 0] = rm;
         }
         int rank = 0, cnt_lane = 0;
 #pragma unroll
@@ -533,8 +570,12 @@
         if constexpr (PACK) {
             K2_WALL(11);
             if (tid == 0) {
-                unsigned kept_s = 0, wide_s = 0;
-                for (int w = 0; w < KW; ++w) { const int2 c = s_pk[PACK ? buf : 0][PACK ? w : 0]; kept_s += (unsigned)c.x; wide_s += (unsigned)c.y; }
+                unsigned kept_s = 0, wide_s = 0, runs_s = 0;
+                for (int w = 0; w < KW; ++w) {
+                    const int2 c = s_pk[PACK ? buf : 0][PACK ? w : 0]; kept_s += (unsigned)c.x; wide_s += (unsigned)c.y;
+                    runs_s += (unsigned)__popcll(s_runm[PACK ? buf : 0][PACK ? w : 0]);
+                }
+                s_base[PACK ? buf ^ 1 : 0][3] = s_base[PACK ? buf : 0][3] + runs_s;
                 s_base[PACK ? buf ^ 1 : 0][0] = s_base[PACK ? buf : 0][0] + kept_s;
                 s_base[PACK ? buf ^ 1 : 0][1] = s_base[PACK ? buf : 0][1] + wide_s;
                 s_base[PACK ? buf ^ 1 : 0][2] = s_base[PACK ? buf : 0][2] + (unsigned long long)n_here;
@@ -565,11 +606,33 @@
                 const unsigned long long real0 = s_base[PACK ? buf : 0][2];
                 const int64_t io = pieces ? (int64_t)real0 + tid : r;
                 unsigned char *const out = SP.out;
+                if (narrow_k) {
+                    reinterpret_cast<uint16_t *>(out)[io] = (uint16_t)close;
+                    reinterpret_cast<uint16_t *>(out + s_lay[0])[io] = (uint16_t)pos;
+                    reinterpret_cast<uint16_t *>(out + s_lay[PACK ? 1 : 0])[io] = (uint16_t)inf;
+                    (out + s_lay[PACK ? 2 : 0])[io] = (uint8_t)(inf >> 16);
+                    const unsigned long long rm = s_runm[PACK ? buf : 0][PACK ? wave : 0];
+                    bool misfit = (inf >> 24) != 0u;
+                    if ((rm >> lane) & 1ull) {
+                        unsigned long long at = s_base[PACK ? buf : 0][3] + (unsigned)__popcll(rm & below);
+#pragma unroll
+                        for (int w = 0; w < KW; ++w)
+                            if (w < wave) at += (unsigned)__popcll(s_runm[PACK ? buf : 0][PACK ? w : 0]);
+                        if (at < s_red[PACK ? 4 : 0][PACK ? 1 : 0])
+                            reinterpret_cast<int4 *>(out + s_lay[PACK ? 7 : 0])[at] = make_int4((int)io, seg, (int)(close >> 16), pos >> 16);
+                        else misfit = true;
+                    }
+                    if (misfit) {
+                        const unsigned long long was = atomicExch(&SP.A.cnt->irregular_pass, SP.A.pass_no);
+                        asm volatile("" :: "v"(was));
+                    }
+                } else {
                 if (SP.close32) reinterpret_cast<int32_t *>(out)[io] = (int32_t)close;
                 else reinterpret_cast<int64_t *>(out)[io] = close;
                 reinterpret_cast<int32_t *>(out + s_lay[0])[io] = pos;
                 reinterpret_cast<int32_t *>(out + s_lay[PACK ? 1 : 0])[io] = seg;
                 reinterpret_cast<uint32_t *>(out + s_lay[PACK ? 2 : 0])[io] = inf;
+                }
                 if (keep) {
                     int32_t *o_lo = reinterpret_cast<int32_t *>(out + s_lay[PACK ? 3 : 0]) + row * k;
                     uint32_t *o_hi = reinterpret_cast<uint32_t *>(out + s_lay[PACK ? 5 : 0]);
@@ -622,7 +685,8 @@
             static_assert(sizeof(Counters::overflow) == 4 && sizeof(Counters::pack_need) == 8 && offsetof(Counters, pack_need) % 8 == 0, "Counters layout");
             const unsigned long long need_bytes = s_red[PACK ? 3 : 0][PACK ? 1 : 0];
             const bool too_big = need_bytes > SP.out_bytes;
-            if (tid < (int)head_words && (tid < kept_word || tid >= kept_word + 4) && tid >= 2) {
+            constexpr int runs_word = (int)(offsetof(Counters, n_runs) / 4);
+            if (tid < (int)head_words && (tid < kept_word || tid >= kept_word + 4) && tid >= 2 && tid != runs_word && tid != runs_word + 1) {
                 unsigned int w = __hip_atomic_load(reinterpret_cast<unsigned int *>(SP.A.cnt) + tid, __ATOMIC_RELAXED, __HIP_MEMORY_SCOPE_AGENT);
                 if (too_big && tid == overflow_word) w |= 1u;
                 if (too_big && (tid == need_word || tid == need_word + 1)) w = (unsigned int)(need_bytes >> (tid == need_word ? 0 : 32));
@@ -632,6 +696,7 @@
                 *reinterpret_cast<volatile unsigned long long *>(&SP.host_status->n_records) = s_red[0][PACK ? 1 : 0];
                 *reinterpret_cast<volatile unsigned long long *>(&SP.host_status->n_kept) = s_red[PACK ? 1 : 0][PACK ? 1 : 0];
                 *reinterpret_cast<volatile unsigned long long *>(&SP.host_status->n_wide) = s_red[PACK ? 2 : 0][PACK ? 1 : 0];
+                *reinterpret_cast<volatile unsigned long long *>(&SP.host_status->n_runs) = s_red[PACK ? 4 : 0][PACK ? 1 : 0];
             }
         }
     }
@@ -1071,7 +1136,6 @@
         rbase += r_strip;
     }
 }
-
 
 }
 
@@ -1136,7 +1200,7 @@
 
 bool mc_launch_side(const DevMlp &M, bool other_classifier, int n_cu, hipStream_t st, const K1Args &A, const Payload *sorted, const int32_t *seg_read,
                     const double *qual, int64_t cap, int score, unsigned char *out, size_t out_bytes, int close32, Counters *host_status,
-                    int piece_room, int64_t n_pieces, hipEvent_t stop) {
+                    int piece_room, int64_t n_pieces, hipEvent_t stop, int narrow) {
     static const bool off = getenv("MCALLER_SIDE_FUSED") && atoi(getenv("MCALLER_SIDE_FUSED")) == 0;
     if (off || cap <= 0) return false;
     if (score && (other_classifier || !M.W1)) return false;
@@ -1145,6 +1209,7 @@
     if (by_piece ? (piece_room >= TH_SIDE || !A.piece_kw || !A.piece_cnt) : !A.chunk_cnt) return false;
     SidePack SP;
     SP.A = A; SP.sorted = sorted; SP.out = out; SP.out_bytes = out_bytes; SP.host_status = host_status; SP.close32 = close32; SP.score = score;
+    SP.narrow = (narrow && !by_piece && close32) ? 1 : 0;
     const K2Pieces P{by_piece ? A.piece_cnt : nullptr, piece_room, n_pieces};
     const bool fast = score && M.fast && M.wp32;
     unsigned grid;
diff --git a/mcaller_amd/csrc/mc_ctx.h b/mcaller_amd/csrc/mc_ctx.h
--- a/mcaller_amd/csrc/mc_ctx.h
+++ b/mcaller_amd/csrc/mc_ctx.h
@@ -150,6 +150,12 @@
     int64_t h_n_wide = 0;
     int32_t *h_close32 = nullptr;
     bool close32 = false;
+    bool narrow = false;
+    const uint16_t *h_close_lo16 = nullptr, *h_pos_lo16 = nullptr, *h_info_lo16 = nullptr;
+    const uint8_t *h_info_next = nullptr;
+    const int32_t *h_runs = nullptr;
+    int64_t h_n_runs = 0;
+    int64_t h_copy_out_bytes = 0;
     int64_t h_n_calls = 0;
     Event ev[EV_N];
     mc_params prm;
diff --git a/mcaller_amd/csrc/mc_dev.h b/mcaller_amd/csrc/mc_dev.h
--- a/mcaller_amd/csrc/mc_dev.h
+++ b/mcaller_amd/csrc/mc_dev.h
@@ -152,8 +152,9 @@
     unsigned long long side_done;
     unsigned long long pack_need;
     unsigned long long irregular_pass;
+    unsigned long long n_runs;
     unsigned long long end_of_head;
-    unsigned long long pad_to_line[SHARD_PAD];
+    unsigned long long pad_to_line[SHARD_PAD - 1];
     unsigned long long shard[NSHARD * SHARD_PAD];
 };
 constexpr unsigned long long ST_UNPUBLISHED = ~0ull;
@@ -262,6 +263,7 @@
 constexpr int PACK_WGS = MC_PACK_WGS, PACK_THREADS = MC_PACK_THREADS;
 
 constexpr int PACK_PAD = 16;
+constexpr int PACK_RUNS_LANE = 3;
 
 __device__ __forceinline__ void count_for_packing(unsigned long long *chunk_cnt, int64_t q, int64_t n_rec, bool kept, int n_wide) {
     if (!chunk_cnt || !kept) return;
@@ -271,9 +273,15 @@
     if (n_wide) atomicAdd(&chunk_cnt[PACK_PAD * b + 1], (unsigned long long)n_wide);
 }
 
-__device__ __forceinline__ void count_wave_for_packing(unsigned long long *chunk_cnt, int64_t n_rec, bool kept, int64_t q, uint32_t wmask, int k) {
+__device__ __forceinline__ void count_wave_for_packing(unsigned long long *chunk_cnt, int64_t n_rec, bool kept, int64_t q, uint32_t wmask, int k, bool run_start) {
     if (!chunk_cnt) return;
     const unsigned long long km = __ballot(kept);
+    const unsigned long long sm = __ballot(run_start);
+    if (sm) {
+        uint32_t per_s = (uint32_t)((n_rec + PACK_WGS - 1) / PACK_WGS);
+        asm volatile("" : "+s"(per_s));
+        if (run_start) atomicAdd(&chunk_cnt[PACK_PAD * ((uint32_t)q / per_s) + PACK_RUNS_LANE], 1ull);
+    }
     if (!km) return;
     uint32_t per = (uint32_t)((n_rec + PACK_WGS - 1) / PACK_WGS);
     asm volatile("" : "+s"(per));
@@ -395,6 +403,23 @@
     L.info = L.seg + (size_t)n * 4;
     L.feats = (L.info + (size_t)n * 4 + 7) & ~(size_t)7;
     return L;
+}
+
+struct RecordRun { int32_t first_record, seg, close_hi, pos_hi; };
+static_assert(sizeof(RecordRun) == 16, "RecordRun layout");
+struct NarrowLayout { size_t close_lo, pos_lo, info_lo, info_next, runs, feats; };
+__host__ __device__ inline NarrowLayout narrow_layout(int64_t n, int64_t n_runs) {
+    NarrowLayout L;
+    L.close_lo = 0;
+    L.pos_lo = (size_t)n * 2;
+    L.info_lo = (size_t)n * 4;
+    L.info_next = (size_t)n * 6;
+    L.runs = ((size_t)n * 7 + 15) & ~(size_t)15;
+    L.feats = L.runs + (size_t)n_runs * sizeof(RecordRun);
+    return L;
+}
+__host__ __device__ inline bool record_starts_run(int32_t seg, int64_t close_row, int32_t pos, int32_t seg_p, int64_t close_row_p, int32_t pos_p) {
+    return seg != seg_p || (close_row >> 16) != (close_row_p >> 16) || (pos >> 16) != (pos_p >> 16);
 }
 
 struct PackTail { size_t lo32, prob, wmask, hi32, end; };
@@ -465,7 +490,7 @@
                     int close32, Counters *host_status, int holes, int look, hipStream_t st, hipEvent_t stop);
 bool mc_launch_side(const DevMlp &M, bool other_classifier, int n_cu, hipStream_t st, const K1Args &A, const Payload *sorted, const int32_t *seg_read,
                     const double *qual, int64_t cap, int score, unsigned char *out, size_t out_bytes, int close32, Counters *host_status,
-                    int piece_room, int64_t n_pieces, hipEvent_t stop);
+                    int piece_room, int64_t n_pieces, hipEvent_t stop, int narrow);
 
 struct KpSeg { long long row; long long name_off; int name_len; int contig; int name_start; int pad; };
 
diff --git a/mcaller_amd/csrc/mc_emit.hip b/mcaller_amd/csrc/mc_emit.hip
--- a/mcaller_amd/csrc/mc_emit.hip
+++ b/mcaller_amd/csrc/mc_emit.hip
@@ -82,6 +82,10 @@
     const int64_t r = P.r;
     const int m = P.m;
     const bool window = live && !(P.flags & PF_EXTRA);
+    const int64_t q_before = max(tw / EG - 1, (int64_t)0);
+    const int32_t nb_before = sorted[q_before].nb, m_before = sorted[q_before].m;
+    const int32_t ch_before = (int32_t)(sorted[q_before].close_row >> 16);
+    const int32_t seg_before = T.nb_seg_begin[nb_before];
     const NbDesc *dp = A.desc + P.nb;
     static_assert(offsetof(NbDesc, row_begin) == 0 && offsetof(NbDesc, mask_off) == 16 && offsetof(NbDesc, first_delta) == 24 && offsetof(NbDesc, contig_len) == 28,
                   "the descriptor's second 16 bytes: mask_off, first_delta, contig_len");
@@ -103,6 +107,13 @@
     asm volatile("" : "+v"(d_rb.x), "+v"(d_rb.y), "+v"(d_1.x), "+v"(d_1.y), "+v"(d_1.z), "+v"(d_1.w), "+v"(d_sdel),
                       "+v"(seg_of), "+v"(pj[0]), "+v"(pj[1]), "+v"(pj[2]), "+v"(pj[3]), "+v"(fj[0]), "+v"(fj[1]), "+v"(fj[2]), "+v"(fj[3]));
     EM_STAMP(1);
+    bool run_start;
+    {
+        const int32_t ch = (int32_t)(P.close_row >> 16);
+        int32_t seg_p = __shfl_up(seg_of, EG), m_p = __shfl_up(m, EG), ch_p = __shfl_up(ch, EG);
+        if (lane_now < EG) { seg_p = seg_before; m_p = m_before; ch_p = ch_before; }
+        run_start = live && s == 0 && (q == 0 || seg_of != seg_p || ch != ch_p || (m >> 16) != (m_p >> 16));
+    }
     const int64_t d_row_begin = ((int64_t)(uint32_t)d_rb.x) | ((int64_t)d_rb.y << 32), d_mask_off = ((int64_t)(uint32_t)d_1.x) | ((int64_t)d_1.y << 32);
     const int64_t d_first = d_1.z < 0 ? -1 : d_row_begin + d_1.z;
     const int64_t Lc = d_1.w;
@@ -269,7 +280,7 @@
         }
         A.O.info[q] = info_out;
     }
-    count_wave_for_packing(A.chunk_cnt, n_rec, kept_rec, q, wide_bit, k);
+    count_wave_for_packing(A.chunk_cnt, n_rec, kept_rec, q, wide_bit, k, run_start);
     EM_STAMP(5);
     ++em_round;
     }
diff --git a/mcaller_amd/csrc/mc_format.cpp b/mcaller_amd/csrc/mc_format.cpp
--- a/mcaller_amd/csrc/mc_format.cpp
+++ b/mcaller_amd/csrc/mc_format.cpp
@@ -181,17 +181,51 @@
     return (int32_t)(std::upper_bound(b, e, r) - b) - 1;
 }
 
-inline bool build_context(const mc_format_args *a, int64_t j, char *ctx) {
-    const mc_calls_view *rec = a->rec;
+inline uint32_t info_of(const mc_calls_view *rec, int64_t j) {
+    return rec->info_lo16 ? ((uint32_t)rec->info_lo16[j] | ((uint32_t)rec->info_next[j] << 16)) : rec->info[j];
+}
+struct RecCols {
+    const mc_calls_view *rec;
+    bool narrow;
+    int64_t run;
+    explicit RecCols(const mc_calls_view *r) : rec(r), narrow(r->close_lo16 != nullptr), run(0) {}
+    RecCols(const mc_calls_view *r, int64_t first) : RecCols(r) { seek(first); }
+    void seek(int64_t j) {
+        if (!narrow) return;
+        int64_t lo = 0, hi = rec->n_runs - 1;
+        while (lo < hi) {
+            const int64_t mid = (lo + hi + 1) >> 1;
+            if (rec->runs[4 * mid] <= j) lo = mid; else hi = mid - 1;
+        }
+        run = lo;
+    }
+    void to(int64_t j) {
+        if (narrow) while (run + 1 < rec->n_runs && rec->runs[4 * (run + 1)] <= j) ++run;
+    }
+    int32_t seg(int64_t j) const { return narrow ? rec->runs[4 * run + 1] : rec->site_seg[j]; }
+    int32_t pos(int64_t j) const { return narrow ? (int32_t)(((uint32_t)rec->runs[4 * run + 3] << 16) | rec->pos_lo16[j]) : rec->site_pos[j]; }
+    int64_t close(int64_t j) const {
+        if (narrow) return (int64_t)rec->runs[4 * run + 2] * 65536 + rec->close_lo16[j];
+        return rec->close_row ? rec->close_row[j] : (int64_t)rec->close_row32[j];
+    }
+};
+bool record_columns_ok(const mc_calls_view *rec, int64_t n) {
+    if (n <= 0) return true;
+    if (!rec->close_lo16) return rec->info && rec->site_pos && rec->site_seg && (rec->close_row || rec->close_row32);
+    if (!rec->pos_lo16 || !rec->info_lo16 || !rec->info_next || !rec->runs || rec->n_runs < 1 || rec->n_runs > n || rec->runs[0] != 0) return false;
+    for (int64_t r = 1; r < rec->n_runs; ++r)
+        if (rec->runs[4 * r] <= rec->runs[4 * (r - 1)] || rec->runs[4 * r] >= n) return false;
+    return true;
+}
+
+inline bool build_context(const mc_format_args *a, uint32_t info, int32_t seg, int32_t site_pos, char *ctx) {
     const mc_ref_view *ref = a->ref;
     const int k = a->k;
-    const uint32_t info = rec->info[j];
     if (info & MC_I_EDGE) return false;
-    const int32_t seg = rec->site_seg[j];
     if (seg < 0 || seg >= a->table->n_seg) return false;
     const int32_t cid = a->table->seg_contig[seg];
     if (cid < 0 || cid >= ref->n_contigs) return false;
-    const int64_t L = ref->contig_len[cid], m = rec->site_pos[j];
+    const int64_t L = ref->contig_len[cid], m = site_pos;
     const int64_t lo = m - k + 1, hi = m + k;
     if (lo < 0 || hi > L) return false;
     const bool rev = info & MC_I_REV;
@@ -215,13 +249,9 @@
     return true;
 }
 
-inline int64_t close_row_of(const mc_calls_view *rec, int64_t j) {
-    return rec->close_row ? rec->close_row[j] : (int64_t)rec->close_row32[j];
-}
-
 int64_t kept_in(const mc_calls_view *rec, int64_t lo, int64_t hi) {
     int64_t kept = 0;
-    for (int64_t j = lo; j < hi; ++j) kept += (rec->info[j] & MC_I_TOO_MANY) ? 0 : 1;
+    for (int64_t j = lo; j < hi; ++j) kept += (info_of(rec, j) & MC_I_TOO_MANY) ? 0 : 1;
     return kept;
 }
 
@@ -290,16 +320,18 @@
     const int k = a->k;
     out.used = 0;
     RowCursor cur = start;
+    RecCols cols(rec, j0);
     int32_t cseg = -1;
     int64_t j = j0;
     for (; j < j1; ++j) {
-        const uint32_t info = rec->info[j];
+        const uint32_t info = info_of(rec, j);
         const int64_t row = cur.row(j, info);
         if (info & MC_I_TOO_MANY) continue;
         if (std::isnan(rec->prob[row])) break;
-        const int32_t seg = rec->site_seg[j];
+        cols.to(j);
+        const int32_t seg = cols.seg(j);
         const int32_t rid = t->seg_read[seg];
-        const int64_t crow = close_row_of(rec, j);
+        const int64_t crow = cols.close(j);
         if (cseg < 0 || crow < t->seg_row_begin[cseg] || (cseg < t->n_seg && crow >= t->seg_row_begin[cseg + 1])) {
             if (cseg >= 0 && cseg + 1 < t->n_seg && crow >= t->seg_row_begin[cseg + 1] && crow < t->seg_row_begin[cseg + 2]) ++cseg;
             else cseg = seg_of_row(t, crow);
@@ -313,8 +345,9 @@
         char *o = out.p + out.used;
         o = put_str(o, chrom, chrom_len); *o++ = '\t';
         o = put_str(o, a->read_names[rid], J.name_len[(size_t)rid]); *o++ = '\t';
-        o = put_int(o, rec->site_pos[j]); *o++ = '\t';
-        if (!build_context(a, j, o)) break;
+        const int32_t site_pos = cols.pos(j);
+        o = put_int(o, site_pos); *o++ = '\t';
+        if (!build_context(a, info, seg, site_pos, o)) break;
         o += 2 * k - 1;
         *o++ = '\t';
         const uint32_t empty = info & MC_I_EMPTY_MASK;
@@ -354,7 +387,8 @@
     *n_bytes = 0;
     *n_rows = 0;
     *stop_at = first;
-    if (!a || !a->rec || !a->table || !a->ref || a->k < 1 || a->k > MC_MAX_K || first < 0 || first > a->n_records) {
+    if (!a || !a->rec || !a->table || !a->ref || a->k < 1 || a->k > MC_MAX_K || first < 0 || first > a->n_records ||
+        !record_columns_ok(a->rec, a->n_records)) {
         mc_set_error("mc_format_diffs: bad arguments");
         return -12;
     }
@@ -441,19 +475,22 @@
 
 extern "C" int mc_count_records(const mc_calls_view *rec, int64_t n, const int32_t *seg_read, int64_t n_seg, int64_t *counts3,
                                 int32_t *ascending, uint8_t *pos_marks, int64_t n_marks, int64_t *pos_min, int64_t *pos_top) {
-    if (!rec || n < 0 || (n > 0 && (!rec->info || !rec->site_pos || !rec->site_seg)) || (counts3 && !seg_read)) {
+    if (!rec || n < 0 || (counts3 && !seg_read) ||
+        (n > 0 && (rec->close_lo16 ? !record_columns_ok(rec, n) : (!rec->info || !rec->site_pos || !rec->site_seg)))) {
         mc_set_error("mc_count_records: bad arguments");
         return -12;
     }
+    RecCols cols(rec);
     int64_t too = 0, wskips = 0, multi = 0, lo_pos = INT64_MAX, top = 0;
     bool asc = true;
     int64_t prev_key = INT64_MIN;
     for (int64_t j = 0; j < n; ++j) {
-        const uint32_t info = rec->info[j];
-        const int32_t pos = rec->site_pos[j];
+        const uint32_t info = info_of(rec, j);
+        cols.to(j);
+        const int32_t pos = cols.pos(j);
         const bool is_too = (info & MC_I_TOO_MANY) != 0;
         if (counts3) {
-            const int32_t seg = rec->site_seg[j];
+            const int32_t seg = cols.seg(j);
             if (seg < 0 || seg >= n_seg) { mc_set_error("mc_count_records: record %lld names segment %d of %lld", (long long)j, seg, (long long)n_seg); return -12; }
             const int64_t key = ((int64_t)seg_read[seg] << 32) | (int64_t)(uint32_t)pos;
             asc = asc && key > prev_key;
@@ -477,7 +514,8 @@
 
 extern "C" int mc_calls_expand(const mc_calls_view *rec, int64_t n, int32_t k, int32_t *call_row_out, int64_t *close_row_out,
                                double *feats_out) {
-    if (!rec || n < 0 || (n > 0 && !rec->info) || (close_row_out && n > 0 && !rec->close_row && !rec->close_row32) ||
+    if (!rec || n < 0 || (n > 0 && !rec->info && !rec->close_lo16) || (n > 0 && rec->close_lo16 && !record_columns_ok(rec, n)) ||
+        (close_row_out && n > 0 && !rec->close_row && !rec->close_row32 && !rec->close_lo16) ||
         (feats_out && (k < 1 || k > MC_MAX_K || (!rec->feats && !(rec->feats_lo32 && rec->feats_wide))))) {
         mc_set_error("mc_calls_expand: bad arguments");
         return -12;
@@ -511,14 +549,16 @@
     mc_parallel_for(nt, [&](int w) {
         int64_t lo, hi;
         piece(w, lo, hi);
-        if (close_row_out)
-            for (int64_t j = lo; j < hi; ++j) close_row_out[j] = close_row_of(rec, j);
+        if (close_row_out) {
+            RecCols cols(rec, lo);
+            for (int64_t j = lo; j < hi; ++j) { cols.to(j); close_row_out[j] = cols.close(j); }
+        }
         if (call_row_out) {
             int64_t row = kept[(size_t)w];
             for (int64_t j = lo; j < hi; ++j) {
                 if (!rec->compacted) call_row_out[j] = (int32_t)j;
                 else if (rec->call_row) call_row_out[j] = rec->call_row[j];
-                else call_row_out[j] = (rec->info[j] & MC_I_TOO_MANY) ? -1 : (int32_t)row++;
+                else call_row_out[j] = (info_of(rec, j) & MC_I_TOO_MANY) ? -1 : (int32_t)row++;
             }
         }
         if (feats_out) {
@@ -531,6 +571,27 @@
                 cur.wide_known = true;
                 for (int64_t r = r0; r < r1; ++r) cur.feats(r, k, feats_out + r * k);
             }
+        }
+    });
+    return 0;
+}
+
+extern "C" int mc_records_expand(const mc_calls_view *rec, int64_t n, int32_t *site_pos_out, int32_t *site_seg_out, uint32_t *info_out,
+                                 int64_t *close_row_out) {
+    if (!rec || n < 0 || !record_columns_ok(rec, n)) {
+        mc_set_error("mc_records_expand: bad arguments");
+        return -12;
+    }
+    const int nt = (int)std::max<int64_t>(1, std::min<int64_t>(mc_host_cores(), n / 16384));
+    mc_parallel_for(nt, [&](int w) {
+        const int64_t lo = n * w / nt, hi = n * (w + 1) / nt;
+        RecCols cols(rec, lo);
+        for (int64_t j = lo; j < hi; ++j) {
+            cols.to(j);
+            if (site_pos_out) site_pos_out[j] = cols.pos(j);
+            if (site_seg_out) site_seg_out[j] = cols.seg(j);
+            if (info_out) info_out[j] = info_of(rec, j);
+            if (close_row_out) close_row_out[j] = cols.close(j);
         }
     });
     return 0;
diff --git a/mcaller_amd/csrc/mc_scan.hip b/mcaller_amd/csrc/mc_scan.hip
--- a/mcaller_amd/csrc/mc_scan.hip
+++ b/mcaller_amd/csrc/mc_scan.hip
@@ -952,7 +952,7 @@
     MC_FRONT_OF_THE_QUEUE;
     const DevTable &T = A.T;
     if (A.chunk_cnt && blockIdx.x == 0)
-        for (int i = threadIdx.x; i < PACK_WGS; i += blockDim.x) { A.chunk_cnt[PACK_PAD * i] = 0ull; A.chunk_cnt[PACK_PAD * i + 1] = 0ull; }
+        for (int i = threadIdx.x; i < PACK_WGS; i += blockDim.x) { A.chunk_cnt[PACK_PAD * i] = 0ull; A.chunk_cnt[PACK_PAD * i + 1] = 0ull; A.chunk_cnt[PACK_PAD * i + PACK_RUNS_LANE] = 0ull; }
     constexpr int LG = 8;
     const int64_t tile = (blockIdx.x * (int64_t)blockDim.x + threadIdx.x) / LG;
     const int l = threadIdx.x & (LG - 1);
diff --git a/mcaller_amd/csrc/mc_stream.hip b/mcaller_amd/csrc/mc_stream.hip
--- a/mcaller_amd/csrc/mc_stream.hip
+++ b/mcaller_amd/csrc/mc_stream.hip
@@ -341,6 +341,9 @@
     out->close_row32 = nullptr;
     out->compacted = 0;
     out->feats_lo32 = nullptr; out->feats_hi32 = nullptr; out->feats_wide = nullptr; out->n_wide = 0;
+    out->close_lo16 = nullptr; out->pos_lo16 = nullptr; out->info_lo16 = nullptr; out->info_next = nullptr;
+    out->runs = nullptr; out->n_runs = 0;
+    out->copy_out_bytes = 0;
     return 0;
 }
 
@@ -358,7 +361,7 @@
         b.n_nb = nb;
     }
     if (pack_rec <= 0 || pack_rec > cap) pack_rec = cap;
-    const size_t pack_bytes = std::max((size_t)pack_rec * (20 + ((size_t)k + 1) * 8 + 1) + 128, c->pack_min_bytes);
+    const size_t pack_bytes = std::max((size_t)pack_rec * (24 + ((size_t)k + 1) * 8 + 1) + 128, c->pack_min_bytes);
     if (b.cap >= cap && b.k == k && b.pack_bytes >= pack_bytes) return 0;
     if (b.used) HIP_TRY(hipEventSynchronize(b.ev[EV_DONE]));
     b.dev_allocs.clear();
@@ -407,9 +410,13 @@
     if (b.prm.score && c->clf.kind != Classifier::MLP) return 0;
     HIP_TRY(hipStreamWaitEvent(st, b.ev[EV_EMIT_END], 0));
     if (b.timed || !MC_EVENTS_ON_KERNELS) HIP_TRY(hipEventRecord(b.ev[EV_K2_START], st));
+    const bool narrow_off = getenv("MCALLER_NARROW_RECORDS") && atoi(getenv("MCALLER_NARROW_RECORDS")) == 0;
+    b.narrow = !narrow_off && b.fused_room == 0 && b.close32 && !b.want_text;
     if (!mc_launch_side(c->clf.M, other, c->n_cu, st, A, b.B.sorted, T.seg_read, c->qual, b.cap, b.prm.score ? 1 : 0, b.pack, b.pack_bytes, b.close32 ? 1 : 0, (Counters *)b.st.dev,
-                        b.fused_room, b.fused_room > 0 ? b.slots / b.fused_room : 0, MC_EVENTS_ON_KERNELS ? b.ev[EV_DONE] : nullptr))
+                        b.fused_room, b.fused_room > 0 ? b.slots / b.fused_room : 0, MC_EVENTS_ON_KERNELS ? b.ev[EV_DONE] : nullptr, b.narrow ? 1 : 0)) {
+        b.narrow = false;
         return 0;
+    }
     if (!MC_EVENTS_ON_KERNELS) HIP_TRY(hipEventRecord(b.ev[EV_DONE], st));
     HIP_TRY(hipGetLastError());
     *done = true;
@@ -443,6 +450,7 @@
         b.B.pass_no = ++c->pass_counter;
         b.used = false;
         b.want_text = 0; b.text_block = -1;
+        b.narrow = false;
         b.fused_room = 0; b.slots = 0;
         b.slot = -1;
         c->ab_head = (c->ab_head + 1) % MC_PASSES_IN_FLIGHT;
@@ -484,6 +492,7 @@
     b.want_text = c->rt.on;
     b.text_block = -1;
     b.one_kernel = false;
+    b.narrow = false;
     if (int rc = enqueue_side(c, b, A, &b.one_kernel)) return rc;
     if (!b.one_kernel) {
         if (int rc = enqueue_k2(c, b, A)) return rc;
@@ -538,7 +547,10 @@
         const size_t m = (size_t)std::min<unsigned long long>(st.n_kept, n);
         const PackLayout L = pack_layout((int64_t)n, b.close32 ? 1 : 0);
         const size_t n_wide = (size_t)std::min<unsigned long long>(st.n_wide, (unsigned long long)m * (size_t)k);
-        const PackTail PT_ = pack_tail(L.feats, m, k, n_wide);
+        const size_t n_runs = b.narrow ? (size_t)std::min<unsigned long long>(st.n_runs, (unsigned long long)n) : 0;
+        const bool narrow = n_runs > 0;
+        const NarrowLayout NL = narrow_layout((int64_t)n, (int64_t)n_runs);
+        const PackTail PT_ = pack_tail(narrow ? NL.feats : L.feats, m, k, n_wide);
         const size_t out_bytes = PT_.end;
         if (out_bytes > b.pack_bytes) {
             mc_set_error("mc_wait_records_begin: pass %llu counts %zu bytes of records, its packed block holds %zu",
@@ -553,11 +565,18 @@
             cs = c->side_stream;
             if (int rc = mc_copy_by_kernel(pack_host, b.pack, out_bytes, cs)) return rc;
         } else HIP_TRY(hipMemcpyAsync(pack_host, b.pack, out_bytes, hipMemcpyDeviceToHost, cs));
-        b.H.close_row = b.close32 ? nullptr : reinterpret_cast<int64_t *>(pack_host);
-        b.h_close32 = b.close32 ? reinterpret_cast<int32_t *>(pack_host) : nullptr;
-        b.H.site_pos = reinterpret_cast<int32_t *>(pack_host + L.pos);
-        b.H.site_seg = reinterpret_cast<int32_t *>(pack_host + L.seg);
-        b.H.info = reinterpret_cast<uint32_t *>(pack_host + L.info);
+        b.H.close_row = (b.close32 || narrow) ? nullptr : reinterpret_cast<int64_t *>(pack_host);
+        b.h_close32 = (b.close32 && !narrow) ? reinterpret_cast<int32_t *>(pack_host) : nullptr;
+        b.H.site_pos = narrow ? nullptr : reinterpret_cast<int32_t *>(pack_host + L.pos);
+        b.H.site_seg = narrow ? nullptr : reinterpret_cast<int32_t *>(pack_host + L.seg);
+        b.H.info = narrow ? nullptr : reinterpret_cast<uint32_t *>(pack_host + L.info);
+        b.h_close_lo16 = narrow ? reinterpret_cast<const uint16_t *>(pack_host + NL.close_lo) : nullptr;
+        b.h_pos_lo16 = narrow ? reinterpret_cast<const uint16_t *>(pack_host + NL.pos_lo) : nullptr;
+        b.h_info_lo16 = narrow ? reinterpret_cast<const uint16_t *>(pack_host + NL.info_lo) : nullptr;
+        b.h_info_next = narrow ? pack_host + NL.info_next : nullptr;
+        b.h_runs = narrow ? reinterpret_cast<const int32_t *>(pack_host + NL.runs) : nullptr;
+        b.h_n_runs = (int64_t)n_runs;
+        b.h_copy_out_bytes = (int64_t)out_bytes;
         b.H.feats = nullptr;
         b.h_lo32 = reinterpret_cast<int32_t *>(pack_host + PT_.lo32);
         b.H.prob = reinterpret_cast<double *>(pack_host + PT_.prob);
@@ -663,6 +682,14 @@
     out->feats_wide = packed ? b.h_wmask : nullptr;
     out->n_wide = packed ? b.h_n_wide : 0;
     out->n_call_rows = n > 0 && b.used ? b.h_n_calls : 0;
+    const bool narrow = packed && b.h_n_runs > 0;
+    out->close_lo16 = narrow ? b.h_close_lo16 : nullptr;
+    out->pos_lo16 = narrow ? b.h_pos_lo16 : nullptr;
+    out->info_lo16 = narrow ? b.h_info_lo16 : nullptr;
+    out->info_next = narrow ? b.h_info_next : nullptr;
+    out->runs = narrow ? b.h_runs : nullptr;
+    out->n_runs = narrow ? b.h_n_runs : 0;
+    out->copy_out_bytes = packed ? b.h_copy_out_bytes : 0;
     return 0;
 }
 
diff --git a/mcaller_amd/rows.py b/mcaller_amd/rows.py
--- a/mcaller_amd/rows.py
+++ b/mcaller_amd/rows.py
@@ -166,10 +166,19 @@
     def _bind(self, rec):
         n = rec.n
         self._rec = rec
-        self._info = rec.info[:n]
-        self._site_pos = rec.site_pos[:n]
-        self._seg_of = rec.site_seg[:n]
         self._lazy = None
+
+    @property
+    def _info(self):
+        return self._rec.info[:self._rec.n]
+
+    @property
+    def _site_pos(self):
+        return self._rec.site_pos[:self._rec.n]
+
+    @property
+    def _seg_of(self):
+        return self._rec.site_seg[:self._rec.n]
 
     def _per_record(self):
         if self._lazy is None:
@@ -332,7 +341,7 @@
     if n == 0:
         every = set(names[int(r)] for r in seg_read)
         return every, every, False
-    first_seg, last_seg = int(rec.site_seg[0]), int(rec.site_seg[n - 1])
+    first_seg, last_seg = rec.end_segments()
     return (set(names[int(r)] for r in seg_read[:first_seg + 1]), set(names[int(r)] for r in seg_read[last_seg:]), True)
 
 
```
